# pierluigiferrari/fcn8s_tensorflow

Measured on AMD Instinct MI355X. Metric: training images/sec at 1024x512 bs16, higher is better.
Workload: dtype f32; 1 GPU; FCN-8s (VGG-16, fc6 7x7, 20 classes) train step, 1024x512, 16 images/GPU, SGD+momentum, keep_prob 0.5; global_batch=16, parallelism=dp1

## Files before the change

### fcn8s_tensorflow_amd/csrc/fcn8s_internal.h

```cpp
#pragma once
#include <hip/hip_runtime.h>
#include <stdint.h>
#include <cmath>
#include "../../include/fcn8s_hip.h"

#if defined(__HIP_DEVICE_COMPILE__) && !defined(__gfx950__)
#error "libfcn8s_hip is written for gfx950 (MI355X) only: build with --offload-arch=gfx950"
#endif
#define FCN8S_LDS_BYTES_NEEDED (160u * 1024u)

#include <string>
namespace fcn8s {

extern thread_local const char* g_last_kernel;
void defer_error(int code, const char* fmt, ...) __attribute__((format(printf, 2, 3)));
int take_deferred_error(std::string* text);

struct IgemmArgs {
    const float* x; const float* w; const float* bias; const float* addend; const float* mask;
    float* y;
    int N, Ma, Mb; long long M;
    int Hi, Wi, Cin, ldx;
    int KW, in_scale, tap_step, tap_off, Ktot;
    int Ho, Wo, Cout, ldy;
    int out_scale, out_offy, out_offx;
    int phases_x; long long w_phase_stride;
    float alpha; int relu; float mask_scale;
    int dropout; float keep_prob; unsigned long long seed; unsigned int stream_id;
    int batched; long long x_batch_stride, y_batch_stride;
    int m_fastest;
    int bt, ldw;
    int fixed_tile;
    int split;
};
void launch_igemm(const IgemmArgs& a, int phases, hipStream_t s);

struct Bf16ConvArgs {
    const float* x; const unsigned short* xh;
    const unsigned short* wt; const float* bias; float* y;
    int N, H, W, Cin, Cout, K;
    int relu, dropout; float keep_prob; unsigned long long seed; unsigned int stream_id;
    long long M; int m_fastest;
};
void launch_w_to_bf16_tiles(const float* w, unsigned short* wt, int K, int Cout, hipStream_t s);
bool launch_conv_bf16(const Bf16ConvArgs& a, hipStream_t s);
void launch_f32_to_bf16(const float* x, unsigned short* y, long long n, hipStream_t s);
struct Bf16Conv256Args {
    const unsigned short* xp; const unsigned short* wt; const float* bias; float* y;
    int N, H, W, Cin, Cout, K;
    int relu, dropout; float keep_prob; unsigned long long seed; unsigned int stream_id;
    long long M; int m_fastest;
    const float* addend;
    const float* mask; float mask_scale;
    int any_shape;
    const unsigned short* mask16;
    float* colpart;
    int ksplit; float* part;
    int rows_bn;
    int guarded;
    unsigned short* yb; int yb_pad;
    long long xp_ps, yb_ps, mask16_ps;
};
bool conv_bf16_256_ok(long long M, int Cin, int Cout, int mode);
void launch_w_to_bf16_t(const float* w, unsigned short* wt, int K, int Cout, hipStream_t s);
void launch_f32_to_bf16_padded(const float* x, unsigned short* xp, int N, int H, int W, int C, int pad, hipStream_t s, long long ps = 0);
int conv_bf16_rows_bm(int Cout, int rows_bn);
bool launch_conv_bf16_256(const Bf16Conv256Args& a, hipStream_t s);
struct Fp8ConvArgs {
    const unsigned char* xp = nullptr; long long xp_ps = 0;
    const unsigned char* wq = nullptr; const int* ew = nullptr;
    const float* bias = nullptr; float* y = nullptr;
    unsigned char* yq = nullptr; long long yq_ps = 0; int yq_pad = 0, yq_exp = 0;
    int ex = 0, relu = 1;
    int N = 0, H = 0, W = 0, Cin = 0, Cout = 0, K = 1;
    long long M = 0;
};
bool launch_conv_fp8(const Fp8ConvArgs& a, hipStream_t s);
void launch_w_to_fp8(const float* w, unsigned char* wq, int* ew, unsigned* amax_scratch, int rows, int Cout, hipStream_t s);
void launch_f32_to_fp8_padded(const float* x, unsigned char* xq, int N, int H, int W, int C, int pad, long long ps, int ex, hipStream_t s);
void launch_zero_border_fp8(unsigned char* xq, int planes, long long ps, int N, int H, int W, int pad, hipStream_t s);
void launch_maxpool_fp8(const unsigned char* xq, long long xps, unsigned char* yq, long long yps, int N, int H, int W, int C, int ypad, hipStream_t s);
void launch_amax(const float* x, long long n, unsigned* amax, hipStream_t s);
bool launch_f32_to_bf16_padded_colsum(const float* x, unsigned short* xp, float* db, int N, int H, int W, int C, int pad, hipStream_t s, long long ps = 0);
void launch_w_to_bf16_flip_t(const float* w, unsigned short* wt, int K, int Cin, int Cout, hipStream_t s);
struct Bf16WgradArgs {
    const unsigned short* A; const unsigned short* B; float* C;
    long long R; int Ci, Cj, K, Wp;
    long long chunk, split_stride; int plain_store;
    long long a_ps, b_ps;
};
bool launch_wgrad_bf16(const Bf16WgradArgs& a, hipStream_t s);

struct WgradArgs {
    const float* A; const float* B; float* C;
    int N, Pa, Pb; long long P;
    int Ha, Wa, Adim, lda, Areal;
    int Bdim, ldb;
    int KW, a_scale, tap_off, ntaps;
    int ldc;
    float alpha;
    float* colsum;
    int batched; long long a_batch_stride, b_batch_stride;
    int c_uninitialized;
    int plain_store;
    int split;
    long long split_stride;
};
void launch_wgrad(const WgradArgs& a, hipStream_t s);

extern thread_local int t_deterministic;
float* det_scratch(hipStream_t s, size_t floats);
float* scratch2(hipStream_t s, size_t floats);
void scratch_release(hipStream_t s);
long long scratch_bytes_live();
void launch_det_reduce(float* C, const float* ws, long long rows, int cols, int ldc, long long slab, int nsplit, bool accumulate, hipStream_t s);
bool launch_wgrad_taps(const float* X, const float* dZ, float* dW, float* db, int N, int H, int W, int Cin, int Cout,
                       int K, hipStream_t s);

bool launch_conv1_wgrad(const float* X4, const float* dZ, float* dW, float* db, int N, int H, int W, int Cout, int mfma, hipStream_t s);

bool launch_conv1_fwd(const float* x4, const float* w48, const float* bias, float* y, const float* zero16, int N, int H, int W, int Cout, int tiled, hipStream_t s, unsigned short* yb16 = nullptr, long long yb16_ps = 0);

bool launch_tconv_wgrad(const float* X, const float* dY, float* dW, int N, int Hi, int Wi, int C, int K, int S, hipStream_t s);

void launch_preprocess(const void* img, int dtype, float* out4, long long npix, hipStream_t s);
void launch_maxpool_fwd(const float* x, float* y, int N, int H, int W, int C, hipStream_t s);
void launch_maxpool_bwd(const float* x, const float* dy, float* dx, int N, int H, int W, int C,
                        int relu_mask, hipStream_t s);
void launch_maxpool_route(const float* x, unsigned char* route, int N, int H, int W, int C, hipStream_t s);
void launch_maxpool_fwd_route(const float* x, float* y, unsigned char* r, int N, int H, int W, int C, hipStream_t s, unsigned short* yb16 = nullptr, int pad = 0, long long yb16_ps = 0, int round16 = 0);
void launch_maxpool_fwd_route16(const unsigned short* xb, long long xb_ps, unsigned char* r, int N, int H, int W, int C, hipStream_t s, unsigned short* yb16, int pad, long long yb16_ps);
struct PixMap { int blocked, H, W, QH, QW, S; };
static __host__ __device__ inline long long pixmap_slots(const PixMap& m, long long npix, int N) { return m.blocked ? (long long)N * m.QH * m.QW * m.S * m.S : npix; }
int  softmax_xent_blocks(long long npix);
void launch_softmax_xent(const float* logits, const uint8_t* labels, float* dlogits, double* partials,
                         long long npix, int C, float grad_scale, hipStream_t s, float* colsum = nullptr,
                         const PixMap* map = nullptr, int N = 0);
enum XentPhase { XENT_PLAIN = 0, XENT_WEIGHTED = 1, XENT_OHEM_LOSS = 2, XENT_OHEM_GRAD = 3 };
struct OhemState {
    unsigned long long valid, ntau, kept;
    unsigned long long krem, above;
    unsigned prefix; int active;
    float t, gscale;
    unsigned pad[2];
};
static_assert(sizeof(OhemState) == 64, "OhemState: 64 bytes");
constexpr size_t LOSS_SCRATCH_BYTES = sizeof(OhemState) + (2048 + 2048 + 1024) * sizeof(unsigned);
struct XentEx {
    const float* cw = nullptr;
    float* lbuf = nullptr;
    OhemState* st = nullptr;
    unsigned* hist = nullptr;
    float tau = 0.f;
    float ce_scale = 1.f;
    const uint8_t* codes = nullptr;
    const float* ptab = nullptr;
};
void launch_softmax_xent_ex(const float* logits, const uint8_t* labels, float* dlogits, double* partials, long long npix, int C, float grad_scale,
                            hipStream_t s, float* colsum, const PixMap* map, int N, const XentEx& x, float ohem_thresh, long long ohem_min_kept);
void launch_finalize_loss(const double* partials, int nparts, long long npix, const float* regsum,
                          float rate, float* loss_out, hipStream_t s, const unsigned long long* den = nullptr, float* terms = nullptr);
struct LovaszLayout {
    int nseg = 0, C = 0, tiles = 0; long long L = 0, nsc = 0;
    size_t o_keys[2] = {0, 0}, o_pays[2] = {0, 0}, o_hist = 0, o_tcnt = 0, o_part = 0, o_G = 0, o_V = 0, o_w = 0, o_ncls = 0, o_colpart = 0, o_lov = 0;
    size_t bytes = 0;
};
LovaszLayout lovasz_layout(long long npix, int nseg, int C);
double lovasz_bytes(long long npix, int C, int nmask);
void launch_lovasz_loss(const float* x, int is_logits, const uint8_t* labels, const PixMap* map, int N, long long npix, const LovaszLayout& y,
                        int classes_all, const uint8_t* mask_dev, char* ws, float* class_loss, float* terms, float lce, float llov, float* loss_out,
                        hipStream_t s);
void launch_lovasz_backward(const float* x, int is_logits, const uint8_t* labels, const PixMap* map, int N, long long npix, const LovaszLayout& y,
                            char* ws, float lambda, int accumulate, float* out, float* colsum, hipStream_t s);
void launch_lovasz_total(float* terms, float lce, float* loss_out, hipStream_t s);
size_t soft_targets_scratch_bytes();
double soft_targets_bytes(long long npix, int C, int K);
void launch_soft_targets(const float* logits, float* dlogits, const float* probs, const uint8_t* labels, const PixMap* map, int N, long long npix, int C,
                         int K, long long row_stride, float lambda, float temperature, int all_pixels, char* ws, float* loss, float* term,
                         float* lastbias, hipStream_t s);
void launch_softmax_argmax(const float* logits, float* softmax_out, long long* argmax_out,
                           long long npix, int C, hipStream_t s, const PixMap* map = nullptr, int N = 0);
void launch_tconv_im2col(const float* x, float* A, int N, int Hi, int Wi, int C, int KP, hipStream_t s);
void launch_tconv_col2im(const float* dA, float* dx, int N, int Hi, int Wi, int C, int KP, hipStream_t s);
void launch_tconv_pack_gemm(const float* w, const float* bias, float* b2, float* b2t, float* bias_tiled, int C, int S, int KP, hipStream_t s);
void launch_tconv_unpack_dw(const float* db2, float* dw, int C, int S, hipStream_t s);
void launch_unblock_logits(const float* blocked, float* nhwc, const PixMap& map, int N, int C, hipStream_t s);
void launch_onehot_to_ids(const void* oh, int elem_bytes, long long npix, int C, uint8_t* ids, int* bad, hipStream_t s);
void launch_confusion(const uint8_t* labels, const long long* pred, long long npix,
                      unsigned long long* conf, int C, hipStream_t s);
bool launch_head_fwd(const float* x, const float* w, const float* bias, float* y, long long M, int K, int C, float alpha, hipStream_t s,
                     float* scratch = nullptr, size_t scratch_floats = 0);
bool launch_head_dgrad(const float* dy, const float* wt, const float* mask, float mask_scale, float* dx, long long M, int K, int C, float alpha,
                       hipStream_t s);
bool launch_head_wgrad(const float* x, const float* dy, float* dw, long long M, int K, int C, float alpha, hipStream_t s);
bool launch_maxpool_bwd_bf16(const float* x, const float* dy, unsigned short* dzb, float* db, int N, int H, int W, int C, hipStream_t s, const unsigned char* route = nullptr, long long dzb_ps = 0);
void launch_colsum(const float* x, float* out, long long rows, int C, hipStream_t s);
void launch_sumsq(const float* x, float* out, long long n, hipStream_t s);
void launch_axpy(float* y, const float* x, float a, long long n, hipStream_t s);
void launch_grad_accumulate(float* dst, const float* src, long long n, int mode, hipStream_t s);
constexpr int kGradNormBlocks = 2048;
struct UpdateStats { float norm, clip, scale; int ok; unsigned long long skipped; };
void launch_grad_norm(const float* g, long long n, float grad_scale, float max_norm, double* partials, void* out, bool as_floats, hipStream_t s);
struct UpdateArgs {
    int opt; float* theta; const float* g; float* m; float* v; float* shadow; long long n;
    float p0, p1, p2, p3, gs; const float* s_dev; const int* ok_dev; float ema_w;
};
void launch_update(const UpdateArgs& a, hipStream_t s);
inline float tf_adam_lr_t(float lr, float b1, float b2, long long t)
{
    return lr * (float)std::sqrt(1.0 - std::pow((double)b2, (double)t)) / (float)(1.0 - std::pow((double)b1, (double)t));
}
void launch_ema_update(float* sh, const float* theta, long long n, float w, const int* ok_dev, hipStream_t s);
void launch_swap(float* a, float* b, long long n, hipStream_t s);
void launch_flip_transpose(const float* w, float* wt, int taps, int Cin, int Cout, hipStream_t s);
void launch_pad_cin(const float* w, float* w4, int taps, int Cin, int Cinp, int Cout, hipStream_t s);
void launch_tconv_phase_pack(const float* w, float* wp, int K, int S, int C, hipStream_t s);
void launch_dropout_mask(float* mask, long long n, float keep_prob, unsigned long long seed,
                         unsigned int stream_id, hipStream_t s);
int wino_r(int KS);
int wino_nsub(int KS);
int wino_alpha(int tile, int KS);
long long wino_slab(long long T, int C);
void launch_wino_filter(int tile, const float* w, float* u, int Cin, int Cout, int KS, hipStream_t s, int transpose_out = 0);
void launch_wino_input(int tile, const float* x, float* v, int N, int H, int W, int C, int KS, hipStream_t s, unsigned* rbits_out = nullptr);
void launch_wino_input_conv1(const float* x0, const float* w4, const float* bias, float* v, int N, int H, int W, hipStream_t s, unsigned* rbits_out = nullptr);
void launch_wino_input_xb(const float* x, float* v, unsigned short* xb, int N, int H, int W, int C, hipStream_t s, unsigned* rbits_out = nullptr);
bool launch_wino_input_dout(int tile, const float* dy, float* v, float* dm, int N, int H, int W, int C, hipStream_t s, const unsigned char* pidx = nullptr);
void launch_wino_output(int tile, const float* m, const float* bias, const float* addend, const float* mask, float mask_scale,
                        int relu, float* y, int N, int H, int W, int C, int dropout, float keep, unsigned long long seed,
                        unsigned int stream_id, hipStream_t s, float* pool = nullptr, unsigned char* pidx = nullptr, int KS = 3,
                        unsigned* rbits_out = nullptr, const unsigned* rbits_in = nullptr);
size_t wino_rbits_words(int tile, int N, int H, int W, int C);
void launch_wino_dout(int tile, const float* dy, float* dm, int N, int H, int W, int C, hipStream_t s, int KS = 3, const unsigned char* pidx = nullptr);
void launch_wino_dgrad_output_dout(const float* dv, const unsigned* rbits_in, float* dm, int N, int H, int W, int C, hipStream_t s);
void launch_wino_dgrad_output_sub44(const float* dv, float* dx, int N, int H, int W, int C, hipStream_t s);
void launch_wino_dgrad_output(const float* dv, const float* addend, const float* mask, float mask_scale, const unsigned* rbits_in, float* y,
                              int N, int H, int W, int C, hipStream_t s);
bool launch_wino_out_in(const float* m, const float* bias, float* v, unsigned* rbits_out, int N, int H, int W, int C, hipStream_t s, bool always = false);
void launch_wino_dfilter(int tile, const float* du, float* dw, int Cin, int Cout, int KS, hipStream_t s);
int fft_fc6_planes();
long long fft_fc6_tiles(int N, int H, int W);
void launch_fft_fc6_filter(const float* w, float* uf, int Cin, int Cout, hipStream_t s);
void launch_fft_fc6_dfilter(const float* duf, float* dw, int Cin, int Cout, hipStream_t s);
void launch_fft_fc6_input(const float* x, float* xf, int N, int H, int W, int C, hipStream_t s);
void launch_fft_fc6_output(const float* yf, const float* bias, float* y, int N, int H, int W, int C, int relu, int dropout, float keep,
                           unsigned long long seed, unsigned int stream_id, hipStream_t s);
void launch_fft_fc6_dout(const float* dz, float* dyf, int N, int H, int W, int C, hipStream_t s);
void launch_fft_fc6_din(const float* dxf, float* patches, float* dx, int N, int H, int W, int C, hipStream_t s);
void launch_augment_u8(const unsigned char* img, const unsigned char* lab, unsigned char* oimg, unsigned char* olab, const int* params,
                       const unsigned char* vlut, int N, int H, int W, int Ho, int Wo, int void_id, hipStream_t s);
void launch_resample_u8(const unsigned char* img, const unsigned char* lab, unsigned char* oimg, unsigned char* olab, const int* params,
                        int N, int H, int W, int Ho, int Wo, int void_id, hipStream_t s);
void launch_tta_input(const void* img, int dtype, int N, int H, int W, int Hs, int Ws, int Hp, int Wp, int flip, float* out4, hipStream_t s);
void launch_tta_accumulate(const float* logits, const PixMap& map, int N, int Hs, int Ws, int flip, int C, int H, int W, float* acc,
                           int first, int last, int npasses, float* softmax_out, long long* argmax_out, hipStream_t s);
void launch_mc_accumulate(const float* logits, const PixMap& map, int N, int H, int W, int C, float* acc, float* ent_acc, int first, int last,
                          int nsamples, float* softmax_out, long long* argmax_out, float* entropy_out, float* mi_out, hipStream_t s);
bool crf_shape_supported(int C, int radius);
void launch_crf_meanfield(const float* qin, const float* prob, const unsigned char* img, int N, int H, int W, int C, int radius, int dilation,
                          float w_app, float w_smooth, float theta_alpha, float theta_beta, float theta_gamma, float* qout, long long* am, hipStream_t s);
void launch_crf_argmax(const float* p, long long npix, int C, long long* am, hipStream_t s);
size_t cityscapes_work_bytes(int N);
void launch_cityscapes_pair(const uint8_t* gt, const uint16_t* inst, const void* pred, int pred_kind, int N, long long P,
                            unsigned long long* conf, void* work, int* entries, int max_entries, unsigned long long* counts, hipStream_t s);
void launch_reliability_pair(const float* prob, const uint8_t* gt, const uint8_t* lut, const float* const* scores, const float* scales, int J,
                             int N, long long P, int C, int B, unsigned long long* calib, unsigned long long* sums, unsigned long long* hist,
                             unsigned long long* bad, hipStream_t s);
// ... 49 lines not shown
```

### fcn8s_tensorflow_amd/csrc/igemm.hip

```cpp
#include "fcn8s_internal.h"
#include <cmath>
#include <cstdlib>
#include <atomic>
#include <map>
#include <mutex>
#include <string>

namespace fcn8s {

thread_local const char* g_last_kernel = nullptr;
#define FCN8S_STR2(x) #x
#define FCN8S_STR(x) FCN8S_STR2(x)

typedef float f32x16 __attribute__((ext_vector_type(16)));
constexpr int BK_ = 16;

static __device__ __forceinline__ float4 ldg4(const float* p) { return *reinterpret_cast<const float4*>(p); }

static __device__ __forceinline__ unsigned xcd_swizzle(unsigned p, unsigned total)
{
    const unsigned q = total >> 3, r = total & 7u, xcd = p & 7u, i = p >> 3;
    return (xcd < r ? xcd * (q + 1) : r * (q + 1) + (xcd - r) * q) + i;
}

thread_local int t_deterministic = 0;
namespace {
struct ScratchBuf { float* p = nullptr; size_t cap = 0; };
std::mutex g_scratch_mu;
std::map<std::pair<int, hipStream_t>, ScratchBuf> g_scratch[2];
std::atomic<long long> g_scratch_bytes{0};
float* scratch_get(int which, hipStream_t s, size_t floats, size_t floor_)
{
    int dev = 0; (void)hipGetDevice(&dev);
    std::lock_guard<std::mutex> lk(g_scratch_mu);
    ScratchBuf& b = g_scratch[which][std::make_pair(dev, s)];
    if (b.cap < floats) {
        if (b.p) { hipFree(b.p); g_scratch_bytes -= (long long)(b.cap * sizeof(float)); }
        b.p = nullptr; b.cap = 0;
        size_t want = floats + floats / 4 + (1u << 20);
        if (want < floor_) want = floor_;
        if (hipMalloc((void**)&b.p, want * sizeof(float)) != hipSuccess) { (void)hipGetLastError(); return nullptr; }
        b.cap = want; g_scratch_bytes += (long long)(want * sizeof(float));
    }
    return b.p;
}
}
float* det_scratch(hipStream_t s, size_t floats) { return scratch_get(0, s, floats, 0); }
float* scratch2(hipStream_t s, size_t floats) { return scratch_get(1, s, floats, 1u << 18); }
void scratch_release(hipStream_t s)
{
    int dev = 0; (void)hipGetDevice(&dev);
    std::lock_guard<std::mutex> lk(g_scratch_mu);
    for (auto& pool : g_scratch) {
        auto it = pool.find(std::make_pair(dev, s));
        if (it != pool.end()) { if (it->second.p) { hipFree(it->second.p); g_scratch_bytes -= (long long)(it->second.cap * sizeof(float)); } pool.erase(it); }
    }
}
long long scratch_bytes_live() { return g_scratch_bytes.load(); }
__global__ __launch_bounds__(256) void det_reduce_kernel(float* __restrict__ C, const float* __restrict__ ws, const long long n, const int cols, const int ldc,
                                                         const long long slab, const int nsplit, const int accumulate)
{
    for (long long i = blockIdx.x * 256LL + threadIdx.x; i < n; i += (long long)gridDim.x * 256) {
        const long long off = (cols == ldc) ? i : (i / cols) * ldc + (i % cols);
        float v = accumulate ? C[off] : 0.f;
        const float* w = ws + off;
        for (int k = 0; k < nsplit; ++k) v += w[(long long)k * slab];
        C[off] = v;
    }
}
void launch_det_reduce(float* C, const float* ws, long long rows, int cols, int ldc, long long slab, int nsplit, bool accumulate, hipStream_t s)
{
    const long long n = rows * cols;
    if (n <= 0) return;
    long long blocks = (n + 255) / 256; if (blocks > 8192) blocks = 8192;
    hipLaunchKernelGGL(det_reduce_kernel, dim3((unsigned)blocks), dim3(256), 0, s, C, ws, n, cols, ldc, slab, nsplit, accumulate ? 1 : 0);
}
static __device__ __attribute__((noinline)) float dropout_apply(float v, unsigned long long idx, unsigned long long seed,
                                                               unsigned int stream, float keep)
{
    return philox_uniform(idx, seed, stream) < keep ? v / keep : 0.f;
}

template <int BM, int BN, int WM, int WN, int MODE, int BK>
__global__ __launch_bounds__(256, (MODE != 0 && BM * BN <= 128 * 128) ? 4 : 1) void igemm_fwd_kernel(const IgemmArgs p)
{
    constexpr bool FAST = MODE != 0;
    constexpr bool PLAIN = MODE == 3;
    constexpr int LDA = BK + 4, LDB = BN, F4R = BK / 4;
    constexpr int TM = BM / WM / 32, TN = BN / WN / 32;
    constexpr int A_LD = BM * F4R / 256;
    constexpr int B_F4 = BK * BN / 4;
    constexpr int B_LD = (B_F4 + 255) / 256;
    static_assert(WM * WN == 4, "4 waves");
    static_assert(TM >= 1 && TN >= 1, "tile");
    __shared__ __attribute__((aligned(16))) float smem[2 * BM * LDA + 2 * BK * LDB];
    float* As = smem;
    float* Bs = smem + 2 * BM * LDA;

    const int tid = threadIdx.x, lane = tid & 63, wave = tid >> 6;
    const int wm = wave / WN, wn = wave % WN;
    const int pz = blockIdx.z;
    const int pzy = p.batched ? 0 : pz / p.phases_x, pzx = p.batched ? 0 : pz - pzy * p.phases_x;
    const float* __restrict__ Wp = p.w + (long long)pz * p.w_phase_stride;
    const float* __restrict__ X = p.batched ? p.x + (long long)pz * p.x_batch_stride : p.x;
    float* __restrict__ Y = p.batched ? p.y + (long long)pz * p.y_batch_stride : p.y;
    const int offy = p.out_offy + pzy, offx = p.out_offx + pzx;
    const unsigned ntn = (unsigned)((p.Cout + BN - 1) / BN);
    const unsigned lid = xcd_swizzle(blockIdx.x, gridDim.x);
    const unsigned ntm = gridDim.x / ntn;
    const long long m0 = (long long)(p.m_fastest ? lid % ntm : lid / ntn) * BM;
    const int n0 = (int)(p.m_fastest ? lid / ntm : lid % ntn) * BN;
    const int MaMb = p.Ma * p.Mb;

    long long a_base[A_LD];
    int a_iy[A_LD], a_ix[A_LD];
    bool a_ok[A_LD];
#pragma unroll
    for (int i = 0; i < A_LD; ++i) {
        const int row = (tid + i * 256) / F4R;
        const long long m = m0 + row;
        a_ok[i] = m < p.M;
        if (PLAIN) { a_iy[i] = a_ix[i] = 0; a_base[i] = a_ok[i] ? m : 0; continue; }
        const long long mm = a_ok[i] ? m : 0;
        const int n = (int)(mm / MaMb);
        const int r = (int)(mm - (long long)n * MaMb);
        const int a = r / p.Mb, b = r - a * p.Mb;
        a_iy[i] = a * p.in_scale; a_ix[i] = b * p.in_scale;
        a_base[i] = (long long)n * p.Hi * p.Wi;
    }
    const int a_c4 = (tid % F4R) * 4;

    float4 ra[A_LD], rb[B_LD];
    constexpr bool TAP_INNER = MODE == 2;
    int f_ci0 = 0, f_ty = 0, f_tx = 0, f_tap = 0;
    const int ntaps = FAST ? p.Ktot / p.Cin : 1;
    const float* a_ptr[A_LD];
    unsigned a_mask[A_LD];
    bool a_val[A_LD], a_ldok[A_LD];
    const float* b_ptr[B_LD];
    auto set_tap = [&]() {
        if (PLAIN) {
#pragma unroll
            for (int i = 0; i < A_LD; ++i) { a_val[i] = a_ok[i]; a_ptr[i] = X + a_base[i] * p.ldx + a_c4; }
            return;
        }
        const int dy = f_ty * p.tap_step + p.tap_off, dx = f_tx * p.tap_step + p.tap_off;
#pragma unroll
        for (int i = 0; i < A_LD; ++i) {
            const int iy = a_iy[i] + dy, ix = a_ix[i] + dx;
            a_val[i] = a_ok[i] && (unsigned)iy < (unsigned)p.Hi && (unsigned)ix < (unsigned)p.Wi;
            const long long pix = a_val[i] ? a_base[i] + (long long)iy * p.Wi + ix : 0;
            a_ptr[i] = X + pix * p.ldx + a_c4;
        }
    };
    if (FAST) {
        if (TAP_INNER) {
#pragma unroll
            for (int i = 0; i < A_LD; ++i) {
                unsigned mk = 0;
                for (int t = 0; t < ntaps; ++t) {
                    const int ty = t / p.KW, tx = t - ty * p.KW;
                    const int iy = a_iy[i] + ty * p.tap_step + p.tap_off, ix = a_ix[i] + tx * p.tap_step + p.tap_off;
                    if (a_ok[i] && (unsigned)iy < (unsigned)p.Hi && (unsigned)ix < (unsigned)p.Wi) mk |= 1u << t;
                }
                a_mask[i] = mk;
                a_ptr[i] = X + (a_base[i] + (long long)a_iy[i] * p.Wi + a_ix[i]) * p.ldx + a_c4;
            }
        } else set_tap();
#pragma unroll
        for (int i = 0; i < B_LD; ++i) {
            const int f = tid + i * 256;
            const int k = f / (BN / 4), j = (f - k * (BN / 4)) * 4;
            b_ptr[i] = Wp + (long long)k * p.Cout + n0 + j;
        }
    }
    auto gload_fast = [&]() {
        if (TAP_INNER) {
            const long long delta = ((long long)(f_ty * p.tap_step + p.tap_off) * p.Wi + (f_tx * p.tap_step + p.tap_off)) * p.ldx + f_ci0;
            const long long boff = ((long long)f_tap * p.Cin + f_ci0) * p.Cout;
#pragma unroll
            for (int i = 0; i < A_LD; ++i) {
                const bool ok = (a_mask[i] >> f_tap) & 1u;
                ra[i] = ldg4(ok ? a_ptr[i] + delta : X);
                a_ldok[i] = ok;
            }
#pragma unroll
            for (int i = 0; i < B_LD; ++i)
                if (B_F4 % 256 == 0 || tid + i * 256 < B_F4) rb[i] = ldg4(b_ptr[i] + boff);
            ++f_tap;
            if (++f_tx == p.KW) { f_tx = 0; ++f_ty; }
            if (f_tap == ntaps) { f_tap = 0; f_tx = 0; f_ty = 0; f_ci0 += BK; }
        } else {
#pragma unroll
            for (int i = 0; i < A_LD; ++i) {
                ra[i] = ldg4(a_ptr[i] + f_ci0);
// ... 319 lines not shown
    int a_off[TM], a_sw[TM];
#pragma unroll
    for (int tm = 0; tm < TM; ++tm) {
        const int row = wm * TM * 32 + tm * 32 + (lane & 31);
        a_off[tm] = row * BK;
        a_sw[tm] = (row >> 2) & 3;
    }
    const int b_off = ((lane >> 5) * 4) * BN + wn * TN * 32 + (lane & 31);
    int bt_off[TN], bt_sw[TN];
#pragma unroll
    for (int tn = 0; tn < TN; ++tn) {
        const int row = wn * TN * 32 + tn * 32 + (lane & 31);
        bt_off[tn] = row * BK;
        bt_sw[tn] = (row >> 2) & 3;
    }
    auto compute = [&](int stage) {
        if (idle) return;
        const float* sa = smem + stage * STAGE;
        const float* sb = sa + BM * BK;
        if constexpr (NSPLIT >= 2) {
            Bf16Pieces<NSPLIT> ap[TM], bp[TN];
#pragma unroll
            for (int tm = 0; tm < TM; ++tm) {
                const float4 u = *reinterpret_cast<const float4*>(sa + a_off[tm] + (((2 * (lane >> 5)) ^ a_sw[tm]) * 4));
                const float4 v = *reinterpret_cast<const float4*>(sa + a_off[tm] + (((2 * (lane >> 5) + 1) ^ a_sw[tm]) * 4));
                const float x[8] = {u.x, u.y, u.z, u.w, v.x, v.y, v.z, v.w};
                split_bf16<NSPLIT>(x, ap[tm]);
            }
#pragma unroll
            for (int tn = 0; tn < TN; ++tn) {
                float x[8];
                if (BT) {
                    const float4 u = *reinterpret_cast<const float4*>(sb + bt_off[tn] + (((2 * (lane >> 5)) ^ bt_sw[tn]) * 4));
                    const float4 v = *reinterpret_cast<const float4*>(sb + bt_off[tn] + (((2 * (lane >> 5) + 1) ^ bt_sw[tn]) * 4));
                    x[0] = u.x; x[1] = u.y; x[2] = u.z; x[3] = u.w; x[4] = v.x; x[5] = v.y; x[6] = v.z; x[7] = v.w;
                } else {
#pragma unroll
                    for (int j = 0; j < 8; ++j) x[j] = sb[((lane >> 5) * 8 + j) * BN + wn * TN * 32 + tn * 32 + (lane & 31)];
                }
                split_bf16<NSPLIT>(x, bp[tn]);
            }
#pragma unroll
            for (int tm = 0; tm < TM; ++tm)
#pragma unroll
                for (int tn = 0; tn < TN; ++tn) acc[tm][tn] = mfma_split<NSPLIT>(ap[tm], bp[tn], acc[tm][tn]);
            return;
        }
#pragma unroll
        for (int kk2 = 0; kk2 < BK / 8; ++kk2) {
            float4 af[TM];
            float bf[TN][4];
#pragma unroll
            for (int tm = 0; tm < TM; ++tm)
                af[tm] = *reinterpret_cast<const float4*>(sa + a_off[tm] + (((kk2 * 2 + (lane >> 5)) ^ a_sw[tm]) * 4));
#pragma unroll
            for (int tn = 0; tn < TN; ++tn) {
                if (BT) {
                    const float4 t = *reinterpret_cast<const float4*>(sb + bt_off[tn] + (((kk2 * 2 + (lane >> 5)) ^ bt_sw[tn]) * 4));
                    bf[tn][0] = t.x; bf[tn][1] = t.y; bf[tn][2] = t.z; bf[tn][3] = t.w;
                } else {
#pragma unroll
                    for (int j = 0; j < 4; ++j) bf[tn][j] = sb[b_off + (kk2 * 8 + j) * BN + tn * 32];
                }
            }
#pragma unroll
            for (int j = 0; j < 4; ++j)
#pragma unroll
                for (int tm = 0; tm < TM; ++tm) {
                    const float av = j == 0 ? af[tm].x : j == 1 ? af[tm].y : j == 2 ? af[tm].z : af[tm].w;
#pragma unroll
                    for (int tn = 0; tn < TN; ++tn) acc[tm][tn] = __builtin_amdgcn_mfma_f32_32x32x2f32(av, bf[tn][j], acc[tm][tn], 0, 0, 0);
                }
        }
    };

#pragma unroll
    for (int t = 0; t < S - 1; ++t)
        if (t < nkt) issue(t, t);
    int stage = 0, pre = S - 1;
    for (int kt = 0; kt < nkt; ++kt) {
        if (kt + S - 2 < nkt) wait_vmcnt<(S - 2) * L>(); else wait_vmcnt<0>();
        __builtin_amdgcn_s_barrier();
        if (kt + S - 1 < nkt) issue(kt + S - 1, pre);
        compute(stage);
        stage = stage + 1 == S ? 0 : stage + 1;
        pre = pre + 1 == S ? 0 : pre + 1;
    }

    if (gridDim.y > 1) {
#pragma unroll
        for (int tn = 0; tn < TN; ++tn)
#pragma unroll
            for (int tm = 0; tm < TM; ++tm)
#pragma unroll
                for (int r = 0; r < 16; ++r) {
                    const long long m = m0 + wm * TM * 32 + tm * 32 + (r & 3) + 8 * (r >> 2) + 4 * (lane >> 5);
                    if (m < p.M) unsafeAtomicAdd(Y + m * p.ldy + n0 + wn * TN * 32 + tn * 32 + (lane & 31), acc[tm][tn][r]);
                }
        return;
    }
    if (!EPI) {
        __builtin_amdgcn_s_barrier();
        constexpr int LDT = 36;
        float* patch = smem + wave * 32 * LDT;
#pragma unroll
        for (int tn = 0; tn < TN; ++tn)
#pragma unroll
            for (int tm = 0; tm < TM; ++tm) {
#pragma unroll
                for (int r = 0; r < 16; ++r) patch[((r & 3) + 8 * (r >> 2) + 4 * (lane >> 5)) * LDT + (lane & 31)] = acc[tm][tn][r];
                __builtin_amdgcn_wave_barrier();
                const long long mrow = m0 + wm * TM * 32 + tm * 32;
                float* yb = Y + n0 + wn * TN * 32 + tn * 32 + (lane & 7) * 4;
                const float4 bv = p.bias ? ldg4(p.bias + n0 + wn * TN * 32 + tn * 32 + (lane & 7) * 4) : make_float4(0.f, 0.f, 0.f, 0.f);
#pragma unroll
                for (int j = 0; j < 4; ++j) {
                    const int row = j * 8 + (lane >> 3);
                    float4 v = *reinterpret_cast<const float4*>(&patch[row * LDT + (lane & 7) * 4]);
                    v.x += bv.x; v.y += bv.y; v.z += bv.z; v.w += bv.w;
                    if (mrow + row < p.M) {
                        if (p.mask) {
                            const float4 mk = ldg4(p.mask + (mrow + row) * p.ldy + n0 + wn * TN * 32 + tn * 32 + (lane & 7) * 4);
                            v.x = mk.x > 0.f ? v.x * p.mask_scale : 0.f; v.y = mk.y > 0.f ? v.y * p.mask_scale : 0.f;
                            v.z = mk.z > 0.f ? v.z * p.mask_scale : 0.f; v.w = mk.w > 0.f ? v.w * p.mask_scale : 0.f;
                        }
                        *reinterpret_cast<float4*>(yb + (mrow + row) * p.ldy) = v;
                    }
                }
                __builtin_amdgcn_wave_barrier();
            }
        return;
    }
#pragma unroll
    for (int tn = 0; tn < TN; ++tn) {
        const int col = n0 + wn * TN * 32 + tn * 32 + (lane & 31);
        const float bv = p.bias ? p.bias[col] : 0.f;
#pragma unroll
        for (int tm = 0; tm < TM; ++tm)
#pragma unroll
            for (int r = 0; r < 16; ++r) {
                const long long m = m0 + wm * TM * 32 + tm * 32 + (r & 3) + 8 * (r >> 2) + 4 * (lane >> 5);
                if (m >= p.M) continue;
                const long long off = m * p.ldy;
                float v = acc[tm][tn][r] * p.alpha + bv;
                if (p.addend) v += p.addend[off + col];
                if (p.relu) v = v > 0.f ? v : 0.f;
                if (p.mask) v = p.mask[off + col] > 0.f ? v * p.mask_scale : 0.f;
                if (p.dropout) v = dropout_apply(v, (unsigned long long)(off + col), p.seed, p.stream_id, p.keep_prob);
                Y[off + col] = v;
            }
    }
}

static __device__ __forceinline__ void glds16v(const float* vaddr, unsigned lds_byte_off)
{
    asm volatile("s_mov_b32 m0, %1\n\ts_nop 0\n\tglobal_load_lds_dwordx4 %0, off" ::"v"(vaddr), "s"(lds_byte_off) : "memory", "m0");
}
struct Conv1Args { const float* x4; const float* w48; const float* bias; float* y; const float* zero16; int N, H, W; long long M;
                   unsigned short* yb16; long long yb16_ps; };

__global__ __launch_bounds__(256, 4) void conv1_glds_kernel(const Conv1Args p)
{
    constexpr int BM = 128, BN = 64, BK = 16, NKT = 3, WN = 2, TM = 2, TN = 1, CH = 4, RPI = 16;
    constexpr int A_PW = BM / RPI / 4;
    constexpr int STAGE = BM * BK + BK * BN;
    __shared__ __attribute__((aligned(16))) float smem[NKT * STAGE];
    const int tid = threadIdx.x, lane = tid & 63, wave = __builtin_amdgcn_readfirstlane(tid >> 6);
    const int wm = wave / WN, wn = wave % WN;
    const long long m0 = (long long)blockIdx.x * BM;
    const unsigned lds0 = (unsigned)(size_t)(__attribute__((address_space(3))) float*)smem;
#pragma unroll
    for (int i = 0; i < A_PW; ++i) {
        const int row = (wave * A_PW + i) * RPI + lane / CH, pc = lane % CH;
        const int c = pc ^ ((row >> 2) & 3);
        long long m = m0 + row; if (m >= p.M) m = p.M - 1;
        const int x = (int)(m % p.W); const long long r = m / p.W; const int y = (int)(r % p.H);
#pragma unroll
        for (int kt = 0; kt < NKT; ++kt) {
            const int t = kt * 4 + c, dy = t / 3 - 1, dx = t % 3 - 1;
            const bool ok = t < 9 && (unsigned)(y + dy) < (unsigned)p.H && (unsigned)(x + dx) < (unsigned)p.W;
            const float* src = ok ? p.x4 + (m + (long long)dy * p.W + dx) * 4 : p.zero16;
            glds16v(src, lds0 + (unsigned)(kt * STAGE + (wave * A_PW + i) * 256) * 4u);
        }
    }
    {
        const int f = wave * 64 + lane;
#pragma unroll
        for (int kt = 0; kt < NKT; ++kt)
            glds16v(p.w48 + (kt * BK + f / (BN / 4)) * BN + (f % (BN / 4)) * 4, lds0 + (unsigned)(kt * STAGE + BM * BK + wave * 256) * 4u);
    }
    f32x16 acc[TM][TN];
#pragma unroll
    for (int i = 0; i < TM; ++i)
#pragma unroll
        for (int r = 0; r < 16; ++r) acc[i][0][r] = 0.f;
    wait_vmcnt<0>();
    __builtin_amdgcn_s_barrier();
    int a_off[TM], a_sw[TM];
#pragma unroll
    for (int tm = 0; tm < TM; ++tm) {
        const int row = wm * TM * 32 + tm * 32 + (lane & 31);
        a_off[tm] = row * BK; a_sw[tm] = (row >> 2) & 3;
    }
    const int b_off = ((lane >> 5) * 4) * BN + wn * TN * 32 + (lane & 31);
#pragma unroll
    for (int kt = 0; kt < NKT; ++kt) {
        const float* sa = smem + kt * STAGE;
        const float* sb = sa + BM * BK;
#pragma unroll
        for (int kk2 = 0; kk2 < BK / 8; ++kk2) {
            if (kt == NKT - 1 && kk2 == 1) continue;
            float4 af[TM]; float bf[3];
#pragma unroll
            for (int tm = 0; tm < TM; ++tm) af[tm] = *reinterpret_cast<const float4*>(sa + a_off[tm] + (((kk2 * 2 + (lane >> 5)) ^ a_sw[tm]) * 4));
#pragma unroll
            for (int j = 0; j < 3; ++j) bf[j] = sb[b_off + (kk2 * 8 + j) * BN];
#pragma unroll
            for (int j = 0; j < 3; ++j)
#pragma unroll
                for (int tm = 0; tm < TM; ++tm) {
                    const float av = j == 0 ? af[tm].x : j == 1 ? af[tm].y : af[tm].z;
                    acc[tm][0] = __builtin_amdgcn_mfma_f32_32x32x2f32(av, bf[j], acc[tm][0], 0, 0, 0);
                }
        }
    }
    __builtin_amdgcn_s_barrier();
    constexpr int LDT = 36;
    float* patch = smem + wave * 32 * LDT;
    const float4 bv = ldg4(p.bias + wn * 32 + (lane & 7) * 4);
#pragma unroll
    for (int tm = 0; tm < TM; ++tm) {
#pragma unroll
        for (int r = 0; r < 16; ++r) patch[((r & 3) + 8 * (r >> 2) + 4 * (lane >> 5)) * LDT + (lane & 31)] = acc[tm][0][r];
        __builtin_amdgcn_wave_barrier();
        const long long mrow = m0 + wm * TM * 32 + tm * 32;
        float* yb = p.y + wn * 32 + (lane & 7) * 4;
#pragma unroll
        for (int j = 0; j < 4; ++j) {
            const int row = j * 8 + (lane >> 3);
            float4 v = *reinterpret_cast<const float4*>(&patch[row * LDT + (lane & 7) * 4]);
            v.x = fmaxf(v.x + bv.x, 0.f); v.y = fmaxf(v.y + bv.y, 0.f); v.z = fmaxf(v.z + bv.z, 0.f); v.w = fmaxf(v.w + bv.w, 0.f);
            if (mrow + row < p.M) *reinterpret_cast<float4*>(yb + (mrow + row) * BN) = v;
        }
        __builtin_amdgcn_wave_barrier();
    }
}
template <int TPB>
__global__ __launch_bounds__(256, 4) void conv1_tile_kernel(const Conv1Args p)
{
    constexpr int TH = 8, TW = 16, BN = 64, BK = 16, NKT = 3, WN = 2, TM = 2, HW_ = TW + 2, HH_ = TH + 2;
    constexpr int LDT = 36;
    __shared__ __attribute__((aligned(16))) float sB[NKT * BK * BN];
    __shared__ __attribute__((aligned(16))) float4 halo[HH_ * HW_];
    __shared__ __attribute__((aligned(16))) float patches[4 * 32 * LDT];
    const int tid = threadIdx.x, lane = tid & 63, wave = __builtin_amdgcn_readfirstlane(tid >> 6);
    const int wm = wave / WN, wn = wave % WN;
    const int tiles_x = p.W / TW / TPB, tiles_y = p.H / TH;
    const int bx = blockIdx.x % tiles_x, by = (blockIdx.x / tiles_x) % tiles_y, n = blockIdx.x / (tiles_x * tiles_y);
    const int y0 = by * TH;
#pragma unroll
    for (int i = 0; i < 3; ++i) reinterpret_cast<float4*>(sB)[tid + i * 256] = ldg4(p.w48 + (tid + i * 256) * 4);
    const float4 bv = ldg4(p.bias + wn * 32 + (lane & 7) * 4);
    float* patch = patches + wave * 32 * LDT;
#pragma unroll 1
  for (int it = 0; it < TPB; ++it) {
    const int x0 = (bx * TPB + it) * TW;
    if (it) __syncthreads();
    if (tid < HH_ * HW_) {
        const int hy = tid / HW_, hx = tid - hy * HW_, yy = y0 + hy - 1, xx = x0 + hx - 1;
        float4 v = make_float4(0.f, 0.f, 0.f, 0.f);
        if ((unsigned)yy < (unsigned)p.H && (unsigned)xx < (unsigned)p.W) v = ldg4(p.x4 + (((long long)n * p.H + yy) * p.W + xx) * 4);
        halo[tid] = v;
    }
    f32x16 acc[TM];
#pragma unroll
    for (int i = 0; i < TM; ++i)
#pragma unroll
        for (int r = 0; r < 16; ++r) acc[i][r] = 0.f;
    __syncthreads();
    int hbase[TM];
#pragma unroll
    for (int tm = 0; tm < TM; ++tm) {
        const int g = wm * TM + tm, py = 2 * g + ((lane & 31) >> 4), px = lane & 15;
        hbase[tm] = (py + 1) * HW_ + (px + 1);
    }
    const int b_off = ((lane >> 5) * 4) * BN + wn * 32 + (lane & 31);
#pragma unroll
    for (int kt = 0; kt < NKT; ++kt) {
#pragma unroll
        for (int kk2 = 0; kk2 < BK / 8; ++kk2) {
            if (kt == NKT - 1 && kk2 == 1) continue;
            const int t = kt * 4 + kk2 * 2 + (lane >> 5), tt = t < 9 ? t : 4, dy = tt / 3 - 1, dx = tt % 3 - 1;
            float4 af[TM]; float bf[3];
#pragma unroll
            for (int tm = 0; tm < TM; ++tm) af[tm] = halo[hbase[tm] + dy * HW_ + dx];
#pragma unroll
            for (int j = 0; j < 3; ++j) bf[j] = sB[kt * BK * BN + b_off + (kk2 * 8 + j) * BN];
#pragma unroll
            for (int j = 0; j < 3; ++j)
#pragma unroll
                for (int tm = 0; tm < TM; ++tm) {
                    const float av = j == 0 ? af[tm].x : j == 1 ? af[tm].y : af[tm].z;
                    acc[tm] = __builtin_amdgcn_mfma_f32_32x32x2f32(av, bf[j], acc[tm], 0, 0, 0);
                }
        }
    }
#pragma unroll
    for (int tm = 0; tm < TM; ++tm) {
#pragma unroll
        for (int r = 0; r < 16; ++r) patch[((r & 3) + 8 * (r >> 2) + 4 * (lane >> 5)) * LDT + (lane & 31)] = acc[tm][r];
        __builtin_amdgcn_wave_barrier();
        const int g = wm * TM + tm;
#pragma unroll
        for (int j = 0; j < 4; ++j) {
            const int row = j * 8 + (lane >> 3);
            float4 v = *reinterpret_cast<const float4*>(&patch[row * LDT + (lane & 7) * 4]);
            v.x = fmaxf(v.x + bv.x, 0.f); v.y = fmaxf(v.y + bv.y, 0.f); v.z = fmaxf(v.z + bv.z, 0.f); v.w = fmaxf(v.w + bv.w, 0.f);
            const long long pix = ((long long)n * p.H + y0 + 2 * g + (row >> 4)) * p.W + x0 + (row & 15);
            if (p.y) *reinterpret_cast<float4*>(p.y + pix * BN + wn * 32 + (lane & 7) * 4) = v;
        }
        if (p.yb16) {
            const float4 b0 = ldg4(p.bias + wn * 32 + (lane & 3) * 8), b1 = ldg4(p.bias + wn * 32 + (lane & 3) * 8 + 4);
#pragma unroll
            for (int j = 0; j < 2; ++j) {
                const int row = j * 16 + (lane >> 2);
                const float4 u = *reinterpret_cast<const float4*>(&patch[row * LDT + (lane & 3) * 8]);
                const float4 w_ = *reinterpret_cast<const float4*>(&patch[row * LDT + (lane & 3) * 8 + 4]);
                __attribute__((ext_vector_type(8))) __bf16 o;
                o[0] = (__bf16)fmaxf(u.x + b0.x, 0.f); o[1] = (__bf16)fmaxf(u.y + b0.y, 0.f); o[2] = (__bf16)fmaxf(u.z + b0.z, 0.f); o[3] = (__bf16)fmaxf(u.w + b0.w, 0.f);
                o[4] = (__bf16)fmaxf(w_.x + b1.x, 0.f); o[5] = (__bf16)fmaxf(w_.y + b1.y, 0.f); o[6] = (__bf16)fmaxf(w_.z + b1.z, 0.f); o[7] = (__bf16)fmaxf(w_.w + b1.w, 0.f);
                const long long q = ((long long)n * (p.H + 2) + y0 + 2 * g + (row >> 4) + 1) * (p.W + 2) + x0 + (row & 15) + 1;
                *reinterpret_cast<__attribute__((ext_vector_type(8))) __bf16*>(p.yb16 + (p.yb16_ps ? (long long)wn * p.yb16_ps + q * 32 + (lane & 3) * 8 : q * BN + wn * 32 + (lane & 3) * 8)) = o;
            }
        }
        __builtin_amdgcn_wave_barrier();
    }
  }
}

bool launch_conv1_fwd(const float* x4, const float* w48, const float* bias, float* y, const float* zero16, int N, int H, int W, int Cout, int tiled, hipStream_t s, unsigned short* yb16, long long yb16_ps)
{
    if (Cout != 64 || !bias || !zero16) return false;
    if ((yb16 || !y) && !(tiled && H % 8 == 0 && W % 16 == 0)) return false;
    Conv1Args a{x4, w48, bias, y, zero16, N, H, W, (long long)N * H * W, yb16, yb16_ps};
    if (tiled && H % 8 == 0 && W % 16 == 0) {
        g_last_kernel = "conv1_tile_kernel";
        const long long tiles = (long long)N * (H / 8) * (W / 16);
        if (W % 64 == 0 && tiles >= 4 * 4096) hipLaunchKernelGGL(conv1_tile_kernel<4>, dim3((unsigned)(tiles / 4)), dim3(256), 0, s, a);
        else                                  hipLaunchKernelGGL(conv1_tile_kernel<1>, dim3((unsigned)tiles), dim3(256), 0, s, a);
        return true;
    }
    g_last_kernel = "conv1_glds_kernel";
    hipLaunchKernelGGL(conv1_glds_kernel, dim3((unsigned)((a.M + 127) / 128)), dim3(256), 0, s, a);
    return true;
}

template <int BM, int BN, int WM, int WN, int BKF = 16>
static void launch_igemm_cfg(const IgemmArgs& a0, int phases, hipStream_t s)
{
    IgemmArgs a = a0;
    a.m_fastest = (double)a.Ktot * a.Cout > (double)a.M * a.Cin;
    dim3 grid((unsigned)(((a.M + BM - 1) / BM) * ((a.Cout + BN - 1) / BN)), 1, (unsigned)phases);
    const bool fast = (phases == 1 || a.batched) && a.Cin % BKF == 0 && a.Cout % BN == 0 && a.Ktot % a.Cin == 0;
    const bool tap_inner = fast && (double)a.Ktot * a.Cout * 4.0 <= 64e6 && a.Ktot / a.Cin <= 32;
    const bool plain = fast && a.batched && a.Ktot == a.Cin && !a.bias && !a.addend && !a.mask && !a.relu && !a.dropout && a.alpha == 1.f &&
                       a.out_scale == 1 && a.ldy >= a.Cout && a.ldy % 4 == 0 && a.in_scale == 1 && a.tap_off == 0;
    const int mode = !fast ? 0 : (plain ? 3 : (tap_inner ? 2 : 1));
    static const std::string base = "igemm_fwd_kernel<" + std::to_string(BM) + ", " + std::to_string(BN) + ", " + std::to_string(WM) + ", " + std::to_string(WN) + ", ";
    static const std::string tags[4] = {base + "0, 16>", base + "1, " + std::to_string(BKF) + ">", base + "2, " + std::to_string(BKF) + ">",
                                        base + "3, " + std::to_string(BKF) + ">"};
    g_last_kernel = tags[mode].c_str();
    const bool linear = (mode == 1 || mode == 3) && !a.relu && !a.mask && !a.dropout && !a.addend && a.out_scale == 1 && a.ldy == a.Cout;
    constexpr int splitk_min_kt = 64;
    const unsigned nblocks = grid.x * (unsigned)phases, nkt_all = (unsigned)(a.Ktot / BKF);
    if (linear && !t_deterministic && !a.fixed_tile && ((grid.x < 512 && nkt_all >= 512) || (nblocks < 2048 && nkt_all >= (unsigned)splitk_min_kt))) {
        unsigned ks = nkt_all >= 512 && grid.x < 512 ? 1024 / grid.x : 4096 / nblocks;
        if (ks > 8) ks = 8;
        if (ks > nkt_all / 16) ks = nkt_all / 16;
        if (ks >= 2) {
            grid.y = ks;
            const size_t nfl = a.batched ? (size_t)(phases - 1) * a.y_batch_stride + (size_t)a.M * a.Cout : (size_t)a.M * a.Cout;
            hipMemsetAsync(a.y, 0, nfl * sizeof(float), s);
        }
    }
    const bool rows1x1 = fast && a.Ktot == a.Cin && a.in_scale == 1 && a.tap_off == 0 && a.out_scale == 1 && a.out_offy == 0 && a.out_offx == 0 &&
                         (a.batched || (phases == 1 && a.Hi == a.Ma && a.Wi == a.Mb && a.Ho == a.Ma && a.Wo == a.Mb)) && a.ldy >= a.Cout;
    const bool bias_only = fast && a.bias && !a.addend && !a.mask && !a.relu && !a.dropout && a.alpha == 1.f && a.ldy % 4 == 0 && a.Cout % 4 == 0 && grid.y == 1;
    if constexpr (BN >= 64 && BKF == 16) {
        if (rows1x1 && (mode == 3 || grid.y == 1) && (long long)(BM - 1) * a.ldx < (1LL << 29) && (long long)16 * a.Cout < (1LL << 29)) {
            static const std::string gbase = "gemm_glds_kernel<" + std::to_string(BM) + ", " + std::to_string(BN) + ", " + std::to_string(WM) + ", " + std::to_string(WN) + ", 3, ";
            static const std::string xbase = "gemm_glds_x3_kernel<" + std::to_string(BM) + ", " + std::to_string(BN) + ", " + std::to_string(WM) + ", " + std::to_string(WN) + ", 3, ";
            static const std::string gt[4] = {gbase + "false>", gbase + "true>", xbase + "false>", xbase + "true>"};
            const bool mask_only = fast && a.mask && !a.bias && !a.addend && !a.relu && !a.dropout && a.alpha == 1.f && a.ldy % 4 == 0 && a.Cout % 4 == 0 && grid.y == 1;
            const bool epi = mode != 3 && !bias_only && !mask_only;
            if (a.bt) {
                static const std::string nb = "gemm_glds_nt_kernel<" + std::to_string(BM) + ", " + std::to_string(BN) + ", " + std::to_string(WM) + ", " + std::to_string(WN) + ", 3>";
                static const std::string nbx = "gemm_glds_nt_x3_kernel<" + std::to_string(BM) + ", " + std::to_string(BN) + ", " + std::to_string(WM) + ", " + std::to_string(WN) + ", 3>";
                if (mode != 3 || (long long)(BN - 1) * a.ldw >= (1LL << 29)) { defer_error(FCN8S_ERR_STATE, "transposed-B GEMM needs the plain batched form"); return; }
                static const std::string nbx2 = "gemm_glds_nt_x2_kernel<" + std::to_string(BM) + ", " + std::to_string(BN) + ", " + std::to_string(WM) + ", " + std::to_string(WN) + ", 3>";
                g_last_kernel = (a.split == 3 ? nbx : a.split == 2 ? nbx2 : nb).c_str();
                if (a.split == 3) hipLaunchKernelGGL((gemm_glds_nt_x3_kernel<BM, BN, WM, WN, 3>), grid, dim3(256), 0, s, a);
                else if (a.split == 2) hipLaunchKernelGGL((gemm_glds_nt_x2_kernel<BM, BN, WM, WN, 3>), grid, dim3(256), 0, s, a);
                else                   hipLaunchKernelGGL((gemm_glds_nt_kernel<BM, BN, WM, WN, 3>), grid, dim3(256), 0, s, a);
                return;
            }
            g_last_kernel = gt[(epi ? 1 : 0) + (a.split == 3 ? 2 : 0)].c_str();
            if (a.split == 3) {
                if (epi) hipLaunchKernelGGL((gemm_glds_x3_kernel<BM, BN, WM, WN, 3, true>), grid, dim3(256), 0, s, a);
                else     hipLaunchKernelGGL((gemm_glds_x3_kernel<BM, BN, WM, WN, 3, false>), grid, dim3(256), 0, s, a);
                return;
            }
            if (a.split == 2) {
                static const std::string x2base = "gemm_glds_x2_kernel<" + std::to_string(BM) + ", " + std::to_string(BN) + ", " + std::to_string(WM) + ", " + std::to_string(WN) + ", 3, ";
                static const std::string x2t[2] = {x2base + "false>", x2base + "true>"};
                g_last_kernel = x2t[epi ? 1 : 0].c_str();
                if (epi) hipLaunchKernelGGL((gemm_glds_x2_kernel<BM, BN, WM, WN, 3, true>), grid, dim3(256), 0, s, a);
                else     hipLaunchKernelGGL((gemm_glds_x2_kernel<BM, BN, WM, WN, 3, false>), grid, dim3(256), 0, s, a);
                return;
            }
            if (epi) hipLaunchKernelGGL((gemm_glds_kernel<BM, BN, WM, WN, 3, true>), grid, dim3(256), 0, s, a);
            else     hipLaunchKernelGGL((gemm_glds_kernel<BM, BN, WM, WN, 3, false>), grid, dim3(256), 0, s, a);
            return;
        }
    }
    if (a.bt) {
        defer_error(FCN8S_ERR_STATE, "transposed-B GEMM (M %lld, K %d, N %d, tile %dx%d) does not fit the LDS-DMA kernel", a.M, a.Ktot, a.Cout, BM, BN);
        return;
    }
    if (mode == 3)      hipLaunchKernelGGL((igemm_fwd_kernel<BM, BN, WM, WN, 3, BKF>), grid, dim3(256), 0, s, a);
    else if (mode == 2) hipLaunchKernelGGL((igemm_fwd_kernel<BM, BN, WM, WN, 2, BKF>), grid, dim3(256), 0, s, a);
    else if (mode == 1) hipLaunchKernelGGL((igemm_fwd_kernel<BM, BN, WM, WN, 1, BKF>), grid, dim3(256), 0, s, a);
    else                hipLaunchKernelGGL((igemm_fwd_kernel<BM, BN, WM, WN, 0, 16>), grid, dim3(256), 0, s, a);
}

void launch_igemm(const IgemmArgs& a, int phases, hipStream_t s)
{
    auto cost = [&](int bm, int bn, int bpc, double eff) {
        const long long blocks = ((a.M + bm - 1) / bm) * ((a.Cout + bn - 1) / bn) * phases;
        const long long n = (blocks + 255) / 256, rem = n % bpc;
        const double tail = rem == 0 ? 0.0 : (rem == 1 ? 2.0 : (rem == 2 ? 2.4 : 3.0));
        return ((double)(n / bpc) * bpc + tail) * bm * bn / eff;
    };
    if (a.fixed_tile && a.Cout % 128 == 0) { launch_igemm_cfg<128, 128, 2, 2>(a, phases, s); return; }
    if (a.fixed_tile && a.Cout % 64 == 0)  { launch_igemm_cfg<128, 64, 2, 2>(a, phases, s); return; }
    if (a.Cout <= 32)      launch_igemm_cfg<128, 32, 4, 1>(a, phases, s);
    else if (a.Cout <= 64) {
        if (cost(128, 64, 4, 1.0) <= cost(64, 64, 4, 0.9)) launch_igemm_cfg<128, 64, 2, 2>(a, phases, s);
        else                                               launch_igemm_cfg<64, 64, 2, 2>(a, phases, s);
    } else {
        const double c128 = cost(128, 128, 3, 1.0), c64x128 = cost(64, 128, 4, 0.9), c64 = cost(64, 64, 4, 0.85);
        if (a.M > 64 && c128 <= c64x128 && c128 <= c64) launch_igemm_cfg<128, 128, 2, 2>(a, phases, s);
        else if (c64x128 <= c64)                        launch_igemm_cfg<64, 128, 2, 2>(a, phases, s);
        else                                            launch_igemm_cfg<64, 64, 2, 2>(a, phases, s);
    }
}

template <int BM, int BN, int WM, int WN, int WK, bool FAST, bool COLSUM>
__global__ __launch_bounds__(256, FAST ? 4 : 1) void wgrad_kernel(const WgradArgs p, const int chunk)
{
    constexpr int BK = 16, LDA = BM, LDB = BN;
    constexpr int TM = BM / WM / 32, TN = BN / WN / 32;
    constexpr int A_F4 = BK * BM / 4, B_F4 = BK * BN / 4;
    constexpr int A_LD = (A_F4 + 255) / 256, B_LD = (B_F4 + 255) / 256;
    static_assert(WM * WN * WK == 4, "4 waves");
    __shared__ __attribute__((aligned(16))) float smem[2 * BK * LDA + 2 * BK * LDB];
    float* As = smem;
    float* Bs = smem + 2 * BK * LDA;

    const int tid = threadIdx.x, lane = tid & 63, wave = tid >> 6;
    const int wk = wave / (WM * WN), wmn = wave % (WM * WN);
    const int wm = wmn / WN, wn = wmn % WN;
    const int ntj = (p.Bdim + BN - 1) / BN;
    const int ti = blockIdx.x / ntj, tj = blockIdx.x - ti * ntj;
    const int i0 = ti * BM, j0 = tj * BN;
    const int tap = blockIdx.z;
    const int ty = tap / p.KW, tx = tap - ty * p.KW;
    const int dy = p.batched ? 0 : ty + p.tap_off, dx = p.batched ? 0 : tx + p.tap_off;
    const float* __restrict__ Ap = p.batched ? p.A + (long long)tap * p.a_batch_stride : p.A;
    const float* __restrict__ Bp = p.batched ? p.B + (long long)tap * p.b_batch_stride : p.B;
    const long long pbeg = (long long)blockIdx.y * chunk;
    const long long pend = (pbeg + chunk < p.P) ? pbeg + chunk : p.P;
    const int PaPb = p.Pa * p.Pb;
    const bool do_colsum = COLSUM && p.colsum != nullptr && tap == 0 && ti == 0 && wm == 0;

    float4 ra[A_LD], rb[B_LD];
    int s_n[A_LD], s_a[A_LD], s_b[A_LD], s_left[A_LD];
    const float* b_ptr[B_LD]; int b_left[B_LD];
    bool a_ldok[A_LD], b_ldok[B_LD];
    if (FAST) {
#pragma unroll
        for (int i = 0; i < A_LD; ++i) {
            const int f = tid + i * 256;
            const int pix = f / (BM / 4);
            const long long pp = pbeg + pix;
            const long long q = pp < p.P ? pp : 0;
            s_n[i] = (int)(q / PaPb);
            const int r = (int)(q - (long long)s_n[i] * PaPb);
            s_a[i] = r / p.Pb; s_b[i] = r - s_a[i] * p.Pb;
            s_left[i] = (int)(pend - pp);
        }
#pragma unroll
        for (int i = 0; i < B_LD; ++i) {
            const int f = tid + i * 256;
            const int pix = f / (BN / 4), c = (f - pix * (BN / 4)) * 4;
            b_ptr[i] = Bp + (pbeg + pix) * p.ldb + j0 + c;
            b_left[i] = (int)(pend - (pbeg + pix));
        }
    }
    auto gload_fast = [&]() {
#pragma unroll
        for (int i = 0; i < A_LD; ++i) {
            const int f = tid + i * 256;
            const int c = (f % (BM / 4)) * 4;
            const int iy = s_a[i] * p.a_scale + dy, ix = s_b[i] * p.a_scale + dx;
            const bool ok = s_left[i] > 0 && (unsigned)iy < (unsigned)p.Ha && (unsigned)ix < (unsigned)p.Wa;
            const long long pixi = ok ? ((long long)s_n[i] * p.Ha + iy) * p.Wa + ix : 0;
            ra[i] = ldg4(Ap + pixi * p.lda + i0 + c);
            a_ldok[i] = ok;
            s_left[i] -= BK;
            s_b[i] += BK;
            if (s_b[i] >= p.Pb) { s_b[i] -= p.Pb; if (++s_a[i] >= p.Pa) { s_a[i] = 0; ++s_n[i]; } }
        }
#pragma unroll
        for (int i = 0; i < B_LD; ++i) {
            const bool ok = b_left[i] > 0;
            rb[i] = ldg4(ok ? b_ptr[i] : Bp);
            b_ldok[i] = ok;
            b_ptr[i] += (long long)BK * p.ldb;
            b_left[i] -= BK;
        }
    };
    auto gload = [&](long long pk) {
        if (FAST) { gload_fast(); return; }
#pragma unroll
        for (int i = 0; i < A_LD; ++i) {
            const int f = tid + i * 256;
            const int pix = f / (BM / 4), c = (f - pix * (BM / 4)) * 4;
            const long long pp = pk + pix;
            bool ok = (A_F4 % 256 == 0 || f < A_F4) && pp < pend && (i0 + c) < p.Adim;
            long long off = 0;
            if (ok) {
                const int n = (int)(pp / PaPb);
                const int r = (int)(pp - (long long)n * PaPb);
                const int a = r / p.Pb, b = r - a * p.Pb;
                const int iy = a * p.a_scale + dy, ix = b * p.a_scale + dx;
                ok = (unsigned)iy < (unsigned)p.Ha && (unsigned)ix < (unsigned)p.Wa;
                off = (((long long)n * p.Ha + iy) * p.Wa + ix) * p.lda + i0 + c;
            }
            ra[i] = ok ? ldg4(Ap + off) : make_float4(0.f, 0.f, 0.f, 0.f);
        }
#pragma unroll
        for (int i = 0; i < B_LD; ++i) {
            const int f = tid + i * 256;
            const int pix = f / (BN / 4), c = (f - pix * (BN / 4)) * 4;
            const long long pp = pk + pix;
            const bool ok = (B_F4 % 256 == 0 || f < B_F4) && pp < pend && (j0 + c) < p.Bdim;
            rb[i] = ok ? ldg4(Bp + pp * p.ldb + j0 + c) : make_float4(0.f, 0.f, 0.f, 0.f);
        }
    };
    auto sstore = [&](int buf) {
#pragma unroll
        for (int i = 0; i < A_LD; ++i) {
            const int f = tid + i * 256;
            if (A_F4 % 256 == 0 || f < A_F4) {
                const int pix = f / (BM / 4), c = (f - pix * (BM / 4)) * 4;
                if (FAST && !a_ldok[i]) ra[i] = make_float4(0.f, 0.f, 0.f, 0.f);
                *reinterpret_cast<float4*>(&As[buf * BK * LDA + pix * LDA + c]) = ra[i];
            }
        }
#pragma unroll
        for (int i = 0; i < B_LD; ++i) {
            const int f = tid + i * 256;
            if (B_F4 % 256 == 0 || f < B_F4) {
                const int pix = f / (BN / 4), c = (f - pix * (BN / 4)) * 4;
                if (FAST && !b_ldok[i]) rb[i] = make_float4(0.f, 0.f, 0.f, 0.f);
                *reinterpret_cast<float4*>(&Bs[buf * BK * LDB + pix * LDB + c]) = rb[i];
            }
        }
    };

    f32x16 acc[TM][TN];
    f32x16 accs[COLSUM ? TN : 1];
#pragma unroll
    for (int j = 0; j < TN; ++j) {
#pragma unroll
        for (int r = 0; r < 16; ++r) if (COLSUM) accs[j][r] = 0.f;
#pragma unroll
        for (int i = 0; i < TM; ++i)
#pragma unroll
            for (int r = 0; r < 16; ++r) acc[i][j][r] = 0.f;
    }

    auto compute = [&](int buf) {
        const float* A = As + buf * BK * LDA + (lane >> 5) * LDA + wm * TM * 32 + (lane & 31);
        const float* B = Bs + buf * BK * LDB + (lane >> 5) * LDB + wn * TN * 32 + (lane & 31);
        constexpr int KK = 8 / WK;
#pragma unroll
// ... 720 lines not shown
```

### fcn8s_tensorflow_amd/csrc/model.hip

```cpp
#include "../../include/fcn8s_hip.h"
#include "fcn8s_internal.h"
#include "device_buffer.h"
#include "pass_state.h"
#include "conv_route.h"
#include <cstdarg>
#include <functional>

#include <dlfcn.h>
#include <atomic>
#include <chrono>
#include <thread>
#include <cmath>
#include <cstdio>
#include <cstring>
#include <cstdlib>
#include <algorithm>
#include <mutex>
#include <map>
#include <set>
#include <string>
#include <vector>

using namespace fcn8s;

extern "C" {
typedef struct ncclComm* ncclComm_t;
typedef struct { char internal[128]; } ncclUniqueId;
typedef enum { ncclSuccess = 0, ncclUnhandledCudaError = 1, ncclSystemError = 2, ncclInternalError = 3, ncclInvalidArgument = 4, ncclInvalidUsage = 5,
               ncclRemoteError = 6, ncclInProgress = 7 } ncclResult_t;
typedef enum { ncclSum = 0 } ncclRedOp_t;
typedef enum { ncclFloat = 7, ncclDouble = 8 } ncclDataType_t;
}
static_assert(sizeof(ncclUniqueId) == FCN8S_COMM_ID_BYTES, "fcn8s_comm_unique_id hands out ncclUniqueId bytes");

namespace {

thread_local std::string g_last_error;
thread_local int t_deferred_code = 0;
thread_local std::string t_deferred_text;

struct ParamInfo {
    std::string name;
    int ndim;
    int64_t shape[4];
    size_t offset, numel;
};

struct ProfGroup {
    std::string name;
    std::vector<std::pair<hipEvent_t, hipEvent_t>> ev;
    std::vector<std::pair<hipEvent_t, hipEvent_t>> ev_shared;
    double flops = 0, bytes = 0;
    int64_t launches = 0;
};

struct Act { float* p = nullptr; size_t n = 0; int H = 0, W = 0, C = 0; };

const int kConvsPerBlock[5] = {2, 2, 3, 3, 3};

struct Layer {
    char name[8], pool_name[8], pool_in[12];
    int block, pos, nconv;
    int h, w, cin, cout, K, real_cin;
    int prev, next;
    size_t w_off, b_off;
    int i_y, i_rb, i_wv, i_pool, i_pidx;
    float *y, *wv, *pool; unsigned* rb; unsigned char* pidx;
    int tile;
    RbWriter rb_writer;
    bool out_in_next, conv1_in_next;
    bool dm_from_next, pool_in_transform;
    ConvShape shape(int N) const { return ConvShape{N, h, w, cin, cout, K}; }
    bool first() const { return real_cin != 0; }
    bool last_of_block() const { return pos == nconv; }
};

}

namespace fcn8s {
void defer_error(int code, const char* fmt, ...)
{
    if (t_deferred_code) return;
    char buf[1024];
    va_list ap; va_start(ap, fmt); vsnprintf(buf, sizeof buf, fmt, ap); va_end(ap);
    t_deferred_code = code; t_deferred_text = buf;
}
int take_deferred_error(std::string* text)
{
    const int c = t_deferred_code;
    if (c && text) *text = t_deferred_text;
    t_deferred_code = 0; t_deferred_text.clear();
    return c;
}
}

struct Q8Buf { DeviceBuf<unsigned char> p; int N = 0, H = 0, W = 0, C = 0, pad = -1, ex = 0; long long ps = 0; };
struct W8Bank { DeviceBuf<unsigned char> wq; int* ew = nullptr; unsigned* amax = nullptr; };

struct fcn8s_model {
    int C = 20, fc6k = 7, device = 0;
    int widths[7] = {64, 128, 256, 512, 512, 4096, 4096};
    uint64_t seed = 0;
    std::vector<ParamInfo> params;
    std::map<std::string, int> index;
    size_t total = 0;
    size_t bucket_off[FCN8S_MAX_BUCKETS] = {0}, bucket_n[FCN8S_MAX_BUCKETS] = {0};
    hipEvent_t bucket_ev[FCN8S_MAX_BUCKETS] = {nullptr};
    bool bucket_final[FCN8S_MAX_BUCKETS] = {false};
    ncclComm_t comm = nullptr; int comm_rank = 0, comm_world = 1;
    hipStream_t comm_stream = nullptr;
    static constexpr int kCommSlots = FCN8S_MAX_BUCKETS + 1, kCommMisc = FCN8S_MAX_BUCKETS;
    hipEvent_t comm_done[kCommSlots] = {nullptr}; bool comm_pending[FCN8S_MAX_BUCKETS] = {false};
    std::mutex comm_mu;
    std::thread comm_watch; std::atomic<bool> comm_watch_stop{false}, comm_failed{false};
    std::atomic<bool> comm_inflight[kCommSlots] = {}; int64_t comm_enq_ns[kCommSlots] = {0};
    std::string comm_error; int64_t comm_timeout_ms = 600000;
    float *d_params = nullptr, *d_grads = nullptr;
    DeviceBuf<float> own_params, own_grads;
    DeviceBuf<float> d_m, d_v, d_wt, d_w1pad, d_tph[3];
    DeviceBuf<float> d_wino_u; float *d_wino_v = nullptr, *d_wino_m = nullptr;
    size_t ufl = 0;
    int wino_min_cin = 64;
    int wino_tile = 6;
    int wino_fc6 = 1;
    int fc6_fft = 1;
    int fc6_fft_wgrad = 1;
    int wino_tile_hires = 0, wino_hires_pixels = 0;
    int wino_force_tile = 0;
    int precision = FCN8S_PREC_F32;
    bool frozen = false;
    unsigned long long frozen_fp = 0; DeviceBuf<unsigned long long> d_fp;
    PinnedBuf<unsigned long long> h_fp; hipEvent_t fp_event = nullptr;
    std::map<std::string, DeviceBuf<float>> u_cache;
    std::map<std::string, DeviceBuf<float>> u_train;
    bool fwd_train = false;
    PassState pass;
    int deterministic = 0;
    int fuse_dgrad_dout = 1;
    int fuse_out_in = 1;
    int conv1_tiled = 1, conv1_wgrad_mfma = 1;
    int conv1_in_transform = 1;
    DeviceBuf<unsigned short> d_wbf16;
    std::map<std::string, DeviceBuf<unsigned short>> wbf16_cache;
    std::set<std::string> bank_stale; bool banks_stale = false;
    int bf16_gemm256 = 1;
    DeviceBuf<unsigned short> d_abf16;
    std::map<std::string, DeviceBuf<unsigned short>> xbf16;
    using G16Map = std::map<std::string, DeviceBuf<unsigned short>>;
    G16Map xg16, dyg16;
    std::set<std::string> g16_stale;
    int bf16_fuse_pool = 1;
    int bf16_infer_copies = 1;
    int bf16_rows_bn = 0;
    int bf16_acts = 1;
    bool fp8_calibrated = false; float fp8_amax[FCN8S_FP8_LAYERS] = {}; DeviceBuf<unsigned> d_fp8_amax;
    std::map<std::string, Q8Buf> q8;
    std::map<std::string, W8Bank> w8; std::set<std::string> w8_valid;
    int saved_wino_min_cin = -1, saved_wino_fc6 = -1;
    int bf16_copy_by_transform = 1;
    int64_t ws_allocs = 0;
    DeviceBuf<char> crf_buf;
    DeviceBuf<char> tta_buf;
    DeviceBuf<char> mc_buf;
    bool mc_masks = false;
    hipStream_t stream = nullptr;
    std::set<hipStream_t> streams_seen; hipEvent_t move_ev = nullptr;
    int64_t step = 0;
    int N = 0, H = 0, W = 0;
    int plan_N = 0;
    DeviceBuf<char> arena;
    std::map<std::string, Act> acts;
    std::vector<Layer> layers;
    struct KeptDy { DeviceBuf<float> p; size_t n = 0; };
    int keep_dy = 0; std::map<std::string, KeptDy> kept_dy;
    int tconv_gemm = 1; PixMap pm{0, 0, 0, 0, 0, 0}; int tg_kp = 0;
    float *logits_b = nullptr, *dlogits_b = nullptr, *tg_A = nullptr, *tg_dA = nullptr;
    DeviceBuf<float> tg_b2, tg_b2t, tg_bias, tg_db2;
    bool logits_nhwc_valid = false;
    float *dlogits = nullptr, *da3 = nullptr, *da4 = nullptr, *ds7 = nullptr, *gskip3 = nullptr, *gskip4 = nullptr;
    float *gbuf[2] = {nullptr, nullptr};
    int gcur = 0;
    void* d_images = nullptr; uint8_t* d_labels = nullptr;
    DeviceBuf<float> d_loss; float *d_regsum = nullptr, *d_softmax = nullptr;
    PinnedBuf<float> h_loss; hipEvent_t loss_ev = nullptr; bool loss_copied = false;
    float* d_lastbias = nullptr;
    double* d_partials = nullptr; long long* d_pred = nullptr;
    int loss_mode = 0, last_loss_mode = 0; float ohem_thresh = 0.f; int64_t ohem_min_kept = 0;
    DeviceBuf<float> d_cw; DeviceBuf<char> loss_ws;
    int bnd_R = 0; long long bnd_last = 0; DeviceBuf<float> d_btab; DeviceBuf<uint8_t> d_bcodes;
    bool lov_on = false, have_terms = false; float lov_ce = 1.f, lov_w = 0.f; int lov_per_image = 0, lov_all = 0;
    DeviceBuf<uint8_t> d_lovmask; int lov_nmask = 0; DeviceBuf<char> lov_ws; float* d_terms = nullptr;
    float kd_w = 0.f, kd_T = 1.f; int kd_all = 0; bool have_kd = false;
    const float* kd_probs = nullptr; int kd_N = 0, kd_H = 0, kd_W = 0, kd_K = 0; long long kd_stride = 0;
    DeviceBuf<char> kd_ws;
    DeviceBuf<float> d_acc; int acc_k[FCN8S_MAX_BUCKETS] = {0}; bool acc_taken[FCN8S_MAX_BUCKETS] = {false};
    float max_norm = 0.f; DeviceBuf<char> upd_ws; bool last_update_clipped = false;
    DeviceBuf<float> d_ema; double ema_decay = 0.0; int ema_warmup = 1; bool ema_swapped = false;
    DeviceBuf<unsigned long long> d_conf;
    double loss_sum = 0; int64_t loss_cnt = 0;
    float keep_prob = 1.f, l2_rate = 0.f;
    uint32_t drop_stream = 0;
    bool have_forward = false, have_loss = false, train_mode = false;
    int next_bucket = 0;
    const uint8_t* cur_labels = nullptr;
    bool profile = false, profile_detail = false;
    struct StageSlot { PinnedBuf<uint8_t> h_img, h_lab; DeviceBuf<uint8_t> d_img, d_lab;
                       hipEvent_t ready = nullptr, consumed = nullptr; bool used = false; };
    StageSlot slots[FCN8S_NUM_STAGE_SLOTS];
    hipStream_t copy_stream = nullptr;
    std::vector<ProfGroup> groups;
    std::string err;
    fcn8s_model() = default;
    fcn8s_model(const fcn8s_model&) = delete;
    ~fcn8s_model()
    {
        for (auto& g : groups) for (auto& ev : g.ev) { hipEventDestroy(ev.first); hipEventDestroy(ev.second); }
        for (auto& e : bucket_ev) if (e) hipEventDestroy(e);
        if (loss_ev) hipEventDestroy(loss_ev);
        if (move_ev) hipEventDestroy(move_ev);
        if (fp_event) hipEventDestroy(fp_event);
        for (auto& sl : slots) { if (sl.ready) hipEventDestroy(sl.ready); if (sl.consumed) hipEventDestroy(sl.consumed); }
        if (copy_stream) hipStreamDestroy(copy_stream);
    }
};

namespace {

int fail(fcn8s_model* m, int code, const std::string& msg)
{
    if (m) m->err = msg;
    g_last_error = msg;
    return code;
}
int deferred_rc(fcn8s_model* m)
{
    std::string t; const int c = take_deferred_error(&t);
    return c ? fail(m, c, t) : FCN8S_OK;
}
#define HIPCHK(m, call) do { hipError_t e_ = (call); if (e_ != hipSuccess) \
    return fail(m, e_ == hipErrorOutOfMemory ? FCN8S_ERR_OOM : FCN8S_ERR_HIP, std::string(#call) + ": " + hipGetErrorString(e_)); } while (0)

size_t align_up(size_t x, size_t a) { return (x + a - 1) / a * a; }

const int kNumBuckets = 4;
const size_t kUpdPartialsOff = 32;

void build_param_table(int C, const int widths[7], int fc6k, std::vector<ParamInfo>& out, size_t& total,
                       size_t boff[FCN8S_MAX_BUCKETS], size_t bn[FCN8S_MAX_BUCKETS])
{
    out.clear();
    size_t off = 0;
    auto add = [&](const std::string& name, std::initializer_list<int64_t> shp) {
        ParamInfo p; p.name = name; p.ndim = (int)shp.size(); p.numel = 1;
        int i = 0; for (auto s : shp) { p.shape[i++] = s; p.numel *= (size_t)s; }
        for (; i < 4; ++i) p.shape[i] = 1;
        p.offset = off; off = align_up(off + p.numel, 64);
        out.push_back(p);
    };
    int cin = 3;
    size_t conv4_start = 0, fc6_start = 0, fc7_start = 0;
    for (int b = 0; b < 5; ++b)
        for (int i = 1; i <= kConvsPerBlock[b]; ++i) {
            char nm[32]; snprintf(nm, sizeof nm, "conv%d_%d", b + 1, i);
            if (b == 3 && i == 1) conv4_start = off;
            add(std::string(nm) + "/filter", {3, 3, cin, widths[b]});
            add(std::string(nm) + "/biases", {widths[b]});
            cin = widths[b];
        }
    fc6_start = off;
    add("fc6/weights", {fc6k, fc6k, widths[4], widths[5]});
    add("fc6/biases", {widths[5]});
    fc7_start = off;
    add("fc7/weights", {1, 1, widths[5], widths[6]});
    add("fc7/biases", {widths[6]});
    add("pool3_1x1/kernel", {1, 1, widths[2], C});
    add("pool3_1x1/bias", {C});
    add("pool4_1x1/kernel", {1, 1, widths[3], C});
    add("pool4_1x1/bias", {C});
    add("fc7_1x1/kernel", {1, 1, widths[6], C});
// ... 282 lines not shown
    a.KW = K; a.in_scale = 1; a.tap_step = 1; a.tap_off = -(K - 1) / 2; a.Ktot = K * K * Cin;
    a.Ho = H; a.Wo = W; a.Cout = Cout; a.ldy = Cout;
    a.out_scale = 1; a.out_offy = 0; a.out_offx = 0; a.phases_x = 1; a.w_phase_stride = 0;
    a.seed = m ? m->seed : 0;
    const double rc = real_cin ? real_cin : Cin;
    const double flops = 2.0 * a.M * K * K * rc * Cout;
    const double bytes = 4.0 * (a.M * rc + (double)a.M * Cout + (double)K * K * rc * Cout);
    auto run = [&]() {
        if (K == 1 && !real_cin && !a.addend && !a.relu && !a.dropout) {
            if (Cout <= 32 && !a.mask && launch_head_fwd(x, w, a.bias, y, a.M, Cin, Cout, a.alpha, s, m ? m->d_wino_u : nullptr, m ? m->ufl : 0)) return;
            if (Cin <= 32 && !a.bias && launch_head_dgrad(x, w, a.mask, a.mask_scale, y, a.M, Cout, Cin, a.alpha, s)) return;
        }
        launch_igemm(a, 1, s);
    };
    { ProfScope ps(m, group, flops, bytes, layer); run(); }
}

bool conv_fwd(fcn8s_model* m, const char* group, const float* x, const float* w, float* y,
              int N, int H, int W, int Cin, int Cout, int K, const FwdEpi& e, hipStream_t s, int real_cin = 0,
              const char* layer = nullptr)
{
    if (m && K == 7 && layer && !real_cin && e.alpha == 1.f && !e.pool_out && !e.relu_bits_out && m->fwd_train && fft6_on(m, N, H, W, Cin, Cout) &&
        conv_fft6_fwd(m, layer, x, w, y, N, H, W, Cin, Cout, e.bias, e.relu, e.dropout, e.keep, e.stream_id, s)) return false;
    if (m) m->pass.drop_backward_handoffs();
    const int tile = fwd_tile(route_opts(m), ConvShape{N, H, W, Cin, Cout, K});
    if (tile && !(K == 3 && e.dropout) && e.alpha == 1.f && !real_cin) {
        const bool v_ready = m->pass.fwd_v.take(layer);
        m->pass.fwd_v.drop();
        float* vbuf = m->d_wino_v;
        if (layer) { auto it = m->acts.find(std::string("wv:") + layer); if (it != m->acts.end()) vbuf = it->second.p; }
        WinoEpi we; we.bias = e.bias; we.relu = e.relu;
        we.dropout = e.dropout; we.keep = e.keep; we.seed = m->seed; we.stream_id = e.stream_id; we.pool = e.pool_out; we.pidx = e.pool_idx;
        we.rbits_out = e.relu_bits_out; we.skip_y = e.skip_y && e.pool_out;
        if (e.relu_bits_out && layer) m->pass.rbits_ok.insert(layer);
        if (e.in_relu_bits_out && e.in_layer && K == 3) { we.in_rbits_out = e.in_relu_bits_out; m->pass.rbits_ok.insert(e.in_layer); }
        bool fused_out = false;
        if (e.next_v && e.next_layer) { we.next_v = e.next_v; we.fused_out = &fused_out; }
        conv_winograd(m, tile, K, true, x, w, y, m->d_wino_u, vbuf, m->d_wino_m, N, H, W, Cin, Cout, we, s, layer, v_ready);
        if (fused_out) { m->pass.fwd_v.give(e.next_layer); if (layer) m->pass.y_unwritten.insert(layer); }
        return e.pool_out != nullptr;
    }
    IgemmArgs a{}; a.bias = e.bias; a.alpha = e.alpha; a.relu = e.relu; a.mask_scale = 1.f; a.dropout = e.dropout; a.keep_prob = e.keep; a.stream_id = e.stream_id;
    conv_direct(m, group, a, x, w, y, N, H, W, Cin, Cout, K, s, real_cin, layer);
    return false;
}

struct BwdCall {
    fcn8s_model* m;
    hipStream_t s;
    const char* layer;
    const char* group;
    ConvShape fwd;
    bool promised = false;
};
enum class Route { taken, declined };
static bool bf16_train_step(const BwdCall& c) { return bf16_train_mode(c.m) && c.m->train_mode && c.layer; }

static Route dgrad_bf16_train(const BwdCall& c, const float* dy, float* dx, const DgradEpi& e)
{
    fcn8s_model* m = c.m; hipStream_t s = c.s; const char* layer = c.layer;
    const int N = c.fwd.N, H = c.fwd.H, W = c.fwd.W, K = c.fwd.K, Cdy = c.fwd.Cout, Cdx = c.fwd.Cin;
    if (!(bf16_train_step(c) && e.w_fwd && e.alpha == 1.f && bf16_kernels_take(transposed(c.fwd)))) return Route::declined;
    const size_t wneed = (size_t)K * K * Cdy * Cdx;
    const bool ok = m->d_wbf16.grow(wneed * sizeof(unsigned short), s, &m->ws_allocs);
    unsigned short* dyb = ok ? dyb_for(m, layer, dy, N, H, W, Cdy, K, s) : nullptr;
    if (!dyb) return Route::declined;
    { ProfScope ps(m, "weight_relayout", 0, 6.0 * wneed); launch_w_to_bf16_flip_t(e.w_fwd, m->d_wbf16, K, Cdx, Cdy, s); }
    Bf16Conv256Args g{};
    g.xp = dyb; g.xp_ps = g16_ps(N, H, W, K); g.wt = m->d_wbf16; g.y = dx; g.N = N; g.H = H; g.W = W; g.Cin = Cdy; g.Cout = Cdx; g.K = K;
    g.addend = e.addend; g.mask = e.mask; g.mask_scale = e.mask_scale; g.any_shape = 1; g.guarded = 1; g.rows_bn = m->bf16_rows_bn;
    if (e.mask && K == 3 && e.mask_scale == 1.f) {
        auto xi = m->xg16.find(layer);
        if (xi != m->xg16.end() && xi->second) { g.mask16 = xi->second + g16_off(bf16_guard_rows(3, W + 2), Cdx); g.mask16_ps = g16_ps(N, H, W, 3); }
    }
    const bool only16 = e.yb_layer && e.yb_only;
    if (only16) { g.yb = g16_for(m, m->dyg16, e.yb_layer, N, H, W, Cdx, e.yb_K, s); g.yb_pad = (e.yb_K - 1) / 2; g.yb_ps = g16_ps(N, H, W, e.yb_K); }
    long long prow = 0;
    if (g.yb) {
        prow = ((long long)N * (H + 2) * (W + 2) + conv_bf16_rows_bm(Cdx, g.rows_bn) - 1) / conv_bf16_rows_bm(Cdx, g.rows_bn);
        g.colpart = det_scratch(s, (size_t)prow * Cdx);
        if (g.colpart) g.y = nullptr; else prow = 0;
    }
    const double M = (double)N * H * W;
    bool done;
    { ProfScope ps(m, K == 1 ? "fc7_dgrad_bf16" : (K == 3 ? "conv3x3_dgrad_bf16" : "fc6_dgrad_bf16"), 2.0 * M * K * K * Cdy * Cdx,
                   (g.y ? 4.0 : 0.0) * M * Cdx + (g.yb ? 2.0 : 0.0) * M * Cdx + (g.mask16 ? 2.0 : (e.mask ? 4.0 : 0.0)) * M * Cdx + 2.0 * M * Cdy + 2.0 * wneed, layer);
      done = launch_conv_bf16_256(g, s); }
    if (done) {
        if (g.yb) m->pass.dyg16_filled.insert(e.yb_layer);
        if (g.colpart) {
            ProfScope ps(m, "colsum", 0, 4.0 * prow * Cdx);
            launch_colsum(g.colpart, Gp(m, std::string(e.yb_layer) + "/biases"), prow, Cdx, s);
            m->pass.db_taken.insert(e.yb_layer); m->pass.dy_bf16_only.insert(e.yb_layer);
        }
        return Route::taken;
    }
    if (g.colpart) { defer_error(FCN8S_ERR_SHAPE, "bf16_train: %s's data gradient was refused by the flat-position kernel", layer); return Route::taken; }
    return Route::declined;
}

static Route dgrad_fft6(const BwdCall& c, const float* dy, float* dx, const DgradEpi& e)
{
    fcn8s_model* m = c.m; const char* layer = c.layer;
    const int N = c.fwd.N, H = c.fwd.H, W = c.fwd.W, Cdy = c.fwd.Cout, Cdx = c.fwd.Cin;
    if (!(m && c.fwd.K == 7 && layer && e.alpha == 1.f && !e.addend && !e.mask && !e.relu_bits_in)) return Route::declined;
    auto kept = m->u_train.find(std::string(layer) + "#fft");
    if (!(m->pass.fft6_ready.holds(layer) && kept != m->u_train.end() && kept->second && fft6_on(m, N, H, W, Cdx, Cdy) && bt_gemm_ok(Cdy, Cdx))) return Route::declined;
    conv_fft6_dgrad(m, layer, dy, kept->second, dx, N, H, W, Cdy, Cdx, c.s);
    return Route::taken;
}

static Route dgrad_adjoint(const BwdCall& c, bool dm_ready, float* dx, const DgradEpi& e)
{
    fcn8s_model* m = c.m; hipStream_t s = c.s; const char* layer = c.layer;
    const int N = c.fwd.N, H = c.fwd.H, W = c.fwd.W, Cdy = c.fwd.Cout, Cdx = c.fwd.Cin;
    if (!(adjoint_dgrad(route_opts(m), c.fwd) && dm_ready && e.w_fwd && e.alpha == 1.f)) return Route::declined;
    const int P = 64;
    const long long T = wino_tiles(6, N, H, W);
    IgemmArgs a = position_gemm(m->d_wino_m, m->d_wino_u, m->d_wino_v, T, Cdy, Cdx); a.split = split_of(m);
    auto kept = m->u_train.find(std::string(layer) + "#6");
    if (kept != m->u_train.end() && kept->second && bt_gemm_ok(Cdy, Cdx)) {
        a.w = kept->second; a.bt = 1; a.ldw = Cdy;
    } else {
        ProfScope ps(m, "wino_transform", 0, (double)(9 + P) * 4 * Cdy * Cdx); launch_wino_filter(6, e.w_fwd, m->d_wino_u, Cdx, Cdy, 3, s, 1);
    }
    { ProfScope ps(m, "wino_gemm_dgrad", 2.0 * P * T * Cdy * Cdx, 4.0 * P * (T * (double)(Cdy + Cdx) + (double)Cdy * Cdx), layer); launch_igemm(a, P, s); }
    if (e.dm_out && e.dm_out_layer && e.relu_bits_in && !e.addend && e.mask_scale == 1.f) {
        ProfScope ps(m, "wino_transform", 0, 4.0 * ((double)N * H * W * Cdx / 32 + 2.0 * P * T * Cdx));
        launch_wino_dgrad_output_dout(m->d_wino_v, e.relu_bits_in, e.dm_out, N, H, W, Cdx, s);
        m->pass.dm_prefilled.give(e.dm_out_layer);
        return Route::taken;
    }
    { ProfScope ps(m, "wino_transform", 0, 4.0 * ((double)N * H * W * Cdx * (1.0 + (e.relu_bits_in ? 1.0 / 32 : (e.mask ? 1.0 : 0.0)) + (e.addend ? 1.0 : 0.0)) + (double)P * T * Cdx));
      launch_wino_dgrad_output(m->d_wino_v, e.addend, e.mask, e.mask_scale, e.relu_bits_in, dx, N, H, W, Cdx, s); }
    return Route::taken;
}

static Route dgrad_fc6_adjoint(const BwdCall& c, bool dm_ready, float* dx, const DgradEpi& e)
{
    fcn8s_model* m = c.m; hipStream_t s = c.s; const char* layer = c.layer;
    const int N = c.fwd.N, H = c.fwd.H, W = c.fwd.W, Cdy = c.fwd.Cout, Cdx = c.fwd.Cin;
    if (!(c.fwd.K == 7 && fc6_wino_map(route_opts(m), H, W) && dm_ready && e.alpha == 1.f && !e.mask && !e.addend && bt_gemm_ok(Cdy, 4 * Cdx))) return Route::declined;
    auto kept = m->u_train.find(std::string(layer) + "#4");
    if (!(kept != m->u_train.end() && kept->second)) return Route::declined;
    const int P = 49, Ng = 4 * Cdx;
    const long long T = wino_tiles(4, N, H, W);
    IgemmArgs a = position_gemm(m->d_wino_m, kept->second, m->d_wino_v, T, Cdy, Ng); a.split = split_of(m);
    a.bt = 1; a.ldw = Cdy;
    { ProfScope ps(m, "wino_gemm_fc6_dgrad", 2.0 * P * T * Cdy * Ng, 4.0 * P * (T * (double)(Cdy + Ng) + (double)Cdy * Ng), layer); launch_igemm(a, P, s); }
    { ProfScope ps(m, "wino_transform", 0, 4.0 * ((double)N * H * W * Cdx + (double)P * T * Ng)); launch_wino_dgrad_output_sub44(m->d_wino_v, dx, N, H, W, Cdx, s); }
    return Route::taken;
}

static Route dgrad_winograd(const BwdCall& c, bool v_ready, const float* dy, const float* wt, float* dx, const DgradEpi& e)
{
    fcn8s_model* m = c.m;
    const int tile = dgrad_tile(route_opts(m), c.fwd);
    if (!(tile && e.alpha == 1.f)) return Route::declined;
    WinoEpi we; we.addend = e.addend; we.mask = e.mask; we.mask_scale = e.mask_scale; we.seed = m->seed; we.rbits_in = e.relu_bits_in;
    conv_winograd(m, tile, c.fwd.K, false, dy, wt, dx, m->d_wino_u, m->d_wino_v, m->d_wino_m, c.fwd.N, c.fwd.H, c.fwd.W, c.fwd.Cout, c.fwd.Cin, we, c.s, c.layer, v_ready);
    return Route::taken;
}

static void dgrad_direct(const BwdCall& c, const float* dy, const float* wt, float* dx, const DgradEpi& e)
{
    IgemmArgs a{}; a.addend = e.addend; a.mask = e.mask; a.alpha = e.alpha; a.mask_scale = e.mask_scale; a.keep_prob = 1.f;
    conv_direct(c.m, c.group, a, dy, wt, dx, c.fwd.N, c.fwd.H, c.fwd.W, c.fwd.Cout, c.fwd.Cin, c.fwd.K, c.s, 0, c.layer);
}

void conv_dgrad(fcn8s_model* m, const char* group, const float* dy, const float* wt, float* dx,
                int N, int H, int W, int Cdy, int Cdx, int K, const DgradEpi& e, hipStream_t s, const char* layer = nullptr)
{
    const BwdCall c{m, s, layer, group, ConvShape{N, H, W, Cdx, Cdy, K}};
    if (dgrad_bf16_train(c, dy, dx, e) == Route::taken) return;
    if (bf16_train_step(c) && m->pass.dy_bf16_only.count(layer)) {
        defer_error(FCN8S_ERR_SHAPE, "bf16_train: %s's data gradient could not run on the bf16 kernel and its fp32 output gradient was not kept (option \"bf16_acts\" = 0 keeps it)", layer); return;
    }
    if (bf16_train_step(c) && e.mask && m->pass.in_bf16_only.count(layer)) {
        defer_error(FCN8S_ERR_SHAPE, "bf16_train: %s's data gradient could not run on the bf16 kernel and its fp32 mask was not kept (option \"bf16_acts\" = 0 keeps it)", layer); return;
    }
    const bool dm_ready = m && m->pass.dm.take(layer), v_ready = m && m->pass.dgrad_v.take(layer);
    if (m) m->pass.drop_backward_handoffs();
    if (dgrad_fft6(c, dy, dx, e) == Route::taken) return;
    if (dgrad_adjoint(c, dm_ready, dx, e) == Route::taken) return;
    if (dgrad_fc6_adjoint(c, dm_ready, dx, e) == Route::taken) return;
    if (e.lazy_wt && e.w_fwd) {
        ProfScope ps(m, "weight_relayout", 0, 8.0 * K * K * Cdy * Cdx); launch_flip_transpose(e.w_fwd, const_cast<float*>(wt), K * K, Cdx, Cdy, s);
    }
    if (dgrad_winograd(c, v_ready, dy, wt, dx, e) == Route::taken) return;
    dgrad_direct(c, dy, wt, dx, e);
}

void tconv_fwd(fcn8s_model* m, const float* x, const float* wp, const float* bias, const float* addend,
               float* y, int N, int Hi, int Wi, int C, int K, int S, hipStream_t s)
{
    IgemmArgs a{}; a.split = split_of(m);
    a.x = x; a.w = wp; a.bias = bias; a.addend = addend; a.mask = nullptr; a.y = y;
    a.N = N; a.Ma = Hi + 1; a.Mb = Wi + 1; a.M = (long long)N * a.Ma * a.Mb;
    a.Hi = Hi; a.Wi = Wi; a.Cin = C; a.ldx = C;
    a.KW = 2; a.in_scale = 1; a.tap_step = -1; a.tap_off = 0; a.Ktot = 4 * C;
    a.Ho = Hi * S; a.Wo = Wi * S; a.Cout = C; a.ldy = C;
    a.out_scale = S; a.out_offy = -(K - S) / 2; a.out_offx = -(K - S) / 2;
    a.phases_x = S; a.w_phase_stride = 4LL * C * C;
    a.alpha = 1.f; a.relu = 0; a.mask_scale = 1.f; a.dropout = 0;
    const double opix = (double)N * Hi * S * Wi * S;
    ProfScope ps(m, "tconv_fwd", 2.0 * opix * 4 * C * C, 4.0 * (opix * C * (addend ? 2 : 1) + (double)N * Hi * Wi * C)); launch_igemm(a, S * S, s);
}

void tconv_dgrad(fcn8s_model* m, const float* dy, const float* w, float* dx, int N, int Hi, int Wi, int C,
                 int K, int S, hipStream_t s)
{
    IgemmArgs a{}; a.split = split_of(m);
    a.x = dy; a.w = w; a.y = dx;
    a.N = N; a.Ma = Hi; a.Mb = Wi; a.M = (long long)N * Hi * Wi;
    a.Hi = Hi * S; a.Wi = Wi * S; a.Cin = C; a.ldx = C;
    a.KW = K; a.in_scale = S; a.tap_step = 1; a.tap_off = -(K - S) / 2; a.Ktot = K * K * C;
    a.Ho = Hi; a.Wo = Wi; a.Cout = C; a.ldy = C;
    a.out_scale = 1; a.phases_x = 1; a.alpha = 1.f; a.mask_scale = 1.f;
    const double flops = 2.0 * a.M * K * K * C * C;
    ProfScope ps(m, "tconv_dgrad", flops, 4.0 * ((double)N * Hi * S * Wi * S * C + (double)a.M * C)); launch_igemm(a, 1, s);
}

static void broken_promise(const BwdCall& c) { defer_error(FCN8S_ERR_STATE, "%s was handed dM instead of dZ but does not take the Winograd-domain path", c.layer); }

static void keep_output_gradient(const BwdCall& c, const float* dz, const unsigned char* pool_idx)
{
    fcn8s_model* m = c.m; const char* layer = c.layer;
    if (!(m && m->keep_dy && layer)) return;
    fcn8s_model::KeptDy& k = m->kept_dy[layer];
    const size_t n = (size_t)c.fwd.N * c.fwd.H * c.fwd.W * c.fwd.Cout;
    k.n = 0;
    if (!(c.promised || pool_idx || m->pass.dy_bf16_only.count(layer) || m->pass.dz_unwritten.count(layer))) {
        if (k.p.grow(n * sizeof(float), c.s)) { k.n = n; hipMemcpyAsync(k.p, dz, n * sizeof(float), hipMemcpyDeviceToDevice, c.s); }
        else defer_error(FCN8S_ERR_OOM, "keep_output_gradients: %s's copy cannot be allocated", layer);
    }
}

static Route wgrad_bf16_train(const BwdCall& c, const float* dz, float* dw, float* db, float alpha, int real_cin)
{
    fcn8s_model* m = c.m; hipStream_t s = c.s; const char* layer = c.layer;
    const int N = c.fwd.N, H = c.fwd.H, W = c.fwd.W, Cin = c.fwd.Cin, Cout = c.fwd.Cout, K = c.fwd.K;
    if (!(bf16_train_step(c) && !real_cin && alpha == 1.f && bf16_kernels_take(c.fwd))) return Route::declined;
    auto it = m->xg16.find(layer);
    if (!(it != m->xg16.end() && it->second)) return Route::declined;
    const long long P = (long long)N * H * W;
    const int pad = (K - 1) / 2, Wp_ = W + 2 * pad;
    const long long G = bf16_guard_rows(K, Wp_), R = (long long)N * (H + 2 * pad) * Wp_;
    bool db_done = false;
    unsigned short* dyb = dyb_for(m, layer, dz, N, H, W, Cout, K, s, db, &db_done);
    if (m->pass.db_taken.count(layer)) db_done = true;
    if (!dyb) return Route::declined;
    Bf16WgradArgs g{};
    g.A = it->second + g16_off(G, Cin); g.B = dyb; g.C = dw; g.R = R; g.Ci = Cin; g.Cj = Cout; g.K = K; g.Wp = Wp_; g.a_ps = g.b_ps = g16_ps(N, H, W, K);
    bool done;
    { ProfScope ps(m, K == 1 ? "fc7_wgrad_bf16" : (K == 3 ? "conv3x3_wgrad_bf16" : "fc6_wgrad_bf16"), 2.0 * P * K * K * (double)Cin * Cout, 2.0 * K * K * R * (Cin + Cout) + 4.0 * K * K * Cin * Cout, layer);
      done = launch_wgrad_bf16(g, s); }
    if (done) {
        if (db && !db_done) { ProfScope ps(m, "colsum", 0, 4.0 * P * Cout); launch_colsum(dz, db, P, Cout, s); }
        return Route::taken;
    }
    if (db_done) { defer_error(FCN8S_ERR_SHAPE, "bf16_train: %s's weight-gradient launch refused its shape after the bias gradient was taken", layer); return Route::taken; }
    return Route::declined;
}

static Route wgrad_fft6(const BwdCall& c, const float* dz, float* dw, float* db, float alpha, int real_cin)
{
    fcn8s_model* m = c.m; const char* layer = c.layer;
    if (!(m && c.fwd.K == 7 && alpha == 1.f && !real_cin && m->train_mode && m->pass.fft6_xf.take(layer))) return Route::declined;
    if (c.promised) broken_promise(c);
    m->pass.drop_backward_handoffs();
    conv_fft6_wgrad(m, layer, m->acts[std::string("wv:") + layer].p, dz, dw, db, c.fwd.N, c.fwd.H, c.fwd.W, c.fwd.Cin, c.fwd.Cout, c.s);
    return Route::taken;
}

static Route wgrad_winograd(const BwdCall& c, const float* dz, float* dw, float* db, float alpha, int real_cin, const unsigned char* pool_idx)
{
    fcn8s_model* m = c.m; hipStream_t s = c.s; const char* layer = c.layer;
    const int N = c.fwd.N, H = c.fwd.H, W = c.fwd.W, Cin = c.fwd.Cin, Cout = c.fwd.Cout, K = c.fwd.K;
    if (!(m && (K == 3 || K == 7) && layer && alpha == 1.f && !real_cin && m->train_mode)) return Route::declined;
    auto it = m->acts.find(std::string("wv:") + layer);
    if (!(it != m->acts.end() && m->d_wino_m && (K == 3 || wino_tile_for(m, H, W, 7) == 4))) return Route::declined;
    const RouteOpts ro = route_opts(m);
    const bool fuse_dgrad_input = dgrad_input_fused(ro, c.fwd), adj_bytes = adjoint_dgrad(ro, c.fwd);
    const int tile = wino_tile_for(m, H, W, K), NP = wino_alpha(tile, K) * wino_alpha(tile, K);
    const long long T = wino_tiles(tile, N, H, W);
    const int Kg = wino_nsub(K) * wino_nsub(K) * Cin;
    WgradArgs g = position_wgrad(it->second.p, m->d_wino_m, m->d_wino_u, T, Kg, Cout, NP); g.split = split_of(m);
    bool fused = false, dm_ready = false;
    const bool prefilled = c.promised && adj_bytes && !pool_idx;
    if (c.promised && !prefilled) broken_promise(c);
    if (prefilled) dm_ready = true;
    else {
        { ProfScope ps(m, "wino_transform", 0, 4.0 * ((double)N * H * W * Cout * (pool_idx ? 0.3125 : 1.0) + ((fuse_dgrad_input && !adj_bytes) ? 2.0 : 1.0) * NP * T * Cout));
          if (adj_bytes) { launch_wino_dout(6, dz, m->d_wino_m, N, H, W, Cout, s, 3, pool_idx); dm_ready = true; }
          else {
              if (fuse_dgrad_input) fused = launch_wino_input_dout(tile, dz, m->d_wino_v, m->d_wino_m, N, H, W, Cout, s, pool_idx);
              if (!fused) launch_wino_dout(tile, dz, m->d_wino_m, N, H, W, Cout, s, K);
          } }
        if (K == 7 && tile == 4 && !fused && Cin % 2 == 0 && bt_gemm_ok(Cout, 4 * Cin) && m->u_train.count(std::string(layer) + "#4") && !m->pass.fft6_ready.holds(layer)) dm_ready = true;
    }
    m->pass.drop_backward_handoffs();
    if (fused) m->pass.dgrad_v.give(layer);
    if (dm_ready) m->pass.dm.give(layer);
    { ProfScope ps(m, K == 7 ? "wino_gemm_fc6_wgrad" : "wino_gemm_wgrad", 2.0 * NP * T * Kg * Cout, 4.0 * NP * (T * (double)(Kg + Cout) + (double)Kg * Cout), layer); launch_wgrad(g, s); }
    { ProfScope ps(m, "wino_transform", 0, 4.0 * (9.0 + NP) * Cin * Cout + 4.0 * N * H * W * Cout * (tile >= 4 ? 1.0 / (tile * tile) : 1.0));
      launch_wino_dfilter(tile, m->d_wino_u, dw, Cin, Cout, K, s);
      if (db) {
          if (tile >= 4) launch_colsum(m->d_wino_m + (wino_alpha(tile, K) + 1) * wino_slab(T, Cout), db, T, Cout, s);
          else launch_colsum(dz, db, (long long)N * H * W, Cout, s);
      } }
    return Route::taken;
}

static void wgrad_direct(const BwdCall& c, const float* x, const float* dz, float* dw, float* db, float alpha, int real_cin)
{
    fcn8s_model* m = c.m; hipStream_t s = c.s;
    const int N = c.fwd.N, H = c.fwd.H, W = c.fwd.W, Cin = c.fwd.Cin, Cout = c.fwd.Cout, K = c.fwd.K;
    WgradArgs a{}; a.split = split_of(m);
    a.A = x; a.B = dz; a.C = dw;
    a.N = N; a.Pa = H; a.Pb = W; a.P = (long long)N * H * W;
    a.Ha = H; a.Wa = W; a.Adim = Cin; a.lda = Cin; a.Areal = real_cin ? real_cin : Cin;
    a.Bdim = Cout; a.ldb = Cout;
    a.KW = K; a.a_scale = 1; a.tap_off = -(K - 1) / 2; a.ntaps = K * K;
    a.ldc = Cout; a.alpha = alpha; a.colsum = db;
    const double rc = a.Areal;
    const double flops = 2.0 * a.P * K * K * rc * Cout;
    const double bytes = 4.0 * (a.P * rc + (double)a.P * Cout + (double)K * K * rc * Cout);
    const bool taps = (K == 3 || K == 7) && alpha == 1.f && !real_cin;
    const bool first = K == 3 && alpha == 1.f && real_cin == 3 && Cin == 4;
    auto run = [&]() {
        if (K == 1 && !real_cin && Cout <= 32 && launch_head_wgrad(x, dz, dw, a.P, Cin, Cout, alpha, s)) {
            if (db) launch_colsum(dz, db, a.P, Cout, s);
            return;
        }
        if (taps && launch_wgrad_taps(x, dz, dw, db, N, H, W, Cin, Cout, K, s)) return;
        if (first && launch_conv1_wgrad(x, dz, dw, db, N, H, W, Cout, m->conv1_wgrad_mfma, s)) return;
        launch_wgrad(a, s);
    };
// ... 599 lines not shown
    if (y16) { m->pass.xg16_filled.insert(nx->name); m->pass.y_unwritten.insert(nm); m->pass.in_bf16_only.insert(nx->name); }
    return FwdStep{};
}

static FwdStep fwd_conv_bf16_train(fcn8s_model* m, Layer& L, const float* x, const Bf16Opts& bo)
{
    hipStream_t s = m->stream; const int N = m->N, h = L.h, w = L.w, cin = L.cin, cout = L.cout; const char* nm = L.name;
    const Layer* nx = in_block_next(m->layers, L); const ConvShape sh = L.shape(N);
    unsigned short* xb = bo.copies ? xg16_for(m, nm, N, h, w, cin, 3, s) : nullptr;
    if (xb && !m->pass.xg16_filled.count(nm)) {
        ProfScope ps(m, "bf16_convert", 0, 4.0 * N * h * w * cin + 2.0 * N * (h + 2) * (w + 2) * cin); launch_f32_to_bf16_padded(x, xb, N, h, w, cin, 1, s, g16_ps(N, h, w, 3));
    }
    unsigned short* yb = nullptr; const char* nxk = "";
    if (out_bf16_copy(bo, nx != nullptr)) { nxk = nx->name; yb = xg16_for(m, nxk, N, h, w, cout, 3, s); }
    const bool pool16 = L.last_of_block() && pool_in_bf16(bo, sh, m->layers[L.next].shape(N), L.block);
    if (pool16) { nxk = L.pool_in; yb = xg16_for(m, nxk, N, h, w, cout, 3, s); }
    const bool only16 = yb && (pool16 || out_bf16_only(bo, sh, nx->shape(N)));
    if (!bf16_plane_fits(g16_ps(N, h, w, 3)))
        return fwd_failed(fail(m, FCN8S_ERR_SHAPE, std::string("bf16_train: a 32-channel plane of the padded bf16 copy of ") + nm + "'s input would reach 4 GiB at this batch size; use a smaller batch per GPU"));
    Bf16LayerIo io; io.allow_small = false; io.any_shape = true;
    io.xb = xb; io.xb_ps = g16_ps(N, h, w, 3); io.yb = yb; io.yb_pad = 1; io.yb_ps = g16_ps(N, h, w, 3);
    if (!bf16_conv_layer(m, "conv3x3_fwd_bf16", L, x, only16 ? nullptr : L.y, s, io)) return fwd_failed(fail(m, FCN8S_ERR_SHAPE, std::string("bf16_train: ") + nm + " does not fit the bf16 convolution kernel"));
    if (yb) m->pass.xg16_filled.insert(nxk);
    if (only16) { m->pass.y_unwritten.insert(nm); if (!pool16) m->pass.in_bf16_only.insert(nxk); }
    return FwdStep{};
}

static FwdStep fwd_conv_bf16_fwd(fcn8s_model* m, Layer& L, const float* x, bool train)
{
    hipStream_t s = m->stream; const int N = m->N;
    unsigned short* xb = train ? xb_by_transform(m, L, N, s) : nullptr;
    auto operands = [&]() {
        const Layer* pv = in_block_prev(m->layers, L);
        unsigned* irb = (pv && pv->rb && !m->pass.rbits_ok.count(pv->name)) ? pv->rb : nullptr;
        wino_backward_operands(m, L.name, x, m->d_params + L.w_off, N, L.h, L.w, L.cin, L.cout, 3, s, irb, irb ? pv->name : nullptr, xb);
    };
    if (xb) operands();
    Bf16LayerIo io; io.allow_small = false; io.xb = xb;
    if (!bf16_conv_layer(m, "conv3x3_fwd_bf16", L, x, L.y, s, io)) return fwd_declined();
    if (train && !xb) operands();
    return FwdStep{};
}

static FwdStep fwd_conv(fcn8s_model* m, Layer& L, const float* x, bool train)
{
    const Layer* nx = in_block_next(m->layers, L);
    FwdEpi e; e.bias = m->d_params + L.b_off; e.relu = 1;
    if (train && L.rb_writer == RbWriter::self) e.relu_bits_out = L.rb;
    if (train && L.pos == 2 && m->layers[L.prev].rb_writer == RbWriter::consumer) {
        e.in_relu_bits_out = m->layers[L.prev].rb; e.in_layer = m->layers[L.prev].name;
    }
    if (L.last_of_block()) {
        e.pool_out = L.pool;
        if (train) e.pool_idx = L.pidx;
        e.skip_y = !train || L.pool_in_transform;
    }
    if (L.out_in_next && m->fuse_out_in && !(bf16_fwd_mode(m) && L.block >= 3) && !bf16_train_mode(m) && !fp8_mode(m) && (!train || e.relu_bits_out)) {
        e.next_v = nx->wv ? nx->wv : m->d_wino_v; e.next_layer = nx->name;
    }
    FwdStep st;
    const float* wt = L.first() ? m->d_w1pad : m->d_params + L.w_off;
    st.pooled = conv_fwd(m, L.first() ? "conv1_1_fwd" : "conv3x3_fwd", x, wt, L.y, m->N, L.h, L.w, L.cin, L.cout, 3, e, m->stream, L.real_cin, L.name);
    return st;
}

static FwdStep fwd_pool(fcn8s_model* m, const Layer& L, const Layer& cons, const float* x, bool train, bool fp8, bool pooled, const Bf16Opts& bo)
{
    hipStream_t s = m->stream; const int N = m->N, b = L.block - 1, h = L.h, w = L.w, cin = L.cout; const char* pn = L.pool_name;
    if (fp8) {
        m->pass.pool_fused[b] = false; m->pass.pool_routed[b] = false;
        if (!pool_feeds_skip(L.block)) {
            const int ck = cons.K;
            Q8Buf* yq = q8_for(m, cons.name, N, h / 2, w / 2, cin, ck, fp8_ex(m, cons.name), s);
            if (!yq) return fwd_failed(fail(m, FCN8S_ERR_OOM, "fp8_infer: hipMalloc of an e4m3 copy failed"));
            const Q8Buf& xi = m->q8[L.pool_in];
            { ProfScope ps(m, "maxpool_fwd_fp8", 0, 1.25 * N * h * w * cin); launch_maxpool_fp8(xi.p, xi.ps, yq->p, yq->ps, N, h, w, cin, (ck - 1) / 2, s); }
            m->pass.q8_filled.insert(cons.name); m->pass.y_unwritten.insert(pn);
        } else { ProfScope ps(m, "maxpool_fwd", 0, 4.0 * N * h * w * cin * 1.25); launch_maxpool_fwd(x, L.pool, N, h, w, cin, s); }
        return FwdStep{};
    }
    m->pass.pool_fused[b] = pooled && train;
    m->pass.pool_routed[b] = false;
    const ConvShape last = L.shape(N), csh = cons.shape(N);
    if (!pooled && bf16_train_mode(m) && pool_routes(bo, last)) {
        const int ck = cons.K;
        unsigned short* yb = pool_out_bf16(bo, last, csh) ? xg16_for(m, cons.name, N, h / 2, w / 2, cin, ck, s) : nullptr;
        const bool only16 = yb && pool_out_bf16_only(bo, last, csh, L.block);
        auto pi = m->xg16.find(L.pool_in);
        const bool in16 = only16 && pool_reads_bf16(bo, last, csh, L.block) && pi != m->xg16.end() && pi->second && m->pass.xg16_filled.count(L.pool_in);
        ProfScope ps(m, "maxpool_fwd", 0, (in16 ? 2.0 : 4.0) * N * h * w * cin + 4.0 * N * h * w * cin * (only16 ? 0.0625 : 0.3125) + (yb ? 0.5 * N * h * w * cin : 0.0));
        if (in16) launch_maxpool_fwd_route16(pi->second + g16_off(bf16_guard_rows(3, w + 2), cin), g16_ps(N, h, w, 3), L.pidx, N, h, w, cin, s, yb, (ck - 1) / 2, g16_ps(N, h / 2, w / 2, ck));
        else launch_maxpool_fwd_route(x, only16 ? nullptr : L.pool, L.pidx, N, h, w, cin, s, yb, (ck - 1) / 2, g16_ps(N, h / 2, w / 2, ck),
                                      pool_feeds_skip(L.block) ? 0 : 1);
        m->pass.pool_routed[b] = true; pooled = true;
        if (yb) m->pass.xg16_filled.insert(cons.name);
        if (only16) { m->pass.y_unwritten.insert(pn); m->pass.in_bf16_only.insert(cons.name); }
    }
    if (!pooled) {
        const bool route = train && cin % 4 == 0 && L.pool_in_transform;
        ProfScope ps(m, "maxpool_fwd", 0, 4.0 * N * h * w * cin * (route ? 1.3125 : 1.25));
        if (route) { launch_maxpool_fwd_route(x, L.pool, L.pidx, N, h, w, cin, s); m->pass.pool_fused[b] = true; }
        else launch_maxpool_fwd(x, L.pool, N, h, w, cin, s);
    }
    return FwdStep{};
}

struct McLoop { int samples = 1; uint32_t stream_base = 0; std::function<void(int)> after_sample; };

static FwdStep fwd_fc(fcn8s_model* m, const float* x, float keep_prob, bool train, bool fp8, const Bf16Opts& bo, const uint32_t* mc_stream = nullptr)
{
    hipStream_t s = m->stream; const int N = m->N;
    const Layer &F6 = m->layers[13], &F7 = m->layers[14];
    const int h5 = F6.h, w5 = F6.w;
    float *w6 = m->d_params + F6.w_off, *b6 = m->d_params + F6.b_off, *w7 = m->d_params + F7.w_off, *b7 = m->d_params + F7.b_off;
    const bool drop = (train || mc_stream) && keep_prob < 1.f;
    m->drop_stream = mc_stream ? *mc_stream : (uint32_t)(2 * m->step);
    Bf16LayerIo io6, io7;
    io6.drop = io7.drop = drop; io6.keep_prob = io7.keep_prob = keep_prob; io6.stream_id = m->drop_stream; io7.stream_id = m->drop_stream + 1;
    if (fp8) {
        const Q8Buf* q7 = q8_for(m, F7.name, N, h5, w5, F7.cin, 1, fp8_ex(m, F7.name), s);
        if (!q7) return fwd_failed(fail(m, FCN8S_ERR_OOM, "fp8_infer: hipMalloc of an e4m3 copy failed"));
        int rc = fp8_conv(m, "fc6_fwd_fp8", F6.name, x, N, h5, w5, F6.cin, F6.cout, F6.K, nullptr, q7, 0, s); if (rc) return fwd_failed(rc);
        m->pass.q8_filled.insert(F7.name); m->pass.y_unwritten.insert(F6.name);
        rc = fp8_conv(m, "fc7_fwd_fp8", F7.name, F6.y, N, h5, w5, F7.cin, F7.cout, 1, F7.y, nullptr, 0, s); if (rc) return fwd_failed(rc);
    } else if (bf16_train_mode(m)) {
        unsigned short* xb6 = bo.copies ? xg16_for(m, F6.name, N, h5, w5, F6.cin, F6.K, s) : nullptr;
        if (xb6 && !m->pass.xg16_filled.count(F6.name)) { ProfScope ps(m, "bf16_convert", 0, 6.0 * N * h5 * w5 * F6.cin); launch_f32_to_bf16_padded(x, xb6, N, h5, w5, F6.cin, (F6.K - 1) / 2, s, g16_ps(N, h5, w5, F6.K)); }
        unsigned short* xb7 = bo.copies ? xg16_for(m, F7.name, N, h5, w5, F7.cin, 1, s) : nullptr;
        const bool fuse7 = xb7 != nullptr && fc7_in_from_fc6(bo);
        io6.allow_small = io7.allow_small = false; io6.any_shape = io7.any_shape = true;
        io6.xb = xb6; io6.xb_ps = g16_ps(N, h5, w5, F6.K); io6.yb = fuse7 ? xb7 : nullptr; io6.yb_pad = 0; io6.yb_ps = g16_ps(N, h5, w5, 1);
        io7.xb = xb7; io7.xb_ps = g16_ps(N, h5, w5, 1);
        if (!bf16_conv_layer(m, "fc6_fwd_bf16", F6, x, F6.y, s, io6)) return fwd_failed(fail(m, FCN8S_ERR_SHAPE, "bf16_train: fc6 does not fit the bf16 convolution kernel"));
        if (xb7 && !fuse7) { ProfScope ps(m, "bf16_convert", 0, 6.0 * N * h5 * w5 * F7.cin); launch_f32_to_bf16_padded(F6.y, xb7, N, h5, w5, F7.cin, 0, s, g16_ps(N, h5, w5, 1)); }
        if (!bf16_conv_layer(m, "fc7_fwd_bf16", F7, F6.y, F7.y, s, io7)) return fwd_failed(fail(m, FCN8S_ERR_SHAPE, "bf16_train: fc7 does not fit the bf16 convolution kernel"));
    } else if (m->precision == FCN8S_PREC_BF16_FC || bf16_fwd_mode(m)) {
        bf16_conv_layer(m, "fc6_fwd_bf16", F6, x, F6.y, s, io6);
        if (train) wino_backward_operands(m, F6.name, x, w6, N, h5, w5, F6.cin, F6.cout, F6.K, s);
        bf16_conv_layer(m, "fc7_fwd_bf16", F7, F6.y, F7.y, s, io7);
    } else {
        { FwdEpi e; e.bias = b6; e.relu = 1; e.dropout = drop; e.keep = keep_prob; e.stream_id = m->drop_stream;
          conv_fwd(m, "fc6_fwd", x, w6, F6.y, N, h5, w5, F6.cin, F6.cout, F6.K, e, s, 0, F6.name); }
        { FwdEpi e; e.bias = b7; e.relu = 1; e.dropout = drop; e.keep = keep_prob; e.stream_id = m->drop_stream + 1;
          conv_fwd(m, "fc7_fwd", F6.y, w7, F7.y, N, h5, w5, F7.cin, F7.cout, 1, e, s); }
    }
    return FwdStep{};
}

struct FwdCall { float keep_prob = 1.f; bool train = false, x0_written = false, calibrating = false; const McLoop* mc = nullptr; };

int forward(fcn8s_model* m, const void* img_dev, int dtype, const FwdCall& call)
{
    const float keep_prob = call.keep_prob; const bool train = call.train; const McLoop* mc = call.mc;
    t_deterministic = m->deterministic;
    hipStream_t s = m->stream;
    const int N = m->N, H = m->H, W = m->W, C = m->C;
    const bool fp8 = fp8_mode(m) && !train && !call.calibrating;
    if (fp8 && !m->fp8_calibrated)
        return fail(m, FCN8S_ERR_STATE, "fp8_infer: the model has no FP8 calibration (never calibrated, or its parameters changed since): run fcn8s_fp8_calibrate "
                                        "(Engine.calibrate_fp8 / FCN8s.calibrate_fp8) or restore one with fcn8s_fp8_set_calibration first");
    m->pass.begin_forward(fp8);
    bool guard_pending = false;
    if (m->frozen && keeps_banks(m) && !m->banks_stale) {
        launch_fingerprint(m->d_params, (long long)m->total, m->d_fp, s);
        m->h_fp.grow(sizeof(unsigned long long), s);
        if (m->h_fp && !m->fp_event) hipEventCreateWithFlags(&m->fp_event, hipEventDisableTiming);
        if (m->h_fp && m->fp_event) {
            hipMemcpyAsync(m->h_fp, m->d_fp, sizeof(unsigned long long), hipMemcpyDeviceToHost, s);
            hipEventRecord(m->fp_event, s);
            guard_pending = true;
        } else {
            unsigned long long fp = 0;
            hipMemcpyAsync(&fp, m->d_fp, sizeof fp, hipMemcpyDeviceToHost, s);
            hipStreamSynchronize(s);
            if (fp != m->frozen_fp) drop_banks(m);
        }
    }
    const bool fill_fp = m->frozen && (!keeps_banks(m) || m->banks_stale);
    if (!m->frozen || fill_fp) prepare_forward_weights(m);
    m->fwd_train = train;
    const Bf16Opts bo = bf16_opts(m, train);
    if (!call.x0_written) { ProfScope ps(m, "preprocess", 0, (double)N * H * W * (16 + (dtype ? 12 : 3))); launch_preprocess(img_dev, dtype, A(m, "x0"), (long long)N * H * W, s); }
    const float* x = A(m, "x0");
    size_t k = 0;
    for (int b = 0; b < 5; ++b) {
        FwdStep st;
        for (; m->layers[k].block == b + 1; ++k) {
            Layer& L = m->layers[k];
            if (fp8 && !L.first()) st = fwd_conv_fp8(m, L, x);
            else {
                st = L.first() ? fwd_conv1_1(m, L, x, train, bo) : fwd_declined();
                if (!st.done && bf16_train_mode(m) && !L.first()) st = fwd_conv_bf16_train(m, L, x, bo);
                if (!st.done && bf16_fwd_mode(m) && b >= 2) st = fwd_conv_bf16_fwd(m, L, x, train);
                if (!st.done) st = fwd_conv(m, L, x, train);
            }
            if (st.rc) return st.rc;
            x = L.y;
        }
        const Layer& last = m->layers[k - 1];
        st = fwd_pool(m, last, m->layers[k], x, train, fp8, st.pooled, bo);
        if (st.rc) return st.rc;
        x = last.pool;
    }
    const int h5 = H / 32, w5 = W / 32;
    auto skip_heads = [&]() {
        { FwdEpi e; e.bias = Wp(m, "pool3_1x1/bias"); e.alpha = 0.0001f;
          conv_fwd(m, "score1x1_fwd", A(m, "pool3"), Wp(m, "pool3_1x1/kernel"), A(m, "p3"), N, H / 8, W / 8, m->widths[2], C, 1, e, s); }
        { FwdEpi e; e.bias = Wp(m, "pool4_1x1/bias"); e.alpha = 0.01f;
          conv_fwd(m, "score1x1_fwd", A(m, "pool4"), Wp(m, "pool4_1x1/kernel"), A(m, "p4"), N, H / 16, W / 16, m->widths[3], C, 1, e, s); }
    };
    auto fc7_head_and_upsampling = [&]() {
        { FwdEpi e; e.bias = Wp(m, "fc7_1x1/bias");
          conv_fwd(m, "score1x1_fwd", A(m, "fc7"), Wp(m, "fc7_1x1/kernel"), A(m, "s7"), N, h5, w5, m->widths[6], C, 1, e, s); }
        tconv_fwd(m, A(m, "s7"), m->d_tph[0], Wp(m, "fc7_conv2d_trans/bias"), A(m, "p4"), A(m, "a4"), N, h5, w5, C, 4, 2, s);
        tconv_fwd(m, A(m, "a4"), m->d_tph[1], Wp(m, "fc7_pool4_conv2d_trans/bias"), A(m, "p3"), A(m, "a3"), N, H / 16, W / 16, C, 4, 2, s);
        if (m->tconv_gemm && m->logits_b) tconv_gemm_fwd(m);
        else tconv_fwd(m, A(m, "a3"), m->d_tph[2], Wp(m, "fc7_pool4_pool3_conv2d_trans/bias"), nullptr, A(m, "logits"), N, H / 8, W / 8, C, 16, 8, s);
        m->logits_nhwc_valid = !(m->tconv_gemm && m->logits_b);
    };
    if (!mc) {
        { const FwdStep st = fwd_fc(m, x, keep_prob, train, fp8, bo); if (st.rc) return st.rc; }
        skip_heads();
        fc7_head_and_upsampling();
    } else {
        skip_heads();
        for (int k = 0; k < mc->samples; ++k) {
            const uint32_t sid = mc->stream_base + 2u * (uint32_t)k;
            const FwdStep st = fwd_fc(m, x, keep_prob, train, fp8, bo, &sid); if (st.rc) return st.rc;
            fc7_head_and_upsampling();
            mc->after_sample(k);
        }
    }
    if (fill_fp) {
        launch_fingerprint(m->d_params, (long long)m->total, m->d_fp, s);
        hipMemcpyAsync(&m->frozen_fp, m->d_fp, sizeof m->frozen_fp, hipMemcpyDeviceToHost, s);
        hipStreamSynchronize(s);
        m->banks_stale = false;
    }
    if (guard_pending) {
        hipEventSynchronize(m->fp_event);
        if (*m->h_fp != m->frozen_fp) {
            drop_banks(m);
            return forward(m, img_dev, dtype, call);
        }
    }
    m->have_forward = true; m->train_mode = train; m->keep_prob = keep_prob; m->mc_masks = mc != nullptr;
    return FCN8S_OK;
}

int run_forward(fcn8s_model* m, const void* img_dev, int dtype, const FwdCall& call)
{
    take_deferred_error(nullptr);
    const int rc = forward(m, img_dev, dtype, call);
    if (rc) { take_deferred_error(nullptr); return rc; }
    return deferred_rc(m);
}
int run_pass(fcn8s_model* m, const void* images, int dtype, const uint8_t* labels, int N, int H, int W, int where, const FwdCall& call,
             const uint8_t** lab_dev = nullptr)
{
    int rc = ensure_workspace(m, N, H, W); if (rc) return rc;
    const void* img; const uint8_t* lab;
    rc = stage_inputs(m, images, dtype, labels, where, &img, &lab); if (rc) return rc;
    if (lab_dev) *lab_dev = lab;
    return run_forward(m, img, dtype, call);
}

struct FrozenForCall {
    fcn8s_model* const m; const bool was_frozen;
    explicit FrozenForCall(fcn8s_model* model) : m(model), was_frozen(model->frozen) { m->frozen = true; }
    ~FrozenForCall()
    {
        if (was_frozen) return;
        for (auto& kv : m->u_cache) m->bank_stale.insert("u:" + kv.first);
        for (auto& kv : m->wbf16_cache) m->bank_stale.insert("w:" + kv.first);
        m->banks_stale = true;
        m->w8_valid.clear();
        m->frozen = false;
    }
};

struct Scratch {
    DeviceBuf<char>& buf; size_t total = 0;
    struct Item { size_t off = 0, bytes = 0; };
    Item take(size_t bytes) { const Item it{total, bytes}; total += align_up(bytes, 256); return it; }
    bool grow(fcn8s_model* m) { return !total || buf.grow(total, m->stream, &m->ws_allocs); }
    template <class T> T* ptr(const Item& it) const { return it.bytes ? (T*)(buf.get() + it.off) : nullptr; }
};

struct PredictIo {
    fcn8s_model* m; Scratch& sc; const bool host;
    struct Port { void* user = nullptr; size_t bytes = 0; Scratch::Item item; } in, outs[3];
    int nouts = 0;
    PredictIo(fcn8s_model* model, Scratch& scratch, int where) : m(model), sc(scratch), host(where == FCN8S_HOST) {}
    void input(const void* images, size_t bytes) { in = Port{const_cast<void*>(images), bytes, sc.take(host ? bytes : 0)}; }
    int output(void* user, size_t bytes) { outs[nouts] = Port{user, bytes, sc.take(host && user ? bytes : 0)}; return nouts++; }
    const void* images_dev() const { return host ? sc.ptr<void>(in.item) : in.user; }
    int stage() { if (host) HIPCHK(m, hipMemcpyAsync(sc.ptr<void>(in.item), in.user, in.bytes, hipMemcpyHostToDevice, m->stream)); return FCN8S_OK; }
    void* dev(int o) const { return host ? sc.ptr<void>(outs[o].item) : outs[o].user; }
    void split(int o, bool argmax, float** sm, long long** am) const { *sm = argmax ? nullptr : (float*)dev(o); *am = argmax ? (long long*)dev(o) : nullptr; }
    int copy_out()
    {
        for (int o = 0; host && o < nouts; ++o)
            if (outs[o].user) HIPCHK(m, hipMemcpyAsync(outs[o].user, dev(o), outs[o].bytes, hipMemcpyDeviceToHost, m->stream));
        if (host) HIPCHK(m, hipStreamSynchronize(m->stream));
        return FCN8S_OK;
    }
};

int check_predict_args(fcn8s_model* m, const char* who, int dtype, int where)
{
    if (dtype != FCN8S_IMG_U8 && dtype != FCN8S_IMG_F32) return fail(m, FCN8S_ERR_BAD_ARG, std::string(who) + ": unknown image dtype");
    if (where != FCN8S_HOST && where != FCN8S_DEVICE) return fail(m, FCN8S_ERR_BAD_ARG, std::string(who) + ": `where` must be FCN8S_HOST or FCN8S_DEVICE");
    return FCN8S_OK;
}
int check_predict_shape(fcn8s_model* m, const char* who, int N, int H, int W)
{ return N <= 0 || H <= 0 || W <= 0 ? fail(m, FCN8S_ERR_SHAPE, std::string(who) + ": N, H and W must be positive") : FCN8S_OK; }
int check_padded_shape(fcn8s_model* m, const char* who, const char* which, int N, int Hp, int Wp)
{ return (double)N * Hp * Wp > (double)(1LL << 31) ? fail(m, FCN8S_ERR_SHAPE, std::string(who) + ": " + which + " padded shape is too large to plan") : FCN8S_OK; }
PixMap logits_map(fcn8s_model* m, int Hp, int Wp) { return LGM(m) ? *LGM(m) : PixMap{0, Hp, Wp, 0, 0, 0}; }

const char* kDecoderKernels[6] ={"pool3_1x1/kernel", "pool4_1x1/kernel", "fc7_1x1/kernel", "fc7_conv2d_trans/kernel",
                                  "fc7_pool4_conv2d_trans/kernel", "fc7_pool4_pool3_conv2d_trans/kernel"};

int ensure_loss_ws(fcn8s_model* m, long long npix, int mode)
{
    const size_t need = LOSS_SCRATCH_BYTES + (mode == 2 ? (size_t)npix * sizeof(float) : 0);
    return m->loss_ws.grow(need, m->stream, &m->ws_allocs) ? FCN8S_OK : fail(m, FCN8S_ERR_OOM, "the training loss's scratch cannot be allocated");
}

int ensure_lovasz_ws(fcn8s_model* m, const LovaszLayout& y)
{
    return m->lov_ws.grow(y.bytes, m->stream, &m->ws_allocs) ? FCN8S_OK : fail(m, FCN8S_ERR_OOM, "the Lovasz sort's scratch cannot be allocated");
}

int compute_loss(fcn8s_model* m, const uint8_t* lab_dev, float l2_rate, bool with_grad)
{
    hipStream_t s = m->stream;
    const long long npix = (long long)m->N * m->H * m->W;
    const int nb = softmax_xent_blocks(npix);
    const bool bnd = with_grad && m->bnd_R > 0;
    const int mode = with_grad ? (m->loss_mode ? m->loss_mode : bnd ? 1 : 0) : 0;
    if (mode) { int rc = ensure_loss_ws(m, npix, mode); if (rc) return rc; }
    if (bnd) {
        if ((long long)m->H * m->W >= (1LL << 31)) return fail(m, FCN8S_ERR_SHAPE, "fcn8s_set_boundary_loss: an image has to have fewer than 2^31 pixels");
        if (!m->d_btab || !m->d_cw) return fail(m, FCN8S_ERR_STATE, "fcn8s_set_boundary_loss: the table is missing");
        if (!m->d_bcodes.grow((size_t)npix, s, &m->ws_allocs)) return fail(m, FCN8S_ERR_OOM, "the boundary weighting's distance codes cannot be allocated");
        ProfScope ps(m, "boundary_distance", 0, 2.0 * (double)npix);
        launch_boundary_distance(lab_dev, m->N, m->H, m->W, m->bnd_R, m->d_bcodes, s);
    }
    OhemState* st = mode ? (OhemState*)m->loss_ws.get() : nullptr;
    const bool lov = with_grad && m->lov_on;
    const bool lov_sort = lov && m->lov_w != 0.f;
    const float gscale = lov ? m->lov_ce * (1.0f / (float)npix) : 1.0f / (float)npix;
    LovaszLayout ly;
    if (lov_sort) {
        if (npix / (m->lov_per_image ? m->N : 1) >= (1LL << 31)) return fail(m, FCN8S_ERR_BAD_ARG, "fcn8s_set_lovasz: a segment holds 2^31 pixels or more");
        ly = lovasz_layout(npix, m->lov_per_image ? m->N : 1, m->C);
        int rc = ensure_lovasz_ws(m, ly); if (rc) return rc;
    }
    const double xbytes = (mode == 2 ? (double)npix * (m->C * 4 * 3 + 2 + 8) : (double)npix * (m->C * 4 * (with_grad ? 2 : 1) + 1)) + (bnd ? (double)npix : 0.0);
    { ProfScope ps(m, "softmax_xent", 0, xbytes);
      if (with_grad) hipMemsetAsync(m->d_lastbias, 0, 64 * sizeof(float), s);
      const bool blk = m->tconv_gemm && m->logits_b;
      if (mode) {
          XentEx x; x.cw = m->d_cw; x.st = st; x.hist = (unsigned*)(m->loss_ws + sizeof(OhemState));
          x.lbuf = mode == 2 ? (float*)(m->loss_ws + LOSS_SCRATCH_BYTES) : nullptr;
          if (lov) x.ce_scale = m->lov_ce;
          if (bnd) { x.codes = m->d_bcodes; x.ptab = m->d_btab; }
          launch_softmax_xent_ex(blk ? m->logits_b : A(m, "logits"), lab_dev, blk ? m->dlogits_b : m->dlogits, m->d_partials, npix, m->C, gscale, s,
                                 m->d_lastbias, blk ? &m->pm : nullptr, m->N, x, mode == 2 ? m->ohem_thresh : 0.f, (long long)m->ohem_min_kept);
      } else
          launch_softmax_xent(blk ? m->logits_b : A(m, "logits"), lab_dev, with_grad ? (blk ? m->dlogits_b : m->dlogits) : nullptr, m->d_partials, npix, m->C,
                              gscale, s, with_grad ? m->d_lastbias : nullptr, blk ? &m->pm : nullptr, m->N); }
    if (with_grad) { m->last_loss_mode = mode; m->bnd_last = bnd ? npix : 0; }
    const float* reg = nullptr;
    if (l2_rate != 0.f) {
        hipMemsetAsync(m->d_regsum, 0, sizeof(float), s);
        for (auto k : kDecoderKernels) launch_sumsq(Wp(m, k), m->d_regsum, (long long)P(m, k).numel, s);
        reg = m->d_regsum;
    }
    launch_finalize_loss(m->d_partials, nb, npix, reg, l2_rate, m->d_loss, s, mode == 2 ? &st->kept : nullptr, with_grad ? m->d_terms : nullptr);
    if (with_grad) m->have_terms = true;
    if (lov_sort) {
        ProfScope ps(m, "lovasz", 0, lovasz_bytes(npix, m->C, m->lov_nmask));
        const bool blk = m->tconv_gemm && m->logits_b;
        const float* lg = blk ? m->logits_b : A(m, "logits");
        launch_lovasz_loss(lg, 1, lab_dev, blk ? &m->pm : nullptr, m->N, npix, ly, m->lov_all, m->d_lovmask, m->lov_ws, nullptr, m->d_terms,
                           m->lov_ce, m->lov_w, m->d_loss, s);
        launch_lovasz_backward(lg, 1, lab_dev, blk ? &m->pm : nullptr, m->N, npix, ly, m->lov_ws, m->lov_w, 1, blk ? m->dlogits_b : m->dlogits,
                               m->d_lastbias, s);
    } else if (lov)
        launch_lovasz_total(m->d_terms, m->lov_ce, m->d_loss, s);
    if (with_grad) m->have_kd = false;
    if (with_grad && m->kd_w != 0.f) {
        if (!m->kd_ws.grow(soft_targets_scratch_bytes(), s, &m->ws_allocs)) return fail(m, FCN8S_ERR_OOM, "the soft-target term's scratch cannot be allocated");
        ProfScope ps(m, "soft_targets", 0, soft_targets_bytes(npix, m->C, m->kd_K));
        const bool blk = m->tconv_gemm && m->logits_b;
        launch_soft_targets(blk ? m->logits_b : A(m, "logits"), blk ? m->dlogits_b : m->dlogits, m->kd_probs, lab_dev, blk ? &m->pm : nullptr, m->N, npix,
                            m->C, m->kd_K, m->kd_stride, m->kd_w, m->kd_T, m->kd_all, m->kd_ws, m->d_loss, m->d_terms + 3, m->d_lastbias, s);
        m->have_kd = true;
    }
    m->loss_copied = m->h_loss && m->loss_ev && hipMemcpyAsync(m->h_loss, m->d_loss, sizeof(float), hipMemcpyDeviceToHost, s) == hipSuccess &&
                     hipEventRecord(m->loss_ev, s) == hipSuccess;
    m->l2_rate = l2_rate; m->have_loss = true;
    return FCN8S_OK;
}

void prepare_backward_weights(fcn8s_model* m)
{
    hipStream_t s = m->stream;
    ProfScope ps(m, "weight_relayout", 0, 8.0 * ((double)m->widths[5] * m->widths[6] +
                                                 (double)m->C * (m->widths[2] + m->widths[3] + m->widths[6])));
    launch_flip_transpose(Wp(m, "fc7/weights"), WTp(m, "fc7/weights"), 1, m->widths[5], m->widths[6], s);
    launch_flip_transpose(Wp(m, "pool3_1x1/kernel"), WTp(m, "pool3_1x1/kernel"), 1, m->widths[2], m->C, s);
    launch_flip_transpose(Wp(m, "pool4_1x1/kernel"), WTp(m, "pool4_1x1/kernel"), 1, m->widths[3], m->C, s);
    launch_flip_transpose(Wp(m, "fc7_1x1/kernel"), WTp(m, "fc7_1x1/kernel"), 1, m->widths[6], m->C, s);
}

void l2_grad(fcn8s_model* m, const char* kernel)
{
    if (m->l2_rate != 0.f) launch_axpy(Gp(m, kernel), Wp(m, kernel), m->l2_rate, (long long)P(m, kernel).numel, m->stream);
}

void mark_bucket_final(fcn8s_model* m, int b, hipStream_t s)
{
    if (!m->bucket_ev[b]) hipEventCreateWithFlags(&m->bucket_ev[b], hipEventDisableTiming);
    hipEventRecord(m->bucket_ev[b], s);
    m->bucket_final[b] = true;
}

void backward_head(fcn8s_model* m)
{
    hipStream_t s = m->stream;
    const int N = m->N, H = m->H, W = m->W, C = m->C;
    const int h5 = H / 32, w5 = W / 32, h4 = H / 16, w4 = W / 16, h3 = H / 8, w3 = W / 8;
    const float inv_keep = (m->train_mode && m->keep_prob < 1.f) ? 1.f / m->keep_prob : 1.f;
    hipMemsetAsync(m->d_grads, 0, m->total * sizeof(float), s);
    prepare_backward_weights(m);
    const bool blk = m->tconv_gemm && m->logits_b;
    if (blk) tconv_gemm_wgrad(m); else tconv_wgrad(m, A(m, "a3"), m->dlogits, Gp(m, "fc7_pool4_pool3_conv2d_trans/kernel"), N, h3, w3, C, 16, 8, s);
    launch_axpy(Gp(m, "fc7_pool4_pool3_conv2d_trans/bias"), m->d_lastbias, 1.f, C, s);
    if (blk) tconv_gemm_dgrad(m); else tconv_dgrad(m, m->dlogits, Wp(m, "fc7_pool4_pool3_conv2d_trans/kernel"), m->da3, N, h3, w3, C, 16, 8, s);
    l2_grad(m, "fc7_pool4_pool3_conv2d_trans/kernel");
    conv_wgrad(m, "score1x1_wgrad", A(m, "pool3"), m->da3, Gp(m, "pool3_1x1/kernel"), Gp(m, "pool3_1x1/bias"), N, h3, w3, m->widths[2], C, 1, 0.0001f, s);
    l2_grad(m, "pool3_1x1/kernel");
    { DgradEpi e; e.alpha = 0.0001f; conv_dgrad(m, "score1x1_dgrad", m->da3, WTp(m, "pool3_1x1/kernel"), m->gskip3, N, h3, w3, C, m->widths[2], 1, e, s); }
    tconv_wgrad(m, A(m, "a4"), m->da3, Gp(m, "fc7_pool4_conv2d_trans/kernel"), N, h4, w4, C, 4, 2, s);
    launch_colsum(m->da3, Gp(m, "fc7_pool4_conv2d_trans/bias"), (long long)N * h3 * w3, C, s);
    tconv_dgrad(m, m->da3, Wp(m, "fc7_pool4_conv2d_trans/kernel"), m->da4, N, h4, w4, C, 4, 2, s);
    l2_grad(m, "fc7_pool4_conv2d_trans/kernel");
    conv_wgrad(m, "score1x1_wgrad", A(m, "pool4"), m->da4, Gp(m, "pool4_1x1/kernel"), Gp(m, "pool4_1x1/bias"), N, h4, w4, m->widths[3], C, 1, 0.01f, s);
    l2_grad(m, "pool4_1x1/kernel");
    { DgradEpi e; e.alpha = 0.01f; conv_dgrad(m, "score1x1_dgrad", m->da4, WTp(m, "pool4_1x1/kernel"), m->gskip4, N, h4, w4, C, m->widths[3], 1, e, s); }
    tconv_wgrad(m, A(m, "s7"), m->da4, Gp(m, "fc7_conv2d_trans/kernel"), N, h5, w5, C, 4, 2, s);
    launch_colsum(m->da4, Gp(m, "fc7_conv2d_trans/bias"), (long long)N * h4 * w4, C, s);
    tconv_dgrad(m, m->da4, Wp(m, "fc7_conv2d_trans/kernel"), m->ds7, N, h5, w5, C, 4, 2, s);
    l2_grad(m, "fc7_conv2d_trans/kernel");
    conv_wgrad(m, "score1x1_wgrad", A(m, "fc7"), m->ds7, Gp(m, "fc7_1x1/kernel"), Gp(m, "fc7_1x1/bias"), N, h5, w5, m->widths[6], C, 1, 1.f, s);
    l2_grad(m, "fc7_1x1/kernel");
    { DgradEpi e; e.mask = A(m, "fc7"); e.mask_scale = inv_keep;
      conv_dgrad(m, "score1x1_dgrad", m->ds7, WTp(m, "fc7_1x1/kernel"), m->gbuf[0], N, h5, w5, C, m->widths[6], 1, e, s); }
    conv_wgrad(m, "fc7_wgrad", A(m, "fc6"), m->gbuf[0], Gp(m, "fc7/weights"), Gp(m, "fc7/biases"), N, h5, w5, m->widths[5], m->widths[6], 1, 1.f, s, 0, "fc7");
    mark_bucket_final(m, 0, s);
}

void backward_fc6(fcn8s_model* m)
{
    hipStream_t s = m->stream;
    const int N = m->N, H = m->H, W = m->W;
    const int h5 = H / 32, w5 = W / 32;
    const float inv_keep = (m->train_mode && m->keep_prob < 1.f) ? 1.f / m->keep_prob : 1.f;
    { DgradEpi e; e.mask = A(m, "fc6"); e.mask_scale = inv_keep; e.w_fwd = Wp(m, "fc7/weights"); e.yb_layer = "fc6"; e.yb_K = m->fc6k;
      conv_dgrad(m, "fc7_dgrad", m->gbuf[0], WTp(m, "fc7/weights"), m->gbuf[1], N, h5, w5, m->widths[6], m->widths[5], 1, e, s, "fc7"); }
    conv_wgrad(m, "fc6_wgrad", A(m, "pool5"), m->gbuf[1], Gp(m, "fc6/weights"), Gp(m, "fc6/biases"), N, h5, w5, m->widths[4], m->widths[5], m->fc6k, 1.f, s, 0, "fc6");
    mark_bucket_final(m, 1, s);
    { DgradEpi e; e.w_fwd = Wp(m, "fc6/weights"); e.lazy_wt = 1;
      conv_dgrad(m, "fc6_dgrad", m->gbuf[1], WTp(m, "fc6/weights"), m->gbuf[0], N, h5, w5, m->widths[5], m->widths[4], m->fc6k, e, s, "fc6"); }
    m->gcur = 0;
}

void backward_blocks(fcn8s_model* m, int b_hi, int b_lo)
{
    hipStream_t s = m->stream;
    const int N = m->N;
    for (int k = (int)m->layers.size() - 1; k >= 0; --k) {
        Layer& L = m->layers[k];
        if (L.block > b_hi || L.block < b_lo) continue;
        const int b = L.block, h = L.h, w = L.w, cw = L.cout, cin = L.cin;
        const char* nm = L.name;
        float *gw = m->d_grads + L.w_off, *gb = m->d_grads + L.b_off;
        const unsigned char* pix = nullptr;
        if (L.last_of_block()) {
            if (pool_backward_fused(L, m->pass.pool_fused[b - 1])) pix = L.pidx;
            bool pool_done = false;
            if (!pix && bf16_train_mode(m) && m->train_mode && pool_bwd_writes_bf16(bf16_opts(m, true), L.shape(N))) {
                unsigned short* dzb = g16_for(m, m->dyg16, nm, N, h, w, cw, 3, s);
                if (dzb) {
                    ProfScope ps(m, "maxpool_bwd", 0, 4.0 * N * h * w * cw * (m->pass.pool_routed[b - 1] ? 0.3125 : 1.25) + 2.0 * N * h * w * cw);
                    pool_done = launch_maxpool_bwd_bf16(L.y, m->gbuf[m->gcur], dzb, gb, N, h, w, cw, s,
                                                        m->pass.pool_routed[b - 1] ? L.pidx : nullptr, g16_ps(N, h, w, 3));
                }
                if (pool_done) { m->pass.dyg16_filled.insert(nm); m->pass.db_taken.insert(nm); m->pass.dz_unwritten.insert(nm); m->gcur ^= 1; }
            }
            if (!pix && !pool_done) {
                ProfScope ps(m, "maxpool_bwd", 0, 4.0 * N * h * w * cw * 2.25);
                launch_maxpool_bwd(L.y, m->gbuf[m->gcur], m->gbuf[m->gcur ^ 1], N, h, w, cw, 1, s);
                m->gcur ^= 1;
            }
        }
        const float* dz = m->gbuf[m->gcur];
        const Layer* pv = in_block_prev(m->layers, L);
        const float* xin = pv ? pv->y : (L.first() ? A(m, "x0") : m->layers[L.prev].pool);
        conv_wgrad(m, L.first() ? "conv1_1_wgrad" : "conv3x3_wgrad", xin, dz, gw, gb, N, h, w, cin, cw, 3, 1.f, s, L.real_cin, nm, pix);
        if (L.first()) break;
        DgradEpi e; e.w_fwd = m->d_params + L.w_off; e.lazy_wt = 1;
        if (pv) {
            e.mask = xin; e.mask_scale = 1.f; e.yb_layer = pv->name; e.yb_K = 3;
            if (m->pass.rbits_ok.count(pv->name)) e.relu_bits_in = pv->rb;
            e.yb_only = bf16_train_mode(m) && dy_bf16_only(bf16_opts(m, true), pv->shape(N), pv->first(), L.shape(N));
            if (pv->dm_from_next && m->fuse_dgrad_dout && e.relu_bits_in && m->train_mode) { e.dm_out = m->d_wino_m; e.dm_out_layer = pv->name; }
        }
        else if (b == 5) e.addend = m->gskip4;
        else if (b == 4) e.addend = m->gskip3;
        conv_dgrad(m, "conv3x3_dgrad", dz, m->d_wt + L.w_off, m->gbuf[m->gcur ^ 1], N, h, w, cw, cin, 3, e, s, nm);
        m->gcur ^= 1;
    }
}

int do_backward_bucket(fcn8s_model* m, int bucket)
{
    t_deterministic = m->deterministic;
    if (!m->have_loss || !m->train_mode) return fail(m, FCN8S_ERR_STATE, "fcn8s_backward_bucket: call fcn8s_forward_loss first");
    if (bucket != m->next_bucket) return fail(m, FCN8S_ERR_STATE, "fcn8s_backward_bucket: buckets must be run in order 0, 1, ... fcn8s_num_buckets() - 1");
    if (bucket == 0) {
        m->pass.begin_backward();
        for (int b = 0; b < kNumBuckets; ++b) m->bucket_final[b] = false;
        for (int b = 0; b < kNumBuckets; ++b)
            if (m->comm_pending[b]) { hipStreamWaitEvent(m->stream, m->comm_done[b], 0); m->comm_pending[b] = false; }
        backward_head(m);
    }
    else if (bucket == 1) backward_fc6(m);
    else if (bucket == 2) backward_blocks(m, 5, 4);
    else backward_blocks(m, 3, 1);
    if (!m->bucket_final[bucket]) mark_bucket_final(m, bucket, m->stream);
    m->next_bucket = bucket + 1;
    hipError_t e = hipGetLastError();
    if (e != hipSuccess) return fail(m, FCN8S_ERR_HIP, std::string("backward launch: ") + hipGetErrorString(e));
    return FCN8S_OK;
}

int ensure_opt_state(fcn8s_model* m)
{
    if (m->d_m) return FCN8S_OK;
    if (!m->d_m.grow(m->total * sizeof(float), m->stream) || !m->d_v.grow(m->total * sizeof(float), m->stream)) {
        m->d_m.reset(); return fail(m, FCN8S_ERR_OOM, "the optimizer's slots cannot be allocated");
    }
    HIPCHK(m, hipMemsetAsync(m->d_m, 0, m->total * sizeof(float), m->stream));
    HIPCHK(m, hipMemsetAsync(m->d_v, 0, m->total * sizeof(float), m->stream));
    return FCN8S_OK;
}

}

extern "C" {

size_t fcn8s_param_floats(const fcn8s_config* cfg)
{
    if (!cfg || cfg->num_classes <= 0) return 0;
    int C, widths[7], k; resolve_cfg(cfg, C, widths, k);
    std::vector<ParamInfo> t; size_t total, bo[FCN8S_MAX_BUCKETS], bn[FCN8S_MAX_BUCKETS];
    build_param_table(C, widths, k, t, total, bo, bn);
    return total;
}

int fcn8s_layout_num_params(const fcn8s_config* cfg)
{
    if (!cfg || cfg->num_classes <= 0) return 0;
    int C, widths[7], k; resolve_cfg(cfg, C, widths, k);
    std::vector<ParamInfo> t; size_t total, bo[FCN8S_MAX_BUCKETS], bn[FCN8S_MAX_BUCKETS];
    build_param_table(C, widths, k, t, total, bo, bn);
    return (int)t.size();
}
int fcn8s_layout_param(const fcn8s_config* cfg, int index, char name_out[64], int32_t* ndim, int64_t shape[4], int64_t* off)
{
    if (!cfg || cfg->num_classes <= 0) return FCN8S_ERR_BAD_ARG;
    int C, widths[7], k; resolve_cfg(cfg, C, widths, k);
    std::vector<ParamInfo> t; size_t total, bo[FCN8S_MAX_BUCKETS], bn[FCN8S_MAX_BUCKETS];
    build_param_table(C, widths, k, t, total, bo, bn);
    if (index < 0 || index >= (int)t.size()) return FCN8S_ERR_BAD_ARG;
    if (name_out) { strncpy(name_out, t[index].name.c_str(), 63); name_out[63] = 0; }
    if (ndim) *ndim = t[index].ndim;
    if (shape) for (int i = 0; i < 4; ++i) shape[i] = t[index].shape[i];
    if (off) *off = (int64_t)t[index].offset;
    return FCN8S_OK;
}
int fcn8s_layout_num_buckets(const fcn8s_config* cfg) { return (cfg && cfg->num_classes > 0) ? kNumBuckets : 0; }
int fcn8s_layout_bucket(const fcn8s_config* cfg, int bucket, size_t* off, size_t* n)
{
    if (!cfg || cfg->num_classes <= 0 || bucket < 0 || bucket >= kNumBuckets) return FCN8S_ERR_BAD_ARG;
    int C, widths[7], k; resolve_cfg(cfg, C, widths, k);
    std::vector<ParamInfo> t; size_t total, bo[FCN8S_MAX_BUCKETS], bn[FCN8S_MAX_BUCKETS];
    build_param_table(C, widths, k, t, total, bo, bn);
    if (off) *off = bo[bucket];
    if (n) *n = bn[bucket];
    return FCN8S_OK;
}

int fcn8s_create(const fcn8s_config* cfg, fcn8s_model** out)
{
    if (!cfg || !out) return fail(nullptr, FCN8S_ERR_BAD_ARG, "fcn8s_create: null argument");
    if (cfg->num_classes <= 0 || cfg->num_classes % 4 != 0 || cfg->num_classes > 64)
        return fail(nullptr, FCN8S_ERR_BAD_ARG, "fcn8s_create: num_classes must be a positive multiple of 4, at most 64 (the Python facade pads other class counts)");
    fcn8s_model* m = new fcn8s_model();
    resolve_cfg(cfg, m->C, m->widths, m->fc6k);
    for (int i = 0; i < 7; ++i)
        if (m->widths[i] % 4) { delete m; return fail(nullptr, FCN8S_ERR_BAD_ARG, "fcn8s_create: channel widths must be multiples of 4"); }
    if (m->fc6k % 2 == 0) { delete m; return fail(nullptr, FCN8S_ERR_BAD_ARG, "fcn8s_create: fc6_ksize must be odd"); }
    m->device = cfg->device_id; m->seed = cfg->seed;
    hipError_t e = hipSetDevice(m->device);
    if (e != hipSuccess) { delete m; return fail(nullptr, FCN8S_ERR_HIP, std::string("hipSetDevice: ") + hipGetErrorString(e) + " (libfcn8s_hip needs an AMD GPU; there is no CPU fallback)"); }
    {
        hipDeviceProp_t prop;
        if (hipGetDeviceProperties(&prop, m->device) == hipSuccess && prop.sharedMemPerBlock < FCN8S_LDS_BYTES_NEEDED) {
            const std::string msg = std::string("fcn8s_create: device ") + std::to_string(m->device) + " (" + prop.gcnArchName + ") offers " + std::to_string(prop.sharedMemPerBlock) +
                                    " bytes of LDS per workgroup; this library is written for gfx950 (MI355X) and needs " + std::to_string(FCN8S_LDS_BYTES_NEEDED);
            delete m; return fail(nullptr, FCN8S_ERR_HIP, msg);
        }
    }
    build_param_table(m->C, m->widths, m->fc6k, m->params, m->total, m->bucket_off, m->bucket_n);
    for (size_t i = 0; i < m->params.size(); ++i) m->index[m->params[i].name] = (int)i;
    bool ok = true;
    auto dev = [&](auto& buf, size_t n, bool zero = false) { ok = ok && buf.grow(n * sizeof(*buf.get()), nullptr, nullptr, zero); };
    if (cfg->ext_params) m->d_params = (float*)cfg->ext_params; else { dev(m->own_params, m->total, true); m->d_params = m->own_params; }
    if (cfg->ext_grads) m->d_grads = (float*)cfg->ext_grads; else { dev(m->own_grads, m->total, true); m->d_grads = m->own_grads; }
    dev(m->d_wt, m->total);
    dev(m->d_w1pad, 12 * 4 * (size_t)m->widths[0] + 64, true);
    const size_t cc = (size_t)m->C * m->C;
    dev(m->d_tph[0], 16 * cc); dev(m->d_tph[1], 16 * cc); dev(m->d_tph[2], 256 * cc);
    {
        int cmax = 0; for (int i = 0; i < 5; ++i) cmax = std::max(cmax, m->widths[i]);
        m->ufl = 64 * (size_t)cmax * cmax;
        if (m->fc6k == 7) m->ufl = std::max(m->ufl, fc6_bank_floats(m->widths[4], m->widths[5]));
        dev(m->d_wino_u, m->ufl);
    }
    dev(m->d_loss, 2 + 64 + 4, true);
    m->d_regsum = m->d_loss + 1; m->d_lastbias = m->d_loss + 2; m->d_terms = m->d_loss + 2 + 64;
    dev(m->d_conf, cc, true); dev(m->d_fp, 1);
    m->tg_kp = (4 * m->C + 63) / 64 * 64;
    {
        const size_t NC = 64 * (size_t)m->C, KP = (size_t)m->tg_kp;
        dev(m->tg_b2, 4 * (size_t)m->C * NC); dev(m->tg_b2t, NC * KP); dev(m->tg_db2, KP * NC); dev(m->tg_bias, NC);
    }
    if (!ok) { fcn8s_destroy(m); return fail(nullptr, FCN8S_ERR_OOM, "fcn8s_create: out of device memory"); }
    hipStreamSynchronize(nullptr);
    m->h_loss.grow(64, nullptr);
    if (hipEventCreateWithFlags(&m->loss_ev, hipEventDisableTiming) != hipSuccess) { m->loss_ev = nullptr; (void)hipGetLastError(); }
    *out = m;
    return FCN8S_OK;
}

int fcn8s_destroy(fcn8s_model* m)
{
    if (!m) return FCN8S_OK;
    const int rc_comm = fcn8s_comm_destroy(m);
    const std::string comm_text = rc_comm ? m->err : std::string();
    hipDeviceSynchronize();
    m->streams_seen.insert(m->stream);
    int cur = m->device; (void)hipGetDevice(&cur);
    if (cur != m->device && hipSetDevice(m->device) != hipSuccess) (void)hipGetLastError();
    for (hipStream_t s : m->streams_seen) scratch_release(s);
    if (cur != m->device) (void)hipSetDevice(cur);
    delete m;
    if (rc_comm) { g_last_error = comm_text; return rc_comm; }
    return FCN8S_OK;
}

const char* fcn8s_last_error(const fcn8s_model* m) { return m ? m->err.c_str() : g_last_error.c_str(); }

int fcn8s_freeze_params(fcn8s_model* m, int frozen)
{
    if (!m) return FCN8S_ERR_BAD_ARG;
    if (!frozen || !m->frozen) drop_banks(m);
    m->frozen = frozen != 0;
    return FCN8S_OK;
}

int fcn8s_set_precision(fcn8s_model* m, int precision)
{
    if (!m) return FCN8S_ERR_BAD_ARG;
    if (precision < FCN8S_PREC_F32 || precision > FCN8S_PREC_FP8_INFER)
        return fail(m, FCN8S_ERR_BAD_ARG, "fcn8s_set_precision: unknown precision");
    if (precision == FCN8S_PREC_BF16_TRAIN) {
        for (int i = 0; i < 7; ++i)
            if (m->widths[i] % 64) return fail(m, FCN8S_ERR_BAD_ARG, "fcn8s_set_precision: the bf16_train mode needs every channel width to be a multiple of 64");
    }
    if (precision == FCN8S_PREC_FP8_INFER) {
        for (int i = 0; i < 7; ++i)
            if (m->widths[i] % 64) return fail(m, FCN8S_ERR_BAD_ARG, "fcn8s_set_precision: the fp8_infer mode needs every channel width to be a multiple of 64");
        if (m->fc6k % 2 == 0) return fail(m, FCN8S_ERR_BAD_ARG, "fcn8s_set_precision: the fp8_infer mode needs an odd fc6 kernel size");
    }
    if (precision == FCN8S_PREC_BF16_FC || precision == FCN8S_PREC_BF16_FWD || precision == FCN8S_PREC_BF16_FWD_X2) {
        if (m->widths[4] % 32 || m->widths[5] % 128 || m->widths[6] % 128)
            return fail(m, FCN8S_ERR_BAD_ARG, "fcn8s_set_precision: the bf16 modes need conv5 width % 32 == 0 and fc6 / fc7 widths % 128 == 0");
    }
    if (precision != m->precision) {
        HIPCHK(m, hipStreamSynchronize(m->stream));
        drop_precision_state(m);
        const bool was = direct_mode(m->precision), now = direct_mode(precision);
        if (was != now) {
            if (now) { m->saved_wino_min_cin = m->wino_min_cin; m->saved_wino_fc6 = m->wino_fc6; m->wino_min_cin = 0; m->wino_fc6 = 0; }
            else { if (m->saved_wino_min_cin >= 0) m->wino_min_cin = m->saved_wino_min_cin; if (m->saved_wino_fc6 >= 0) m->wino_fc6 = m->saved_wino_fc6; }
            drop_arena(m);
        }
    }
    m->precision = precision;
    return FCN8S_OK;
}
int fcn8s_get_precision(const fcn8s_model* m) { return m ? m->precision : -1; }

int fcn8s_fp8_calibrate(fcn8s_model* m, const void* images, int dtype, int N, int H, int W, int where, int reset)
{
    if (!m || !images) return fail(m, FCN8S_ERR_BAD_ARG, "fcn8s_fp8_calibrate: null argument");
    if (!fp8_mode(m)) return fail(m, FCN8S_ERR_STATE, "fcn8s_fp8_calibrate: set the fp8_infer precision first (fcn8s_set_precision(m, FCN8S_PREC_FP8_INFER))");
    int rc = check_shape(m, N, H, W); if (rc) return rc;
    if (!m->d_fp8_amax.grow(FCN8S_FP8_LAYERS * sizeof(unsigned), m->stream)) return fail(m, FCN8S_ERR_OOM, "fcn8s_fp8_calibrate: out of device memory");
    float start[FCN8S_FP8_LAYERS] = {};
    if (!reset && m->fp8_calibrated) memcpy(start, m->fp8_amax, sizeof start);
    HIPCHK(m, hipStreamSynchronize(m->stream));
    HIPCHK(m, hipMemcpy(m->d_fp8_amax, start, sizeof start, hipMemcpyHostToDevice));
    FwdCall call; call.calibrating = true;
    rc = run_pass(m, images, dtype, nullptr, N, H, W, where, call); if (rc) return rc;
    {
        double by = 0;
        for (int L = 0; L < FCN8S_FP8_LAYERS; ++L) by += 4.0 * N * (H / kFp8InDiv[L]) * (W / kFp8InDiv[L]) * m->widths[kFp8InWidth[L]];
        ProfScope ps(m, "fp8_calibrate", 0, by);
        for (int L = 0; L < FCN8S_FP8_LAYERS; ++L) {
            const char* in = kFp8Inputs[L];
            auto it = m->acts.find(in);
            if (it == m->acts.end() || !it->second.p || m->pass.y_unwritten.count(in))
                return fail(m, FCN8S_ERR_STATE, std::string("fcn8s_fp8_calibrate: the fp32 pass did not materialise ") + in);
            const long long n = (long long)N * (H / kFp8InDiv[L]) * (W / kFp8InDiv[L]) * m->widths[kFp8InWidth[L]];
            launch_amax(it->second.p, n, m->d_fp8_amax + L, m->stream);
        }
    }
    unsigned bits[FCN8S_FP8_LAYERS];
    HIPCHK(m, hipMemcpyAsync(bits, m->d_fp8_amax, sizeof bits, hipMemcpyDeviceToHost, m->stream));
    HIPCHK(m, hipStreamSynchronize(m->stream));
    memcpy(m->fp8_amax, bits, sizeof bits);
    m->fp8_calibrated = true;
    return FCN8S_OK;
}
int fcn8s_fp8_get_calibration(const fcn8s_model* m, float* amax, int n)
{
    if (!m || !amax || n != FCN8S_FP8_LAYERS) return FCN8S_ERR_BAD_ARG;
    if (!m->fp8_calibrated) return FCN8S_ERR_STATE;
    memcpy(amax, m->fp8_amax, sizeof m->fp8_amax);
    return FCN8S_OK;
}
int fcn8s_fp8_set_calibration(fcn8s_model* m, const float* amax, int n)
{
    if (!m || !amax) return fail(m, FCN8S_ERR_BAD_ARG, "fcn8s_fp8_set_calibration: null argument");
    if (n != FCN8S_FP8_LAYERS) return fail(m, FCN8S_ERR_BAD_ARG, "fcn8s_fp8_set_calibration: needs FCN8S_FP8_LAYERS (14) maxima");
    for (int i = 0; i < n; ++i)
        if (!std::isfinite(amax[i]) || amax[i] < 0.f) return fail(m, FCN8S_ERR_BAD_ARG, "fcn8s_fp8_set_calibration: maxima must be finite and >= 0");
    memcpy(m->fp8_amax, amax, sizeof m->fp8_amax);
    m->fp8_calibrated = true;
    return FCN8S_OK;
}

static int* model_option(fcn8s_model* m, const std::string& key)
{
    if (key == "winograd_min_cin") return &m->wino_min_cin;
    if (key == "winograd_tile") return &m->wino_tile;
    if (key == "winograd_fc6") return &m->wino_fc6;
    if (key == "fc6_fft") return &m->fc6_fft;
    if (key == "fc6_fft_wgrad") return &m->fc6_fft_wgrad;
    if (key == "tconv_gemm") return &m->tconv_gemm;
    if (key == "fuse_dgrad_dout") return &m->fuse_dgrad_dout;
    if (key == "fuse_out_in") return &m->fuse_out_in;
    if (key == "bf16_gemm256") return &m->bf16_gemm256;
    if (key == "winograd_tile_hires") return &m->wino_tile_hires;
    if (key == "winograd_hires_pixels") return &m->wino_hires_pixels;
    if (key == "conv1_tiled") return &m->conv1_tiled;
    if (key == "conv1_wgrad_mfma") return &m->conv1_wgrad_mfma;
    if (key == "bf16_copy_by_transform") return &m->bf16_copy_by_transform;
    if (key == "conv1_in_transform") return &m->conv1_in_transform;
    if (key == "deterministic") return &m->deterministic;
    if (key == "bf16_acts") return &m->bf16_acts;
    if (key == "bf16_rows_bn") return &m->bf16_rows_bn;
    if (key == "keep_output_gradients") return &m->keep_dy;
    if (key == "bf16_infer_copies") return &m->bf16_infer_copies;
    if (key == "bf16_fuse_pool") return &m->bf16_fuse_pool;
    return nullptr;
}
int fcn8s_set_option(fcn8s_model* m, const char* key, int64_t value)
{
    if (!key) return fail(m, FCN8S_ERR_BAD_ARG, "fcn8s_set_option: null key");
    const std::string k = key;
    if (k == "device_bytes_live" || k == "scratch_bytes_live") return fail(m, FCN8S_ERR_BAD_ARG, "fcn8s_set_option: '" + k + "' is read-only");
    if (!m) {
        if (k == "op_f32x3") { t_op_split = value ? 3 : 0; return FCN8S_OK; }
        if (k == "op_deterministic") { t_deterministic = value ? 1 : 0; return FCN8S_OK; }
        if (k == "op_bf16_planes") { t_op_planes = value ? 1 : 0; return FCN8S_OK; }
        if (k == "op_bf16_rows_bn") { if (value != 0 && value != 64 && value != 128) return fail(nullptr, FCN8S_ERR_BAD_ARG, "op_bf16_rows_bn must be 0, 64 or 128"); t_op_rows_bn = (int)value; return FCN8S_OK; }
        if (k == "op_split_pieces") {
            if (value != 0 && value != 2 && value != 3) return fail(nullptr, FCN8S_ERR_BAD_ARG, "fcn8s_set_option: op_split_pieces is 0, 2 or 3");
            t_op_split = (int)value; return FCN8S_OK;
        }
        return fail(nullptr, FCN8S_ERR_NOT_FOUND, "fcn8s_set_option: unknown op-context option '" + k + "' (model options need a model)");
    }
    if (k == "workspace_allocations" || k == "frozen") return fail(m, FCN8S_ERR_BAD_ARG, "fcn8s_set_option: '" + k + "' is read-only (the frozen state is set with fcn8s_freeze_params)");
    if (k == "comm_timeout_ms") {
        if (value < 1) return fail(m, FCN8S_ERR_BAD_ARG, "comm_timeout_ms must be >= 1");
        std::lock_guard<std::mutex> lk(m->comm_mu); m->comm_timeout_ms = value; return FCN8S_OK;
    }
    if (k == "conv1_tiled" || k == "conv1_wgrad_mfma" || k == "bf16_copy_by_transform" || k == "conv1_in_transform" || k == "deterministic" || k == "bf16_acts" || k == "bf16_rows_bn" || k == "bf16_fuse_pool" || k == "keep_output_gradients" || k == "bf16_infer_copies") {
        *model_option(m, k) = k == "bf16_rows_bn" ? (int)value : (value ? 1 : 0);
        return FCN8S_OK;
    }
    int* slot = model_option(m, k);
    if (!slot) return fail(m, FCN8S_ERR_NOT_FOUND, "fcn8s_set_option: unknown option '" + k + "'");
    if (direct_mode(m->precision) && (k == "winograd_min_cin" || k == "winograd_fc6")) {
        if (value < 0) return fail(m, FCN8S_ERR_BAD_ARG, "fcn8s_set_option: negative value");
        (k == "winograd_min_cin" ? m->saved_wino_min_cin : m->saved_wino_fc6) = (int)value;
        return FCN8S_OK;
    }
    if (k == "winograd_tile" && value != 2 && value != 4 && value != 6) return fail(m, FCN8S_ERR_BAD_ARG, "winograd_tile must be 2, 4 or 6");
    if (k == "winograd_tile_hires" && value != 0 && value != 2 && value != 4 && value != 6) return fail(m, FCN8S_ERR_BAD_ARG, "winograd_tile_hires must be 0, 2, 4 or 6");
    if (k == "winograd_min_cin" && value < 0) return fail(m, FCN8S_ERR_BAD_ARG, "winograd_min_cin must be >= 0 (0 = direct convolution everywhere)");
    if (k == "fuse_out_in" && (value < 0 || value > 2)) return fail(m, FCN8S_ERR_BAD_ARG, "fuse_out_in must be 0, 1 or 2");
    if (k == "fc6_fft_wgrad" && (value < 0 || value > 2)) return fail(m, FCN8S_ERR_BAD_ARG, "fc6_fft_wgrad must be 0, 1 or 2");
    if (*slot == (int)value) return FCN8S_OK;
    HIPCHK(m, hipStreamSynchronize(m->stream));
    *slot = (k == "winograd_fc6" || k == "fc6_fft" || k == "tconv_gemm") ? (value != 0) : (int)value;
    drop_arena(m);
    drop_banks(m, true); m->u_train.clear();
    return FCN8S_OK;
}
int fcn8s_get_option(const fcn8s_model* m, const char* key, int64_t* value)
{
    if (!key || !value) return FCN8S_ERR_BAD_ARG;
    const std::string k = key;
    if (k == "device_bytes_live") { *value = g_device_bytes_live.load(); return FCN8S_OK; }
    if (k == "scratch_bytes_live") { *value = scratch_bytes_live(); return FCN8S_OK; }
    if (!m) {
        if (k == "op_f32x3") { *value = t_op_split == 3; return FCN8S_OK; }
        if (k == "op_deterministic") { *value = t_deterministic; return FCN8S_OK; }
        if (k == "op_bf16_planes") { *value = t_op_planes; return FCN8S_OK; }
        if (k == "op_bf16_rows_bn") { *value = t_op_rows_bn; return FCN8S_OK; }
        if (k == "op_split_pieces") { *value = t_op_split; return FCN8S_OK; }
        return FCN8S_ERR_NOT_FOUND;
    }
    if (k == "comm_timeout_ms") { *value = m->comm_timeout_ms; return FCN8S_OK; }
    if (k == "workspace_allocations") { *value = m->ws_allocs; return FCN8S_OK; }
    if (k == "frozen") { *value = m->frozen ? 1 : 0; return FCN8S_OK; }
    const int* slot = model_option(const_cast<fcn8s_model*>(m), k);
    if (!slot) return FCN8S_ERR_NOT_FOUND;
    *value = *slot;
    if (direct_mode(m->precision) && k == "winograd_min_cin" && m->saved_wino_min_cin >= 0) *value = m->saved_wino_min_cin;
    if (direct_mode(m->precision) && k == "winograd_fc6" && m->saved_wino_fc6 >= 0) *value = m->saved_wino_fc6;
    return FCN8S_OK;
}

int fcn8s_set_stream(fcn8s_model* m, void* s)
{
    if (!m) return FCN8S_ERR_BAD_ARG;
    hipStream_t to = (hipStream_t)s;
    if (to == m->stream) return FCN8S_OK;
    int cur = m->device; (void)hipGetDevice(&cur);
    if (cur != m->device) HIPCHK(m, hipSetDevice(m->device));
    hipError_t e = hipSuccess;
    if (!m->move_ev) { e = hipEventCreateWithFlags(&m->move_ev, hipEventDisableTiming); if (e != hipSuccess) m->move_ev = nullptr; }
    if (e == hipSuccess) e = hipEventRecord(m->move_ev, m->stream);
    if (e == hipSuccess) e = hipStreamWaitEvent(to, m->move_ev, 0);
    if (e != hipSuccess) {
        (void)hipGetLastError();
        e = hipStreamSynchronize(m->stream);
        if (e != hipSuccess) { (void)hipGetLastError(); e = hipDeviceSynchronize(); }
    }
    m->streams_seen.insert(m->stream);
    m->stream = to;
    if (cur != m->device) (void)hipSetDevice(cur);
    HIPCHK(m, e);
    return FCN8S_OK;
}
int fcn8s_synchronize(fcn8s_model* m) { if (!m) return FCN8S_ERR_BAD_ARG; HIPCHK(m, hipStreamSynchronize(m->stream)); return FCN8S_OK; }

int fcn8s_num_params(const fcn8s_model* m) { return m ? (int)m->params.size() : 0; }
int fcn8s_param_info(const fcn8s_model* m, int i, const char** name, int32_t* ndim, int64_t shape[4], int64_t* off)
{
    if (!m || i < 0 || i >= (int)m->params.size()) return FCN8S_ERR_BAD_ARG;
    const ParamInfo& p = m->params[i];
    if (name) *name = p.name.c_str();
    if (ndim) *ndim = p.ndim;
    if (shape) for (int k = 0; k < 4; ++k) shape[k] = p.shape[k];
    if (off) *off = (int64_t)p.offset;
    return FCN8S_OK;
}
int fcn8s_param_index(const fcn8s_model* m, const char* name)
{
    if (!m || !name) return -1;
    auto it = m->index.find(name);
    return it == m->index.end() ? -1 : it->second;
}
static int xfer_named(fcn8s_model* m, float* base, const char* name, void* host, size_t n, bool to_dev)
{
    if (!m || !name || !host) return fail(m, FCN8S_ERR_BAD_ARG, "null argument");
    const int i = fcn8s_param_index(m, name);
    if (i < 0) return fail(m, FCN8S_ERR_NOT_FOUND, std::string("unknown variable '") + name + "'");
    const ParamInfo& p = m->params[i];
    if (n != p.numel) return fail(m, FCN8S_ERR_SHAPE, std::string("variable '") + name + "' has " + std::to_string(p.numel) + " elements, got " + std::to_string(n));
    if (base == m->d_grads) { int rcw = fcn8s_comm_wait(m); if (rcw) return rcw; }
    HIPCHK(m, hipStreamSynchronize(m->stream));
    if (to_dev) HIPCHK(m, hipMemcpy(base + p.offset, host, n * sizeof(float), hipMemcpyHostToDevice));
    else HIPCHK(m, hipMemcpy(host, base + p.offset, n * sizeof(float), hipMemcpyDeviceToHost));
    return FCN8S_OK;
}
int fcn8s_set_param(fcn8s_model* m, const char* name, const float* host, size_t n)
{
    if (m && m->frozen) fcn8s_freeze_params(m, 0);
    fp8_clear_calibration(m);
    return xfer_named(m, m ? m->d_params : nullptr, name, (void*)host, n, true);
}
int fcn8s_get_param(fcn8s_model* m, const char* name, float* host, size_t n) { return xfer_named(m, m ? m->d_params : nullptr, name, host, n, false); }
int fcn8s_get_grad(fcn8s_model* m, const char* name, float* host, size_t n) { return xfer_named(m, m ? m->d_grads : nullptr, name, host, n, false); }
void* fcn8s_param_buffer(fcn8s_model* m, size_t* n) { if (!m) return nullptr; if (n) *n = m->total; return m->d_params; }
void* fcn8s_grad_buffer(fcn8s_model* m, size_t* n) { if (!m) return nullptr; if (n) *n = m->total; return m->d_grads; }
int fcn8s_num_buckets(const fcn8s_model* m) { return m ? kNumBuckets : 0; }
int fcn8s_bucket_range(const fcn8s_model* m, int b, size_t* off, size_t* n)
{
    if (!m || b < 0 || b >= kNumBuckets) return FCN8S_ERR_BAD_ARG;
    if (off) *off = m->bucket_off[b];
    if (n) *n = m->bucket_n[b];
    return FCN8S_OK;
}

int fcn8s_init_params(fcn8s_model* m, uint64_t seed)
{
    if (m && m->frozen) fcn8s_freeze_params(m, 0);
    fp8_clear_calibration(m);
    if (!m) return FCN8S_ERR_BAD_ARG;
    HIPCHK(m, hipMemsetAsync(m->d_params, 0, m->total * sizeof(float), m->stream));
    uint32_t sid = 1000;
    for (auto& p : m->params) {
        ++sid;
        if (p.ndim == 1) continue;
        float std; int trunc = 0;
        const bool vgg = p.name.find("/filter") != std::string::npos || p.name.find("/weights") != std::string::npos;
        if (vgg) std = sqrtf(2.0f / (float)(p.shape[0] * p.shape[1] * p.shape[2]));
        else if (p.name.find("trans") != std::string::npos) { std = 0.01f; trunc = 1; }
        else { std = 0.001f; trunc = 1; }
        launch_init_normal(m->d_params + p.offset, (long long)p.numel, std, trunc, seed, sid, m->stream);
    }
    HIPCHK(m, hipGetLastError());
    return FCN8S_OK;
}

int fcn8s_forward_loss(fcn8s_model* m, const void* images, int dtype, const uint8_t* labels, int N, int H, int W,
                       float keep_prob, float l2_rate, int where)
{
    if (fp8_mode(m)) return fp8_refuse_training(m, "fcn8s_forward_loss");
    if (m && m->frozen) fcn8s_freeze_params(m, 0);
    fp8_clear_calibration(m);
    if (!m || !images || !labels) return fail(m, FCN8S_ERR_BAD_ARG, "fcn8s_forward_loss: null argument");
    if (!(keep_prob > 0.f && keep_prob <= 1.f)) return fail(m, FCN8S_ERR_BAD_ARG, "keep_prob must be in (0, 1]");
    if (m->kd_w != 0.f) {
        if (!m->kd_probs) return fail(m, FCN8S_ERR_STATE, "fcn8s_set_soft_targets is on and no targets are bound: call fcn8s_bind_soft_targets before every training loss");
        if (m->kd_N != N || m->kd_H != H || m->kd_W != W)
            return fail(m, FCN8S_ERR_SHAPE, "the bound soft targets are for a batch of " + std::to_string(m->kd_N) + " x " + std::to_string(m->kd_H) + " x " +
                        std::to_string(m->kd_W) + ", the training loss for " + std::to_string(N) + " x " + std::to_string(H) + " x " + std::to_string(W));
    }
    FwdCall call; call.keep_prob = keep_prob; call.train = true;
    const uint8_t* lab;
    int rc = run_pass(m, images, dtype, labels, N, H, W, where, call, &lab); if (rc) return rc;
    rc = compute_loss(m, lab, l2_rate, true); if (rc) return rc;
    m->kd_probs = nullptr;
    m->next_bucket = 0;
    for (int b = 0; b < kNumBuckets; ++b) m->acc_taken[b] = false;
    HIPCHK(m, hipGetLastError());
    return FCN8S_OK;
}

int fcn8s_backward_bucket(fcn8s_model* m, int bucket)
{
    if (!m || bucket < 0 || bucket >= kNumBuckets) return fail(m, FCN8S_ERR_BAD_ARG, "bad bucket");
    if (fp8_mode(m)) return fp8_refuse_training(m, "fcn8s_backward_bucket");
    take_deferred_error(nullptr);
    int rc = do_backward_bucket(m, bucket); if (rc) { take_deferred_error(nullptr); return rc; }
    return deferred_rc(m);
}

int fcn8s_bucket_wait(fcn8s_model* m, int bucket, void* hip_stream)
{
    if (!m || bucket < 0 || bucket >= kNumBuckets) return fail(m, FCN8S_ERR_BAD_ARG, "fcn8s_bucket_wait: bad bucket");
    if (!m->bucket_final[bucket] || !m->bucket_ev[bucket])
        return fail(m, FCN8S_ERR_STATE, "fcn8s_bucket_wait: the bucket's gradients are not queued yet (call fcn8s_backward_bucket(bucket) first)");
    HIPCHK(m, hipStreamWaitEvent((hipStream_t)hip_stream, m->bucket_ev[bucket], 0));
    return FCN8S_OK;
}

int fcn8s_bucket_complete_after(const fcn8s_model* m, int bucket)
{
    if (!m || bucket < 0 || bucket >= kNumBuckets) return -1;
// ... 1774 lines not shown
```

Baseline: 294.6 images/sec.

## Add stream-K GEMM kernel with partial-tile fixup and route 1x1 dgrad through transposed-B

Adds a stream-K variant of the MFMA implicit GEMM. It splits the total k-iteration space evenly across a resident-sized grid and merges partial tiles through a global scratch buffer, using atomic counters and spin-waits. A cost model picks it only when it beats the tiled schedule's wave-quantization tail. Separately, fc7 dgrad now uses a transposed-B GEMM directly on the forward weights, which removes an eager weight flip-transpose. The stream-K path adds fixup traffic, spin-wait risk, and extra scratch memory.

```diff
diff --git a/fcn8s_tensorflow_amd/csrc/fcn8s_internal.h b/fcn8s_tensorflow_amd/csrc/fcn8s_internal.h
--- a/fcn8s_tensorflow_amd/csrc/fcn8s_internal.h
+++ b/fcn8s_tensorflow_amd/csrc/fcn8s_internal.h
@@ -113,6 +113,8 @@
 float* scratch2(hipStream_t s, size_t floats);
 void scratch_release(hipStream_t s);
 long long scratch_bytes_live();
+extern thread_local int t_gemm_streamk, t_gemm_streamk_grid;
+extern thread_local long long t_gemm_streamk_launches;
 void launch_det_reduce(float* C, const float* ws, long long rows, int cols, int ldc, long long slab, int nsplit, bool accumulate, hipStream_t s);
 bool launch_wgrad_taps(const float* X, const float* dZ, float* dW, float* db, int N, int H, int W, int Cin, int Cout,
                        int K, hipStream_t s);
diff --git a/fcn8s_tensorflow_amd/csrc/igemm.hip b/fcn8s_tensorflow_amd/csrc/igemm.hip
--- a/fcn8s_tensorflow_amd/csrc/igemm.hip
+++ b/fcn8s_tensorflow_amd/csrc/igemm.hip
@@ -24,13 +24,16 @@
 }
 
 thread_local int t_deterministic = 0;
+thread_local int t_gemm_streamk = 1, t_gemm_streamk_grid = 0;
+thread_local long long t_gemm_streamk_launches = 0;
 namespace {
 struct ScratchBuf { float* p = nullptr; size_t cap = 0; };
 std::mutex g_scratch_mu;
-std::map<std::pair<int, hipStream_t>, ScratchBuf> g_scratch[2];
+std::map<std::pair<int, hipStream_t>, ScratchBuf> g_scratch[3];
 std::atomic<long long> g_scratch_bytes{0};
-float* scratch_get(int which, hipStream_t s, size_t floats, size_t floor_)
-{
+float* scratch_get(int which, hipStream_t s, size_t floats, size_t floor_, bool* fresh = nullptr)
+{
+    if (fresh) *fresh = false;
     int dev = 0; (void)hipGetDevice(&dev);
     std::lock_guard<std::mutex> lk(g_scratch_mu);
     ScratchBuf& b = g_scratch[which][std::make_pair(dev, s)];
@@ -41,6 +44,7 @@
         if (want < floor_) want = floor_;
         if (hipMalloc((void**)&b.p, want * sizeof(float)) != hipSuccess) { (void)hipGetLastError(); return nullptr; }
         b.cap = want; g_scratch_bytes += (long long)(want * sizeof(float));
+        if (fresh) *fresh = true;
     }
     return b.p;
 }
@@ -666,6 +670,234 @@
     }
 }
 
+struct StreamKArgs { float* partials; unsigned* counters; long long total; int ntm, ntn, nkt; };
+constexpr unsigned kStreamKSpinLimit = 1u << 22;
+
+template <int BM, int BN, int WM, int WN, int S, bool BT>
+__global__ __launch_bounds__(256, (S * (BM + BN) * 64 <= 40960) ? 4 : 3) void gemm_glds_sk_kernel(const IgemmArgs p, const StreamKArgs q)
+{
+    constexpr int BK = 16, CH = 4, RPI = 16;
+    constexpr int TM = BM / WM / 32, TN = BN / WN / 32;
+    constexpr int A_PW = BM / RPI / 4, B_PW = BT ? BN / RPI / 4 : BK * BN / 256 / 4;
+    static_assert(WM * WN == 4 && A_PW >= 1 && B_PW >= 1 && BM == 128, "tile / wave split");
+    constexpr int L = A_PW + B_PW;
+    constexpr int STAGE = BM * BK + BK * BN;
+    __shared__ __attribute__((aligned(16))) float smem[S * STAGE];
+    static_assert(S * STAGE >= 4 * 32 * 36, "epilogue patches");
+
+    const int tid = threadIdx.x, lane = tid & 63, wave = __builtin_amdgcn_readfirstlane(tid >> 6);
+    const int wm = wave / WN, wn = wave % WN;
+    const unsigned G = gridDim.x, lg = xcd_swizzle(blockIdx.x, G);
+    auto range_start = [&](unsigned b) { return (long long)((unsigned long long)q.total * b / G); };
+    const long long it0 = range_start(lg), it1 = range_start(lg + 1);
+
+    unsigned b_voff[B_PW];
+#pragma unroll
+    for (int i = 0; i < B_PW; ++i) {
+        if (BT) {
+            const int row = (wave * B_PW + i) * RPI + lane / CH, pc = lane % CH;
+            const int c = pc ^ ((row >> 2) & 3);
+            b_voff[i] = (unsigned)(row * p.ldw + c * 4) * 4u;
+        } else {
+            const int f = (wave * B_PW + i) * 64 + lane;
+            const int k = f / (BN / 4), j = (f % (BN / 4)) * 4;
+            b_voff[i] = (unsigned)(k * p.Cout + j) * 4u;
+        }
+    }
+    const unsigned lds0 = (unsigned)(size_t)(__attribute__((address_space(3))) float*)smem;
+    int a_off[TM], a_sw[TM];
+#pragma unroll
+    for (int tm = 0; tm < TM; ++tm) {
+        const int row = wm * TM * 32 + tm * 32 + (lane & 31);
+        a_off[tm] = row * BK;
+        a_sw[tm] = (row >> 2) & 3;
+    }
+    const int b_off = ((lane >> 5) * 4) * BN + wn * TN * 32 + (lane & 31);
+    int bt_off[TN], bt_sw[TN];
+#pragma unroll
+    for (int tn = 0; tn < TN; ++tn) {
+        const int row = wn * TN * 32 + tn * 32 + (lane & 31);
+        bt_off[tn] = row * BK;
+        bt_sw[tn] = (row >> 2) & 3;
+    }
+
+    const int per = q.ntm * q.ntn;
+    long long it_end = it1;
+    while (it_end > it0) {
+        const long long tile = (it_end - 1) / q.nkt, tile_it = tile * q.nkt;
+        const long long seg0 = it0 > tile_it ? it0 : tile_it;
+        const int kb = (int)(seg0 - tile_it), ke = (int)(it_end - tile_it), nkt = ke - kb;
+        const int pz = (int)(tile / per), t = (int)(tile % per);
+        const long long m0 = (long long)(p.m_fastest ? t % q.ntm : t / q.ntn) * BM;
+        const int n0 = (p.m_fastest ? t / q.ntm : t % q.ntn) * BN;
+        const float* __restrict__ Wp = p.w + (long long)pz * p.w_phase_stride;
+        const float* __restrict__ X = p.batched ? p.x + (long long)pz * p.x_batch_stride : p.x;
+        float* __restrict__ Y = p.batched ? p.y + (long long)pz * p.y_batch_stride : p.y;
+
+        unsigned a_voff[A_PW];
+#pragma unroll
+        for (int i = 0; i < A_PW; ++i) {
+            const int row = (wave * A_PW + i) * RPI + lane / CH, pc = lane % CH;
+            const int c = pc ^ ((row >> 2) & 3);
+            long long m = m0 + row; if (m >= p.M) m = p.M - 1;
+            a_voff[i] = (unsigned)((m - m0) * p.ldx + c * 4) * 4u;
+        }
+        const float* a_base = X + m0 * p.ldx + (long long)kb * BK;
+        const float* b_base = BT ? Wp + (long long)n0 * p.ldw + (long long)kb * BK : Wp + n0 + (long long)kb * BK * p.Cout;
+        auto issue = [&](int kt, int stage) {
+            const float* ga = a_base + (long long)kt * BK;
+            const float* gb = BT ? b_base + (long long)kt * BK : b_base + (long long)kt * BK * p.Cout;
+            const unsigned la = lds0 + (unsigned)(stage * STAGE + wave * A_PW * 256) * 4u;
+            const unsigned lb = lds0 + (unsigned)(stage * STAGE + BM * BK + wave * B_PW * 256) * 4u;
+#pragma unroll
+            for (int i = 0; i < A_PW; ++i) glds16(ga, a_voff[i], la + i * 1024);
+#pragma unroll
+            for (int i = 0; i < B_PW; ++i) glds16(gb, b_voff[i], lb + i * 1024);
+        };
+
+        f32x16 acc[TM][TN];
+#pragma unroll
+        for (int i = 0; i < TM; ++i)
+#pragma unroll
+            for (int j = 0; j < TN; ++j)
+#pragma unroll
+                for (int r = 0; r < 16; ++r) acc[i][j][r] = 0.f;
+
+        auto compute = [&](int stage) {
+            const float* sa = smem + stage * STAGE;
+            const float* sb = sa + BM * BK;
+#pragma unroll
+            for (int kk2 = 0; kk2 < BK / 8; ++kk2) {
+                float4 af[TM];
+                float bf[TN][4];
+#pragma unroll
+                for (int tm = 0; tm < TM; ++tm)
+                    af[tm] = *reinterpret_cast<const float4*>(sa + a_off[tm] + (((kk2 * 2 + (lane >> 5)) ^ a_sw[tm]) * 4));
+#pragma unroll
+                for (int tn = 0; tn < TN; ++tn) {
+                    if (BT) {
+                        const float4 tt = *reinterpret_cast<const float4*>(sb + bt_off[tn] + (((kk2 * 2 + (lane >> 5)) ^ bt_sw[tn]) * 4));
+                        bf[tn][0] = tt.x; bf[tn][1] = tt.y; bf[tn][2] = tt.z; bf[tn][3] = tt.w;
+                    } else {
+#pragma unroll
+                        for (int j = 0; j < 4; ++j) bf[tn][j] = sb[b_off + (kk2 * 8 + j) * BN + tn * 32];
+                    }
+                }
+#pragma unroll
+                for (int j = 0; j < 4; ++j)
+#pragma unroll
+                    for (int tm = 0; tm < TM; ++tm) {
+                        const float av = j == 0 ? af[tm].x : j == 1 ? af[tm].y : j == 2 ? af[tm].z : af[tm].w;
+#pragma unroll
+                        for (int tn = 0; tn < TN; ++tn) acc[tm][tn] = __builtin_amdgcn_mfma_f32_32x32x2f32(av, bf[tn][j], acc[tm][tn], 0, 0, 0);
+                    }
+            }
+        };
+
+        wait_vmcnt<0>();
+#pragma unroll
+        for (int tt = 0; tt < S - 1; ++tt)
+            if (tt < nkt) issue(tt, tt);
+        int stage = 0, pre = S - 1;
+        for (int kt = 0; kt < nkt; ++kt) {
+            if (kt + S - 2 < nkt) wait_vmcnt<(S - 2) * L>(); else wait_vmcnt<0>();
+            __builtin_amdgcn_s_barrier();
+            if (kt + S - 1 < nkt) issue(kt + S - 1, pre);
+            compute(stage);
+            stage = stage + 1 == S ? 0 : stage + 1;
+            pre = pre + 1 == S ? 0 : pre + 1;
+        }
+        __builtin_amdgcn_s_barrier();
+
+        bool store_tile = true, poisoned = false;
+        if (ke < q.nkt) {
+            float4* slot = reinterpret_cast<float4*>(q.partials + (size_t)lg * (BM * BN));
+#pragma unroll
+            for (int tm = 0; tm < TM; ++tm)
+#pragma unroll
+                for (int tn = 0; tn < TN; ++tn)
+#pragma unroll
+                    for (int g4 = 0; g4 < 4; ++g4)
+                        slot[((tm * TN + tn) * 4 + g4) * 256 + tid] = make_float4(acc[tm][tn][4 * g4], acc[tm][tn][4 * g4 + 1], acc[tm][tn][4 * g4 + 2], acc[tm][tn][4 * g4 + 3]);
+            asm volatile("s_waitcnt vmcnt(0)" ::: "memory");
+            __syncthreads();
+            if (tid == 0) {
+                __builtin_amdgcn_fence(__ATOMIC_RELEASE, "agent");
+                asm volatile("s_waitcnt vmcnt(0)" ::: "memory");
+                __hip_atomic_fetch_add(q.counters + tile, 1u, __ATOMIC_RELAXED, __HIP_MEMORY_SCOPE_AGENT);
+            }
+            store_tile = false;
+        } else if (kb > 0) {
+            unsigned gf = lg;
+            while (gf > 0 && range_start(gf) > tile_it) --gf;
+            const unsigned need = lg - gf;
+            if (tid == 0) {
+                unsigned spins = 0;
+                while (__hip_atomic_load(q.counters + tile, __ATOMIC_RELAXED, __HIP_MEMORY_SCOPE_AGENT) < need && spins < kStreamKSpinLimit) { __builtin_amdgcn_s_sleep(16); ++spins; }
+                if (spins >= kStreamKSpinLimit) __hip_atomic_store(q.counters - 1, 1u, __ATOMIC_RELAXED, __HIP_MEMORY_SCOPE_AGENT);
+                else __hip_atomic_store(q.counters + tile, 0u, __ATOMIC_RELAXED, __HIP_MEMORY_SCOPE_AGENT);
+                __builtin_amdgcn_fence(__ATOMIC_ACQUIRE, "agent");
+                asm volatile("s_waitcnt vmcnt(0)" ::: "memory");
+                smem[0] = spins >= kStreamKSpinLimit ? 1.f : 0.f;
+            }
+            __syncthreads();
+            poisoned = smem[0] != 0.f;
+#pragma unroll
+            for (int tm = 0; tm < TM; ++tm)
+#pragma unroll
+                for (int tn = 0; tn < TN; ++tn) {
+                    f32x16 sum;
+#pragma unroll
+                    for (int r = 0; r < 16; ++r) sum[r] = 0.f;
+                    for (unsigned b = gf; b < lg; ++b) {
+                        const float4* slot = reinterpret_cast<const float4*>(q.partials + (size_t)b * (BM * BN));
+#pragma unroll
+                        for (int g4 = 0; g4 < 4; ++g4) {
+                            const float4 v = slot[((tm * TN + tn) * 4 + g4) * 256 + tid];
+                            sum[4 * g4] += v.x; sum[4 * g4 + 1] += v.y; sum[4 * g4 + 2] += v.z; sum[4 * g4 + 3] += v.w;
+                        }
+                    }
+#pragma unroll
+                    for (int r = 0; r < 16; ++r) acc[tm][tn][r] = poisoned ? __builtin_nanf("") : sum[r] + acc[tm][tn][r];
+                }
+            __syncthreads();
+        }
+
+        if (store_tile) {
+            constexpr int LDT = 36;
+            float* patch = smem + wave * 32 * LDT;
+#pragma unroll
+            for (int tn = 0; tn < TN; ++tn)
+#pragma unroll
+                for (int tm = 0; tm < TM; ++tm) {
+#pragma unroll
+                    for (int r = 0; r < 16; ++r) patch[((r & 3) + 8 * (r >> 2) + 4 * (lane >> 5)) * LDT + (lane & 31)] = acc[tm][tn][r];
+                    __builtin_amdgcn_wave_barrier();
+                    const long long mrow = m0 + wm * TM * 32 + tm * 32;
+                    float* yb = Y + n0 + wn * TN * 32 + tn * 32 + (lane & 7) * 4;
+                    const float4 bv = p.bias ? ldg4(p.bias + n0 + wn * TN * 32 + tn * 32 + (lane & 7) * 4) : make_float4(0.f, 0.f, 0.f, 0.f);
+#pragma unroll
+                    for (int j = 0; j < 4; ++j) {
+                        const int row = j * 8 + (lane >> 3);
+                        float4 v = *reinterpret_cast<const float4*>(&patch[row * LDT + (lane & 7) * 4]);
+                        v.x += bv.x; v.y += bv.y; v.z += bv.z; v.w += bv.w;
+                        if (mrow + row < p.M) {
+                            if (p.mask) {
+                                const float4 mk = ldg4(p.mask + (mrow + row) * p.ldy + n0 + wn * TN * 32 + tn * 32 + (lane & 7) * 4);
+                                v.x = mk.x > 0.f ? v.x * p.mask_scale : 0.f; v.y = mk.y > 0.f ? v.y * p.mask_scale : 0.f;
+                                v.z = mk.z > 0.f ? v.z * p.mask_scale : 0.f; v.w = mk.w > 0.f ? v.w * p.mask_scale : 0.f;
+                            }
+                            *reinterpret_cast<float4*>(yb + (mrow + row) * p.ldy) = v;
+                        }
+                    }
+                    __builtin_amdgcn_wave_barrier();
+                }
+        }
+        __syncthreads();
+        it_end = seg0;
+    }
+}
+
 static __device__ __forceinline__ void glds16v(const float* vaddr, unsigned lds_byte_off)
 {
     asm volatile("s_mov_b32 m0, %1\n\ts_nop 0\n\tglobal_load_lds_dwordx4 %0, off" ::"v"(vaddr), "s"(lds_byte_off) : "memory", "m0");
@@ -866,6 +1098,59 @@
     }
     g_last_kernel = "conv1_glds_kernel";
     hipLaunchKernelGGL(conv1_glds_kernel, dim3((unsigned)((a.M + 127) / 128)), dim3(256), 0, s, a);
+    return true;
+}
+
+constexpr size_t kStreamKMaxTiles = 1u << 20;
+constexpr size_t kStreamKHead = 4 + kStreamKMaxTiles;
+template <typename Kern>
+static int streamk_slots(Kern kernel, int lds_bpc, int* cus_out)
+{
+    static std::mutex mu; static std::map<int, std::pair<int, int>> known;
+    int dev = 0; (void)hipGetDevice(&dev);
+    std::lock_guard<std::mutex> lk(mu);
+    auto it = known.find(dev);
+    if (it != known.end()) { *cus_out = it->second.second; return it->second.first; }
+    int nb = 0, cus = 0;
+    if (hipOccupancyMaxActiveBlocksPerMultiprocessor(&nb, kernel, 256, 0) != hipSuccess) { (void)hipGetLastError(); nb = 0; }
+    if (hipDeviceGetAttribute(&cus, hipDeviceAttributeMultiprocessorCount, dev) != hipSuccess) { (void)hipGetLastError(); cus = 0; }
+    const int slots = std::min(nb, lds_bpc) * cus;
+    known[dev] = std::make_pair(slots, cus); *cus_out = cus;
+    return slots;
+}
+constexpr double kStreamKFixup = 0.5, kStreamKLoop = 1.09;
+static bool streamk_cheaper(long long blocks, int bpc, int cus, int nkt)
+{
+    const long long n = (blocks + cus - 1) / cus, rem = n % bpc;
+    const double tail = rem == 0 ? 0.0 : (rem == 1 ? 2.0 : (rem == 2 ? 2.4 : 3.0));
+    const double tiled = (double)(n / bpc) * bpc + tail, even = kStreamKLoop * blocks / cus + kStreamKFixup * 32.0 / nkt;
+    return even < tiled;
+}
+template <int BM, int BN, int WM, int WN, bool BT>
+static bool launch_streamk(const IgemmArgs& a, int phases, unsigned ntm, unsigned ntn, bool by_cost, hipStream_t s)
+{
+    constexpr int S = 3, lds_bpc = (S * (BM + BN) * 64 <= 40960) ? 4 : 3;
+    auto kernel = gemm_glds_sk_kernel<BM, BN, WM, WN, S, BT>;
+    int cus = 0;
+    const int slots = streamk_slots(kernel, lds_bpc, &cus);
+    const long long tiles = (long long)ntm * ntn * phases;
+    const int nkt = a.Ktot / 16;
+    if (slots <= 0 || tiles <= 0 || (size_t)tiles > kStreamKMaxTiles || nkt <= 0) return false;
+    if (by_cost && !(tiles > slots && streamk_cheaper(tiles, lds_bpc, cus, nkt))) return false;
+    StreamKArgs q{};
+    q.total = tiles * nkt; q.ntm = (int)ntm; q.ntn = (int)ntn; q.nkt = nkt;
+    long long G = std::min<long long>(slots, tiles);
+    if (t_gemm_streamk_grid > 0) G = std::min<long long>(std::min<long long>(t_gemm_streamk_grid, slots), q.total);
+    if (G < 1 || G > slots) { defer_error(FCN8S_ERR_STATE, "stream-K GEMM: a grid of %lld blocks on %d resident slots", G, slots); return true; }
+    bool fresh = false;
+    float* sc = scratch_get(2, s, kStreamKHead + (size_t)G * BM * BN, 0, &fresh);
+    if (!sc) return false;
+    if (fresh) hipMemsetAsync(sc, 0, kStreamKHead * sizeof(float), s);
+    q.counters = reinterpret_cast<unsigned*>(sc) + 4; q.partials = sc + kStreamKHead;
+    static const std::string tag = "gemm_glds_sk_kernel<" + std::to_string(BM) + ", " + std::to_string(BN) + ", " + std::to_string(WM) + ", " + std::to_string(WN) + ", 3, " + (BT ? "true>" : "false>");
+    g_last_kernel = tag.c_str();
+    hipLaunchKernelGGL(kernel, dim3((unsigned)G), dim3(256), 0, s, a, q);
+    ++t_gemm_streamk_launches;
     return true;
 }
 
@@ -887,7 +1172,12 @@
     const bool linear = (mode == 1 || mode == 3) && !a.relu && !a.mask && !a.dropout && !a.addend && a.out_scale == 1 && a.ldy == a.Cout;
     constexpr int splitk_min_kt = 64;
     const unsigned nblocks = grid.x * (unsigned)phases, nkt_all = (unsigned)(a.Ktot / BKF);
-    if (linear && !t_deterministic && !a.fixed_tile && ((grid.x < 512 && nkt_all >= 512) || (nblocks < 2048 && nkt_all >= (unsigned)splitk_min_kt))) {
+    const bool rows1x1 = fast && a.Ktot == a.Cin && a.in_scale == 1 && a.tap_off == 0 && a.out_scale == 1 && a.out_offy == 0 && a.out_offx == 0 &&
+                         (a.batched || (phases == 1 && a.Hi == a.Ma && a.Wi == a.Mb && a.Ho == a.Ma && a.Wo == a.Mb)) && a.ldy >= a.Cout;
+    const bool store16 = mode == 3 || (fast && !a.addend && !a.relu && !a.dropout && a.alpha == 1.f && a.ldy % 4 == 0 && a.Cout % 4 == 0 && (a.bias != nullptr) != (a.mask != nullptr));
+    const bool sk_legal = BM == 128 && BN >= 64 && BKF == 16 && t_gemm_streamk != 0 && a.split == 0 && rows1x1 && store16 && (long long)(BM - 1) * a.ldx < (1LL << 29) &&
+                          (long long)16 * a.Cout < (1LL << 29) && (!a.bt || (long long)(BN - 1) * a.ldw < (1LL << 29));
+    if (linear && !t_deterministic && !a.fixed_tile && !(sk_legal && t_gemm_streamk == 2) && ((grid.x < 512 && nkt_all >= 512) || (nblocks < 2048 && nkt_all >= (unsigned)splitk_min_kt))) {
         unsigned ks = nkt_all >= 512 && grid.x < 512 ? 1024 / grid.x : 4096 / nblocks;
         if (ks > 8) ks = 8;
         if (ks > nkt_all / 16) ks = nkt_all / 16;
@@ -897,8 +1187,6 @@
             hipMemsetAsync(a.y, 0, nfl * sizeof(float), s);
         }
     }
-    const bool rows1x1 = fast && a.Ktot == a.Cin && a.in_scale == 1 && a.tap_off == 0 && a.out_scale == 1 && a.out_offy == 0 && a.out_offx == 0 &&
-                         (a.batched || (phases == 1 && a.Hi == a.Ma && a.Wi == a.Mb && a.Ho == a.Ma && a.Wo == a.Mb)) && a.ldy >= a.Cout;
     const bool bias_only = fast && a.bias && !a.addend && !a.mask && !a.relu && !a.dropout && a.alpha == 1.f && a.ldy % 4 == 0 && a.Cout % 4 == 0 && grid.y == 1;
     if constexpr (BN >= 64 && BKF == 16) {
         if (rows1x1 && (mode == 3 || grid.y == 1) && (long long)(BM - 1) * a.ldx < (1LL << 29) && (long long)16 * a.Cout < (1LL << 29)) {
@@ -907,10 +1195,18 @@
             static const std::string gt[4] = {gbase + "false>", gbase + "true>", xbase + "false>", xbase + "true>"};
             const bool mask_only = fast && a.mask && !a.bias && !a.addend && !a.relu && !a.dropout && a.alpha == 1.f && a.ldy % 4 == 0 && a.Cout % 4 == 0 && grid.y == 1;
             const bool epi = mode != 3 && !bias_only && !mask_only;
+            if constexpr (BM == 128) {
+                if (sk_legal && !epi && grid.y == 1) {
+                    const unsigned ntm = (unsigned)((a.M + BM - 1) / BM), ntn = (unsigned)(a.Cout / BN);
+                    const bool by_cost = t_gemm_streamk != 2;
+                    if (a.bt ? launch_streamk<BM, BN, WM, WN, true>(a, phases, ntm, ntn, by_cost, s) : launch_streamk<BM, BN, WM, WN, false>(a, phases, ntm, ntn, by_cost, s)) return;
+                    g_last_kernel = tags[mode].c_str();
+                }
+            }
             if (a.bt) {
                 static const std::string nb = "gemm_glds_nt_kernel<" + std::to_string(BM) + ", " + std::to_string(BN) + ", " + std::to_string(WM) + ", " + std::to_string(WN) + ", 3>";
                 static const std::string nbx = "gemm_glds_nt_x3_kernel<" + std::to_string(BM) + ", " + std::to_string(BN) + ", " + std::to_string(WM) + ", " + std::to_string(WN) + ", 3>";
-                if (mode != 3 || (long long)(BN - 1) * a.ldw >= (1LL << 29)) { defer_error(FCN8S_ERR_STATE, "transposed-B GEMM needs the plain batched form"); return; }
+                if (epi || (long long)(BN - 1) * a.ldw >= (1LL << 29)) { defer_error(FCN8S_ERR_STATE, "transposed-B GEMM needs the plain batched form, or rows with at most a bias or a mask"); return; }
                 static const std::string nbx2 = "gemm_glds_nt_x2_kernel<" + std::to_string(BM) + ", " + std::to_string(BN) + ", " + std::to_string(WM) + ", " + std::to_string(WN) + ", 3>";
                 g_last_kernel = (a.split == 3 ? nbx : a.split == 2 ? nbx2 : nb).c_str();
                 if (a.split == 3) hipLaunchKernelGGL((gemm_glds_nt_x3_kernel<BM, BN, WM, WN, 3>), grid, dim3(256), 0, s, a);
@@ -955,8 +1251,9 @@
         const double tail = rem == 0 ? 0.0 : (rem == 1 ? 2.0 : (rem == 2 ? 2.4 : 3.0));
         return ((double)(n / bpc) * bpc + tail) * bm * bn / eff;
     };
-    if (a.fixed_tile && a.Cout % 128 == 0) { launch_igemm_cfg<128, 128, 2, 2>(a, phases, s); return; }
-    if (a.fixed_tile && a.Cout % 64 == 0)  { launch_igemm_cfg<128, 64, 2, 2>(a, phases, s); return; }
+    const bool rows128 = a.fixed_tile || (t_gemm_streamk == 2 && a.split == 0);
+    if (rows128 && a.Cout % 128 == 0) { launch_igemm_cfg<128, 128, 2, 2>(a, phases, s); return; }
+    if (rows128 && a.Cout % 64 == 0)  { launch_igemm_cfg<128, 64, 2, 2>(a, phases, s); return; }
     if (a.Cout <= 32)      launch_igemm_cfg<128, 32, 4, 1>(a, phases, s);
     else if (a.Cout <= 64) {
         if (cost(128, 64, 4, 1.0) <= cost(64, 64, 4, 0.9)) launch_igemm_cfg<128, 64, 2, 2>(a, phases, s);
diff --git a/fcn8s_tensorflow_amd/csrc/model.hip b/fcn8s_tensorflow_amd/csrc/model.hip
--- a/fcn8s_tensorflow_amd/csrc/model.hip
+++ b/fcn8s_tensorflow_amd/csrc/model.hip
@@ -125,6 +125,7 @@
     int wino_fc6 = 1;
     int fc6_fft = 1;
     int fc6_fft_wgrad = 1;
+    int gemm_streamk = 1;
     int wino_tile_hires = 0, wino_hires_pixels = 0;
     int wino_force_tile = 0;
     int precision = FCN8S_PREC_F32;
@@ -713,6 +714,16 @@
     return Route::taken;
 }
 
+static Route dgrad_1x1_bt(const BwdCall& c, const float* dy, float* dx, const DgradEpi& e)
+{
+    const int Cdy = c.fwd.Cout, Cdx = c.fwd.Cin;
+    if (!(c.fwd.K == 1 && e.w_fwd && e.mask && !e.addend && !e.relu_bits_in && e.alpha == 1.f && Cdy >= 64 && bt_gemm_ok(Cdy, Cdx))) return Route::declined;
+    IgemmArgs a{}; a.mask = e.mask; a.alpha = 1.f; a.mask_scale = e.mask_scale; a.keep_prob = 1.f;
+    a.bt = 1; a.ldw = Cdy;
+    conv_direct(c.m, c.group, a, dy, e.w_fwd, dx, c.fwd.N, c.fwd.H, c.fwd.W, Cdy, Cdx, 1, c.s, 0, c.layer);
+    return Route::taken;
+}
+
 static Route dgrad_winograd(const BwdCall& c, bool v_ready, const float* dy, const float* wt, float* dx, const DgradEpi& e)
 {
     fcn8s_model* m = c.m;
@@ -745,6 +756,7 @@
     if (dgrad_fft6(c, dy, dx, e) == Route::taken) return;
     if (dgrad_adjoint(c, dm_ready, dx, e) == Route::taken) return;
     if (dgrad_fc6_adjoint(c, dm_ready, dx, e) == Route::taken) return;
+    if (dgrad_1x1_bt(c, dy, dx, e) == Route::taken) return;
     if (e.lazy_wt && e.w_fwd) {
         ProfScope ps(m, "weight_relayout", 0, 8.0 * K * K * Cdy * Cdx); launch_flip_transpose(e.w_fwd, const_cast<float*>(wt), K * K, Cdx, Cdy, s);
     }
@@ -1650,7 +1662,7 @@
 int forward(fcn8s_model* m, const void* img_dev, int dtype, const FwdCall& call)
 {
     const float keep_prob = call.keep_prob; const bool train = call.train; const McLoop* mc = call.mc;
-    t_deterministic = m->deterministic;
+    t_deterministic = m->deterministic; t_gemm_streamk = m->gemm_streamk; t_gemm_streamk_grid = 0;
     hipStream_t s = m->stream;
     const int N = m->N, H = m->H, W = m->W, C = m->C;
     const bool fp8 = fp8_mode(m) && !train && !call.calibrating;
@@ -1907,9 +1919,7 @@
 void prepare_backward_weights(fcn8s_model* m)
 {
     hipStream_t s = m->stream;
-    ProfScope ps(m, "weight_relayout", 0, 8.0 * ((double)m->widths[5] * m->widths[6] +
-                                                 (double)m->C * (m->widths[2] + m->widths[3] + m->widths[6])));
-    launch_flip_transpose(Wp(m, "fc7/weights"), WTp(m, "fc7/weights"), 1, m->widths[5], m->widths[6], s);
+    ProfScope ps(m, "weight_relayout", 0, 8.0 * (double)m->C * (m->widths[2] + m->widths[3] + m->widths[6]));
     launch_flip_transpose(Wp(m, "pool3_1x1/kernel"), WTp(m, "pool3_1x1/kernel"), 1, m->widths[2], m->C, s);
     launch_flip_transpose(Wp(m, "pool4_1x1/kernel"), WTp(m, "pool4_1x1/kernel"), 1, m->widths[3], m->C, s);
     launch_flip_transpose(Wp(m, "fc7_1x1/kernel"), WTp(m, "fc7_1x1/kernel"), 1, m->widths[6], m->C, s);
@@ -1968,7 +1978,7 @@
     const int N = m->N, H = m->H, W = m->W;
     const int h5 = H / 32, w5 = W / 32;
     const float inv_keep = (m->train_mode && m->keep_prob < 1.f) ? 1.f / m->keep_prob : 1.f;
-    { DgradEpi e; e.mask = A(m, "fc6"); e.mask_scale = inv_keep; e.w_fwd = Wp(m, "fc7/weights"); e.yb_layer = "fc6"; e.yb_K = m->fc6k;
+    { DgradEpi e; e.mask = A(m, "fc6"); e.mask_scale = inv_keep; e.w_fwd = Wp(m, "fc7/weights"); e.lazy_wt = 1; e.yb_layer = "fc6"; e.yb_K = m->fc6k;
       conv_dgrad(m, "fc7_dgrad", m->gbuf[0], WTp(m, "fc7/weights"), m->gbuf[1], N, h5, w5, m->widths[6], m->widths[5], 1, e, s, "fc7"); }
     conv_wgrad(m, "fc6_wgrad", A(m, "pool5"), m->gbuf[1], Gp(m, "fc6/weights"), Gp(m, "fc6/biases"), N, h5, w5, m->widths[4], m->widths[5], m->fc6k, 1.f, s, 0, "fc6");
     mark_bucket_final(m, 1, s);
@@ -2027,7 +2037,7 @@
 
 int do_backward_bucket(fcn8s_model* m, int bucket)
 {
-    t_deterministic = m->deterministic;
+    t_deterministic = m->deterministic; t_gemm_streamk = m->gemm_streamk; t_gemm_streamk_grid = 0;
     if (!m->have_loss || !m->train_mode) return fail(m, FCN8S_ERR_STATE, "fcn8s_backward_bucket: call fcn8s_forward_loss first");
     if (bucket != m->next_bucket) return fail(m, FCN8S_ERR_STATE, "fcn8s_backward_bucket: buckets must be run in order 0, 1, ... fcn8s_num_buckets() - 1");
     if (bucket == 0) {
@@ -2273,6 +2283,7 @@
     if (key == "winograd_fc6") return &m->wino_fc6;
     if (key == "fc6_fft") return &m->fc6_fft;
     if (key == "fc6_fft_wgrad") return &m->fc6_fft_wgrad;
+    if (key == "gemm_streamk") return &m->gemm_streamk;
     if (key == "tconv_gemm") return &m->tconv_gemm;
     if (key == "fuse_dgrad_dout") return &m->fuse_dgrad_dout;
     if (key == "fuse_out_in") return &m->fuse_out_in;
@@ -2305,12 +2316,18 @@
             if (value != 0 && value != 2 && value != 3) return fail(nullptr, FCN8S_ERR_BAD_ARG, "fcn8s_set_option: op_split_pieces is 0, 2 or 3");
             t_op_split = (int)value; return FCN8S_OK;
         }
+        if (k == "gemm_streamk") { if (value < 0 || value > 2) return fail(nullptr, FCN8S_ERR_BAD_ARG, "gemm_streamk must be 0, 1 or 2"); t_gemm_streamk = (int)value; return FCN8S_OK; }
+        if (k == "op_gemm_streamk_grid") { if (value < 0 || value > 4096) return fail(nullptr, FCN8S_ERR_BAD_ARG, "op_gemm_streamk_grid must be 0 .. 4096"); t_gemm_streamk_grid = (int)value; return FCN8S_OK; }
         return fail(nullptr, FCN8S_ERR_NOT_FOUND, "fcn8s_set_option: unknown op-context option '" + k + "' (model options need a model)");
     }
     if (k == "workspace_allocations" || k == "frozen") return fail(m, FCN8S_ERR_BAD_ARG, "fcn8s_set_option: '" + k + "' is read-only (the frozen state is set with fcn8s_freeze_params)");
     if (k == "comm_timeout_ms") {
         if (value < 1) return fail(m, FCN8S_ERR_BAD_ARG, "comm_timeout_ms must be >= 1");
         std::lock_guard<std::mutex> lk(m->comm_mu); m->comm_timeout_ms = value; return FCN8S_OK;
+    }
+    if (k == "gemm_streamk") {
+        if (value < 0 || value > 2) return fail(m, FCN8S_ERR_BAD_ARG, "gemm_streamk must be 0, 1 or 2");
+        m->gemm_streamk = (int)value; return FCN8S_OK;
     }
     if (k == "conv1_tiled" || k == "conv1_wgrad_mfma" || k == "bf16_copy_by_transform" || k == "conv1_in_transform" || k == "deterministic" || k == "bf16_acts" || k == "bf16_rows_bn" || k == "bf16_fuse_pool" || k == "keep_output_gradients" || k == "bf16_infer_copies") {
         *model_option(m, k) = k == "bf16_rows_bn" ? (int)value : (value ? 1 : 0);
@@ -2347,6 +2364,9 @@
         if (k == "op_bf16_planes") { *value = t_op_planes; return FCN8S_OK; }
         if (k == "op_bf16_rows_bn") { *value = t_op_rows_bn; return FCN8S_OK; }
         if (k == "op_split_pieces") { *value = t_op_split; return FCN8S_OK; }
+        if (k == "gemm_streamk") { *value = t_gemm_streamk; return FCN8S_OK; }
+        if (k == "op_gemm_streamk_grid") { *value = t_gemm_streamk_grid; return FCN8S_OK; }
+        if (k == "op_gemm_streamk_launches") { *value = t_gemm_streamk_launches; return FCN8S_OK; }
         return FCN8S_ERR_NOT_FOUND;
     }
     if (k == "comm_timeout_ms") { *value = m->comm_timeout_ms; return FCN8S_OK; }
```

After: 296.6 images/sec, median of 6. No clear change (+0.7%).
